# Gabriel-SGama/Semantic-SuperPoint

Hardware: AMD Instinct MI355X
Metric: image-pairs/sec at 240x320 bs32 (pair training step) (higher is better)
Workload: dtype f32

## Files before the change

### include/ssp_hip.h

```cpp
#ifndef SSP_HIP_H
#define SSP_HIP_H

#include <stddef.h>
#include <stdint.h>

#ifdef __cplusplus
extern "C" {
#endif

typedef struct ssp_handle ssp_handle;

enum { SSP_ARCH_GAUSS2 = 0, SSP_ARCH_GAUSS2_SSMALL = 1 };
enum { SSP_NREP = 32 };

typedef struct {
  int arch;
  int n_classes;
  int max_batch;
  int height;
  int width;
  int n_match;
  int n_non;
  int dense_loss;
} ssp_config;
// ... 333 lines not shown
int ssp_op_world_correspondences(const double* x_dev, const int32_t* state_dev, int map_cap, const float* match_dev,
                                 const int32_t* n_match_dev, int cap, const double* pts_new_dev, int pt_stride,
                                 const int32_t* count_new_dev, int point_cap, double* corr_dev, int32_t* n_corr_dev, void* stream);
int ssp_world_repair(const double* rw_dev, const double* c_dev, const int32_t* status_dev, double* state_dev, double* table_dev,
                     int capacity, int map_cap, int32_t* world_state_dev, void* stream);

#define SSP_LOOP_MAX_EDGES 256
#define SSP_LOOP_EDGE_WORDS 16
#define SSP_LOOP_STATE_WORDS 8
#define SSP_LOOP_CAND_WORDS 16
#define SSP_LOOP_MAX_INNER 8
#define SSP_LOOP_INFO_WORDS 8
#define SSP_LOOP_MAX_ITERATIONS 64
#define SSP_POSE_FLAG_LOOP 32
size_t ssp_pose_graph_workspace_bytes(int capacity);
int ssp_op_loop_correspondences(const double* x_dev, const int32_t* last_dev, const int32_t* state_dev, int map_cap,
                                const float* match_dev, const int32_t* n_match_dev, int cap, const double* pts_new_dev, int pt_stride,
                                const int32_t* count_new_dev, int point_cap, const double* landmarks_dev,
                                const int32_t* n_landmarks_dev, int row_cap, int f, int min_gap, double* corr_dev, double* xnew_dev,
                                int32_t* n_dev, void* stream);
int ssp_loop_edge(const double* rw_dev, const double* c_dev, const uint8_t* mask_dev, const int32_t* status_dev,
                  const double* corr_dev, const double* xnew_dev, const int32_t* n_dev, int cap, const int32_t* last_dev, int map_cap,
                  const double* table_dev, int capacity, int f, int min_inliers, int cooldown, double weight, double* edges_dev,
                  int32_t* state_dev, double* cand_dev, void* stream);
int ssp_pose_graph(const double* table_dev, int capacity, const double* edges_dev, const int32_t* state_dev, int f, int iterations,
                   void* workspace_dev, double* rw_out_dev, double* c_out_dev, double* sigma_out_dev, double* info_dev, void* stream);
int ssp_loop_apply(const double* info_dev, const double* rw_new_dev, const double* c_new_dev, const double* sigma_dev,
                   int32_t* loop_state_dev, int f, double* state_dev, double* table_dev, int capacity, double* x_dev,
                   const int32_t* last_dev, const int32_t* world_state_dev, int map_cap, void* stream);

#define SSP_EVAL_ACC_MAX_PAIRS 128
#define SSP_EVAL_ROW_WORDS 16
#define SSP_EVAL_STATE_WORDS 16
int ssp_eval_pixel_homographies(const float* hn_dev, int n_pairs, int height, int width, double* hom_dev, double* hom_inv_dev,
                                void* stream);
int ssp_eval_accumulate(const double* rep_dev, const double* h_dev, const int32_t* n_inlier_dev, const int32_t* status_dev,
                        const double* ap_dev, const int32_t* n1_dev, int pair_stride, const double* hom_dev, int n_pairs,
                        int corner_h, int corner_w, const double* thresholds, int64_t first_pair, double* rows_dev,
                        int64_t capacity, double* state_dev, void* stream);

#define SSP_DET_EVAL_MAX_R2 64
#define SSP_DET_EVAL_STATE_WORDS 80
#define SSP_DET_EVAL_CURVE_TILE 1024
typedef struct ssp_det_eval_params {
  int32_t height, width;
  float remove_zero;
  int32_t r2;
  float prob_thresh;
  int32_t simplified;
} ssp_det_eval_params;
size_t ssp_det_eval_workspace_bytes(const ssp_det_eval_params* p, int b, int cap);
int ssp_op_det_tp_fp(const float* prob_dev, const void* labels_dev, int labels_u8, const ssp_det_eval_params* p, int b,
                     void* workspace_dev, int64_t* keys_dev, int64_t capacity, int64_t* state_dev, void* stream);
int ssp_op_det_tp_fp_points(const float* pts_dev, const int32_t* count_dev, int cap, const void* labels_dev, int labels_u8,
                            const ssp_det_eval_params* p, int b, void* workspace_dev, int64_t* keys_dev, int64_t capacity,
                            int64_t* state_dev, void* stream);
size_t ssp_det_pr_curve_workspace_bytes(int64_t n_records);
int ssp_op_det_pr_curve(const int64_t* sorted_keys_dev, int64_t n_records, const int64_t* state_dev, void* workspace_dev,
                        float* prob_dev, uint8_t* tp_dev, double* precision_dev, double* recall_dev, double* map_dev,
                        void* stream);

#define SSP_TRACK_MAX_LENGTH 16
size_t ssp_track_workspace_bytes(int max_length, int point_cap, int row_cap);
int ssp_op_track_update(const int32_t* ids_in_dev, const int32_t* tid_in_dev, const double* score_in_dev,
                        const int32_t* state_in_dev, const float* match_dev, const double* match_score64_dev,
                        const int32_t* n_match_dev, const int32_t* n_points_dev, int max_length, int point_cap, int row_cap,
                        void* workspace_dev, int32_t* ids_out_dev, int32_t* tid_out_dev, double* score_out_dev,
                        int32_t* state_out_dev, void* stream);
int ssp_op_track_select(const int32_t* ids_dev, const int32_t* tid_dev, const double* score_dev, const int32_t* state_dev,
                        int max_length, int row_cap, int min_length, void* workspace_dev, double* tracks_dev,
                        int32_t* n_tracks_dev, void* stream);
int ssp_op_track_points(const double* tracks_dev, const int32_t* n_tracks_dev, const double* pts_dev, const int32_t* state_dev,
                        int max_length, int point_cap, int track_cap, int first_slot, double* xy_dev, void* stream);

int ssp_op_bn_bwd(const float* y_dev, const float* dout_dev, const float* gamma_dev, const float* stats4_dev,
                  float* dy_dev, float* dgamma_dev, float* dbeta_dev, float* dbias_dev, double* sums_dev, int n, int h,
                  int w, int c, int relu, int pool, void* stream);
int ssp_op_bn_bwd_strided(const float* y_dev, const float* dout_dev, const float* gamma_dev, const float* stats4_dev,
                          float* dy_dev, float* dgamma_dev, float* dbeta_dev, float* dbias_dev, double* sums_dev, int n,
                          int h, int w, int c, int cs, int relu, int pool, void* stream);

int ssp_set_conv_algo(int algo);
int ssp_handle_set_conv_algo(ssp_handle* h, int algo);

int ssp_debug_conv_knobs(int ablate, int grid);
int ssp_debug_occupancy(int which);

int ssp_debug_buffer(ssp_handle* h, int slot, const char* name, float** ptr, size_t* nfloats);

int ssp_debug_backward_taps(ssp_handle* h, float* arena_dev, size_t arena_floats, unsigned layer_mask);
size_t ssp_debug_backward_tap_floats(const ssp_handle* h, unsigned layer_mask);
int ssp_debug_backward_tap(ssp_handle* h, int slot, int layer, int which, size_t* offset, size_t* nfloats, unsigned* route);

int ssp_op_sparse_loss(const float* desc_a_nhwc_dev, const float* desc_b_nhwc_dev, const int32_t* match_a_dev,
                       const int32_t* match_b_dev, const int32_t* nonmatch_b_dev, int b, int hc, int wc, int n_match,
                       int n_non, int method, int dist, float coef_pos, float coef_neg, float* dd_a_nhwc_dev, float* dd_b_nhwc_dev,
                       float* out2_dev, void* stream);
int ssp_op_sparse_loss_path(const float* desc_a_nhwc_dev, const float* desc_b_nhwc_dev, const int32_t* match_a_dev,
                            const int32_t* match_b_dev, const int32_t* nonmatch_b_dev, int b, int hc, int wc, int n_match,
                            int n_non, int method, int dist, float coef_pos, float coef_neg, float* dd_a_nhwc_dev, float* dd_b_nhwc_dev,
                            float* out2_dev, int gather, int32_t* csr_off_dev, int32_t* csr_match_dev, float* csr_weight_dev,
                            void* stream);

int ssp_op_dense_loss(const float* desc_a_nhwc_dev, const float* desc_b_nhwc_dev, const float* homographies_dev,
                      const float* valid_dev, int b, int hc, int wc, float lamda_d, float descriptor_dist, int multi_task,
                      float scale, void* scratch_dev, size_t scratch_bytes, float* out3_dev, float* dda_dev,
                      float* ddb_dev, void* stream);

#ifdef __cplusplus
}
#endif
#endif
```

### semantic-superpoint_amd/csrc/bn_kernels.hip.h

```cpp
#pragma once
#include <hip/hip_runtime.h>
#include <stdint.h>

#include "conv_mfma.hip.h"

namespace sspk {

template <typename T>
__device__ __forceinline__ float4 ld4(const T* p) {
  if constexpr (sizeof(T) == 4) {
    return *reinterpret_cast<const float4*>(p);
  } else {
    const u32x2 v = *reinterpret_cast<const u32x2*>(p);
    return make_float4(bf16_lo(v[0]), bf16_hi(v[0]), bf16_lo(v[1]), bf16_hi(v[1]));
  }
}
template <typename T>
__device__ __forceinline__ void st4(T* p, float4 v) {
  if constexpr (sizeof(T) == 4) {
    *reinterpret_cast<float4*>(p) = v;
  } else {
    u32x2 o;
    o[0] = pack_bf16(v.x, v.y);
    o[1] = pack_bf16(v.z, v.w);
// ... 192 lines not shown
      var = s2 / L.count - mean * mean;
      if (var < 0) var = 0;
      const double unbiased = L.count > 1 ? var * L.count / (L.count - 1) : var;
      if (writer) {
        L.running_mean[c] = (float)(0.9 * (double)L.running_mean[c] + 0.1 * mean);
        L.running_var[c] = (float)(0.9 * (double)L.running_var[c] + 0.1 * unbiased);
        if (c == 0 && nbt != nullptr) *nbt += 1;
      }
    } else {
      mean = L.running_mean[c];
      var = L.running_var[c];
    }
    if (writer) {
      const float invstd = (float)(1.0 / sqrt(var + 1e-5));
      const float sc = L.gamma[c] * invstd;
      L.mean[c] = (float)mean;
      L.invstd[c] = invstd;
      L.scale[c] = sc;
      L.shift[c] = L.beta[c] - (float)mean * sc;
    }
  }
}
__global__ void bn_finalize_kernel(const BnLayer L0, const BnLayer L1, int nviews, int train, int64_t* nbt) {
  bn_finalize_body(L0, L1, nviews, train, nbt);
}
struct BnFinJobs {
  BnLayer L0[3], L1[3];
  int64_t* nbt[3];
  int n;
};
__global__ void bn_finalize_multi_kernel(const BnFinJobs J, int nviews, int train) {
  const int j = blockIdx.y;
  bn_finalize_body(J.L0[j], J.L1[j], nviews, train, J.nbt[j]);
}

__global__ __launch_bounds__(256) void bn_relu_pool_kernel(const float* __restrict__ y0, const float* __restrict__ scale0,
                                                           const float* __restrict__ shift0, float* __restrict__ out0,
                                                           const float* __restrict__ y1, const float* __restrict__ scale1,
                                                           const float* __restrict__ shift1, float* __restrict__ out1,
                                                           int N, int H, int W, int C) {
  const float* __restrict__ y = blockIdx.y ? y1 : y0;
  const float* __restrict__ scale = blockIdx.y ? scale1 : scale0;
  const float* __restrict__ shift = blockIdx.y ? shift1 : shift0;
  float* __restrict__ out = blockIdx.y ? out1 : out0;
  const int nq = C >> 2;
  const long total = (long)N * (H / 2) * (W / 2) * nq;
  const int Wo = W / 2, Ho = H / 2;
  for (long idx = (long)blockIdx.x * blockDim.x + threadIdx.x; idx < total; idx += (long)gridDim.x * blockDim.x) {
    const int q = (int)(idx % nq);
    const long p = idx / nq;
    const int ox = (int)(p % Wo), oy = (int)((p / Wo) % Ho), n = (int)(p / ((long)Wo * Ho));
    const float4 sc = *reinterpret_cast<const float4*>(scale + q * 4);
    const float4 sh = *reinterpret_cast<const float4*>(shift + q * 4);
    const size_t base = ((size_t)(n * H + 2 * oy) * W + 2 * ox) * C + q * 4;
    const float4 a = xform<1>(*reinterpret_cast<const float4*>(y + base), sc, sh);
    const float4 b = xform<1>(*reinterpret_cast<const float4*>(y + base + C), sc, sh);
    const float4 c = xform<1>(*reinterpret_cast<const float4*>(y + base + (size_t)W * C), sc, sh);
    const float4 d = xform<1>(*reinterpret_cast<const float4*>(y + base + (size_t)W * C + C), sc, sh);
    *reinterpret_cast<float4*>(out + (size_t)p * C + q * 4) = max4(max4(a, b), max4(c, d));
  }
}

struct BnBwdArgs {
  const float* y;
  const float* dout;
  float* dy;
  const float* scale;
  const float* shift;
  const float* mean;
  const float* invstd;
  const float* gamma;
  double* sums;
  const float* k12;
  float* dbias;
  const float* x;
  const float* apool;
  const float* beta;
  int pool_fix;
  int N, H, W, C;
  int y_cs, y_co, d_cs, d_co, dy_cs, dy_co;
  double count;
};

template <bool RELU, bool POOL, bool APPLY, typename T = float>
__global__ __launch_bounds__(256) void bn_bwd_kernel(const BnBwdArgs a0, const BnBwdArgs a1, const BnBwdArgs b0, const BnBwdArgs b1) {
  const BnBwdArgs& a = blockIdx.y == 0 ? a0 : blockIdx.y == 1 ? a1 : blockIdx.y == 2 ? b0 : b1;
  const T* const t_y = reinterpret_cast<const T*>(a.y);
  const T* const t_dout = reinterpret_cast<const T*>(a.dout);
  T* const t_dy = reinterpret_cast<T*>(a.dy);
  __shared__ float red[256 * 8];
  const int tid = threadIdx.x;
  const int nq = (a.C + 3) / 4;
  const int rows = 256 / nq;
  const int q = tid % nq, pl = tid / nq;
  const bool active = pl < rows;
  const int c0 = q * 4;
  const int Ho = POOL ? a.H / 2 : a.H, Wo = POOL ? a.W / 2 : a.W;
  const long npix = (long)a.N * Ho * Wo;
  float4 sc = make_float4(0, 0, 0, 0), sh = sc, mu = sc, is = sc, k1 = sc, k2 = sc, gs = sc;
  bool cv[4];
#pragma unroll
  for (int i = 0; i < 4; ++i) cv[i] = (c0 + i) < a.C;
  auto ldp = [&](const float* p) {
    float4 v = make_float4(0, 0, 0, 0);
    if (cv[0]) v.x = p[c0];
    if (cv[1]) v.y = p[c0 + 1];
    if (cv[2]) v.z = p[c0 + 2];
    if (cv[3]) v.w = p[c0 + 3];
    return v;
  };
  if (active) {
    sc = ldp(a.scale);
    sh = ldp(a.shift);
    mu = ldp(a.mean);
    is = ldp(a.invstd);
    if (APPLY) {
      const float4 g = ldp(a.gamma);
      float s1[4], s2[4];
#pragma unroll
      for (int i = 0; i < 4; ++i) {
        s1[i] = cv[i] ? a.k12[c0 + i] : 0.f;
        s2[i] = cv[i] ? a.k12[a.C + c0 + i] : 0.f;
      }
      k1 = make_float4(s1[0], s1[1], s1[2], s1[3]);
      k2 = make_float4(s2[0], s2[1], s2[2], s2[3]);
      gs = make_float4(g.x * is.x, g.y * is.y, g.z * is.z, g.w * is.w);
    }
  }
  float acc[8] = {0, 0, 0, 0, 0, 0, 0, 0};
  const float scv[4] = {sc.x, sc.y, sc.z, sc.w}, shv[4] = {sh.x, sh.y, sh.z, sh.w};
  const float muv[4] = {mu.x, mu.y, mu.z, mu.w}, isv[4] = {is.x, is.y, is.z, is.w};
  const float k1v[4] = {k1.x, k1.y, k1.z, k1.w}, k2v[4] = {k2.x, k2.y, k2.z, k2.w};
  const float gsv[4] = {gs.x, gs.y, gs.z, gs.w};
  if (active) {
    for (long p = (long)blockIdx.x * rows + pl; p < npix; p += (long)gridDim.x * rows) {
      const int ox = (int)(p % Wo);
      const int oy = (int)((p / Wo) % Ho);
      const int n = (int)(p / ((long)Wo * Ho));
      const float4 d4 = ld4<T>(t_dout + (size_t)p * a.d_cs + a.d_co + c0);
      const float dv[4] = {d4.x, d4.y, d4.z, d4.w};
      if (!POOL) {
        const size_t yo = (size_t)p * a.y_cs + a.y_co + c0;
        const float4 y4 = ld4<T>(t_y + yo);
        const float yv[4] = {y4.x, y4.y, y4.z, y4.w};
        float o[4];
#pragma unroll
        for (int i = 0; i < 4; ++i) {
          const float z = fmaf(yv[i], scv[i], shv[i]);
          const float dz = (!RELU || z > 0.f) ? dv[i] : 0.f;
          const float xh = (yv[i] - muv[i]) * isv[i];
          if (!APPLY) {
            acc[i] += dz;
            acc[4 + i] += dz * xh;
          } else {
            o[i] = gsv[i] * (dz - k1v[i] - xh * k2v[i]);
            acc[i] += o[i];
          }
        }
        if (APPLY) st4<T>(t_dy + (size_t)p * a.dy_cs + a.dy_co + c0, make_float4(o[0], o[1], o[2], o[3]));
      } else {
        float yv[4][4], o[4][4];
        size_t yo[4];
#pragma unroll
        for (int k = 0; k < 4; ++k) {
          const int yy = 2 * oy + (k >> 1), xx = 2 * ox + (k & 1);
          yo[k] = ((size_t)(n * a.H + yy) * a.W + xx);
// ... 372 lines not shown
  if (idx >= (long)N * C * HW) return;
  const int c = (int)(idx % C);
  const int p = (int)((idx / C) % HW);
  const int n = (int)(idx / ((long)HW * C));
  out[((size_t)n * HW + p) * cs + co + c] = in[((size_t)n * C + c) * HW + p];
}

__global__ __launch_bounds__(256) void desc_normalize_kernel(const float* __restrict__ y0, const float* __restrict__ scale0,
                                                             const float* __restrict__ shift0, float* __restrict__ desc0,
                                                             float* __restrict__ inv_norm0, float* __restrict__ zero_out0, int ncells,
                                                             int cs, int co, const float* __restrict__ y1 = nullptr,
                                                             const float* __restrict__ scale1 = nullptr,
                                                             const float* __restrict__ shift1 = nullptr, float* __restrict__ desc1 = nullptr,
                                                             float* __restrict__ inv_norm1 = nullptr, float* __restrict__ zero_out1 = nullptr) {
  const bool v1 = blockIdx.y != 0;
  const float* __restrict__ y = v1 ? y1 : y0;
  const float* __restrict__ scale = v1 ? scale1 : scale0;
  const float* __restrict__ shift = v1 ? shift1 : shift0;
  float* __restrict__ desc = v1 ? desc1 : desc0;
  float* __restrict__ inv_norm = v1 ? inv_norm1 : inv_norm0;
  float* __restrict__ zero_out = v1 ? zero_out1 : zero_out0;
  const int wave = (blockIdx.x * blockDim.x + threadIdx.x) >> 6;
  const int lane = threadIdx.x & 63;
  if (wave >= ncells) return;
  if (zero_out != nullptr) *reinterpret_cast<float4*>(zero_out + (size_t)wave * 256 + lane * 4) = make_float4(0.f, 0.f, 0.f, 0.f);
  const float4 v = *reinterpret_cast<const float4*>(y + (size_t)wave * cs + co + lane * 4);
  const float4 sc = *reinterpret_cast<const float4*>(scale + lane * 4);
  const float4 sh = *reinterpret_cast<const float4*>(shift + lane * 4);
  float4 r = make_float4(fmaf(v.x, sc.x, sh.x), fmaf(v.y, sc.y, sh.y), fmaf(v.z, sc.z, sh.z), fmaf(v.w, sc.w, sh.w));
  float s = r.x * r.x + r.y * r.y + r.z * r.z + r.w * r.w;
#pragma unroll
  for (int o = 32; o > 0; o >>= 1) s += __shfl_xor(s, o);
  const float inv = 1.f / sqrtf(s);
  *reinterpret_cast<float4*>(desc + (size_t)wave * 256 + lane * 4) = make_float4(r.x * inv, r.y * inv, r.z * inv, r.w * inv);
  if (lane == 0) inv_norm[wave] = inv;
}

struct DescGather {
  const int32_t* off;
  const int32_t* match;
  const float* weight;
  const float* rows;
  int cells, n_match;
};
__device__ __forceinline__ float4 desc_gather_cell(const DescGather& G, int cell, int side, int lane, float4 g) {
  const int img = cell / G.cells, c = cell - img * G.cells;
  const int list = img * 2 + side;
  const int32_t* off = G.off + (size_t)list * (G.cells + 1);
  const int e0 = off[c], e1 = off[c + 1];
  const int32_t* em = G.match + (size_t)list * 4 * G.n_match;
  const float* ew = G.weight + (size_t)list * 4 * G.n_match;
  const float* rows = G.rows + ((size_t)img * G.n_match * 2 + side) * 256 + lane * 4;
  for (int b0 = e0; b0 < e1; b0 += 64) {
    const int n = min(64, e1 - b0);
    const int le = b0 + min(lane, n - 1);
    const int ml = em[le];
    const int wl = lane < n ? __float_as_int(ew[le]) : 0;
    for (int i = 0; i < n; i += 4) {
      float4 r[4];
      float w[4];
#pragma unroll
      for (int u = 0; u < 4; ++u) {
        const int s = min(i + u, 63);
        w[u] = __int_as_float(__builtin_amdgcn_readlane(wl, s));
        r[u] = *reinterpret_cast<const float4*>(rows + (size_t)__builtin_amdgcn_readlane(ml, s) * 512);
      }
#pragma unroll
      for (int u = 0; u < 4; ++u) {
        g.x = fmaf(w[u], r[u].x, g.x); g.y = fmaf(w[u], r[u].y, g.y); g.z = fmaf(w[u], r[u].z, g.z); g.w = fmaf(w[u], r[u].w, g.w);
      }
    }
  }
  return g;
}
__global__ __launch_bounds__(256) void desc_gather_kernel(float* __restrict__ d0, float* __restrict__ d1, int ncells, DescGather G) {
  float* __restrict__ d = blockIdx.y != 0 ? d1 : d0;
  const int wave = (blockIdx.x * blockDim.x + threadIdx.x) >> 6;
  const int lane = threadIdx.x & 63;
  if (wave >= ncells) return;
  float4* p = reinterpret_cast<float4*>(d + (size_t)wave * 256 + lane * 4);
  *p = desc_gather_cell(G, wave, (int)blockIdx.y, lane, *p);
}

__global__ __launch_bounds__(256) void desc_normalize_bwd_kernel(const float* __restrict__ desc0,
                                                                 const float* __restrict__ inv_norm0,
                                                                 float* __restrict__ d0, int ncells,
                                                                 const float* __restrict__ desc1 = nullptr,
                                                                 const float* __restrict__ inv_norm1 = nullptr,
                                                                 float* __restrict__ d1 = nullptr,
                                                                 DescGather G = DescGather{nullptr, nullptr, nullptr, nullptr, 0, 0}) {
  const bool v1 = blockIdx.y != 0;
  const float* __restrict__ desc = v1 ? desc1 : desc0;
  const float* __restrict__ inv_norm = v1 ? inv_norm1 : inv_norm0;
  float* __restrict__ d = v1 ? d1 : d0;
  const int wave = (blockIdx.x * blockDim.x + threadIdx.x) >> 6;
  const int lane = threadIdx.x & 63;
  if (wave >= ncells) return;
  const float4 n = *reinterpret_cast<const float4*>(desc + (size_t)wave * 256 + lane * 4);
  float4 g = *reinterpret_cast<const float4*>(d + (size_t)wave * 256 + lane * 4);
  if (G.off != nullptr) g = desc_gather_cell(G, wave, v1 ? 1 : 0, lane, g);
  float s = n.x * g.x + n.y * g.y + n.z * g.z + n.w * g.w;
#pragma unroll
  for (int o = 32; o > 0; o >>= 1) s += __shfl_xor(s, o);
  const float inv = inv_norm[wave];
  g = make_float4((g.x - n.x * s) * inv, (g.y - n.y * s) * inv, (g.z - n.z * s) * inv, (g.w - n.w * s) * inv);
  *reinterpret_cast<float4*>(d + (size_t)wave * 256 + lane * 4) = g;
}

__global__ void adam_kernel(float* __restrict__ p, const float* __restrict__ g, float* __restrict__ m,
                            float* __restrict__ v, long n, float step_size, float bc2_sqrt) {
  const long i = (long)blockIdx.x * blockDim.x + threadIdx.x;
  if (i >= n) return;
  const float gi = g[i];
  const float mi = 0.9f * m[i] + 0.1f * gi;
  const float vi = 0.999f * v[i] + 0.001f * gi * gi;
  m[i] = mi;
  v[i] = vi;
  const float denom = sqrtf(vi) / bc2_sqrt + 1e-8f;
  p[i] -= step_size * (mi / denom);
}

__global__ void adam_scaled_kernel(float* __restrict__ p, const float* __restrict__ g, float* __restrict__ m,
                                   float* __restrict__ v, long n, float step_size, float bc2_sqrt, float gscale) {
  const long i = (long)blockIdx.x * blockDim.x + threadIdx.x;
  if (i >= n) return;
  const float gi = g[i] * gscale;
  const float mi = 0.9f * m[i] + 0.1f * gi;
  const float vi = 0.999f * v[i] + 0.001f * gi * gi;
  m[i] = mi;
  v[i] = vi;
  const float denom = sqrtf(vi) / bc2_sqrt + 1e-8f;
  p[i] -= step_size * (mi / denom);
}

}
```

### semantic-superpoint_amd/csrc/loss_kernels.hip.h

```cpp
#pragma once
#include <hip/hip_runtime.h>
#include <stdint.h>

#include "det.hip.h"

namespace sspk {

template <typename Op>
__device__ __forceinline__ float wave_reduce(float v, float identity, Op op) {
  auto dpp = [&](float x, int ctrl_sel) {
    const int xi = __float_as_int(x), idn = __float_as_int(identity);
    int r;
    switch (ctrl_sel) {
      case 0: r = __builtin_amdgcn_update_dpp(idn, xi, 0xB1, 0xF, 0xF, false); break;
      case 1: r = __builtin_amdgcn_update_dpp(idn, xi, 0x4E, 0xF, 0xF, false); break;
      case 2: r = __builtin_amdgcn_update_dpp(idn, xi, 0x141, 0xF, 0xF, false); break;
      case 3: r = __builtin_amdgcn_update_dpp(idn, xi, 0x140, 0xF, 0xF, false); break;
      case 4: r = __builtin_amdgcn_update_dpp(idn, xi, 0x142, 0xA, 0xF, false); break;
      default: r = __builtin_amdgcn_update_dpp(idn, xi, 0x143, 0xC, 0xF, false); break;
    }
    return __int_as_float(r);
  };
  v = op(v, dpp(v, 0));
  v = op(v, dpp(v, 1));
  v = op(v, dpp(v, 2));
  v = op(v, dpp(v, 3));
  v = op(v, dpp(v, 4));
  v = op(v, dpp(v, 5));
  return __int_as_float(__builtin_amdgcn_readlane(__float_as_int(v), 63));
}
__device__ __forceinline__ float wave_sum(float v) {
  return wave_reduce(v, 0.f, [](float a, float b) { return a + b; });
}
__device__ __forceinline__ float wave_max(float v) {
  return wave_reduce(v, -__builtin_inff(), [](float a, float b) { return fmaxf(a, b); });
}
__device__ __forceinline__ float wave_prod(float v) {
  return wave_reduce(v, 1.f, [](float a, float b) { return a * b; });
}

__device__ __forceinline__ float block_sum_of_waves(float v, float* smem4) {
  const int wave = threadIdx.x >> 6, lane = threadIdx.x & 63;
  __syncthreads();
  if (lane == 0) smem4[wave] = v;
  __syncthreads();
  return smem4[0] + smem4[1] + smem4[2] + smem4[3];
}

constexpr int SSP_MAX_PAIRS = 128;
constexpr int SSP_DENSE_REPS = 1024;
struct StepAccum {
  double det_sum[2];
  double mask_cnt[2];
  double sem_sum[2];
  double sem_cnt[2];
  double pos_sum[SSP_MAX_PAIRS * 16];
  double neg_sum[SSP_MAX_PAIRS * 16];
  unsigned int nnz[SSP_MAX_PAIRS * 16];
  unsigned int nnz_img[SSP_MAX_PAIRS];
  double dense_sum[SSP_DENSE_REPS];
  float coef_det, coef_pos, coef_neg, coef_sem;
};

static_assert(sizeof(StepAccum) <= 65536, "the ssp_op_* loss operators carve a StepAccum out of a 64 KiB scratch");

__device__ __forceinline__ unsigned nnz_of_image(const StepAccum* acc, int img) {
  unsigned nz = 0;
#pragma unroll
  for (int r = 0; r < 16; ++r) nz += acc->nnz[img * 16 + r];
  return nz;
}

__global__ __launch_bounds__(256) void cell_mask_kernel(const float* __restrict__ mask2d0, float* __restrict__ cellmask0,
                                                        double* __restrict__ mask_cnt0, int B, int H, int W,
                                                        const float* __restrict__ mask2d1 = nullptr, float* __restrict__ cellmask1 = nullptr,
                                                        double* __restrict__ mask_cnt1 = nullptr) {
  const float* __restrict__ mask2d = blockIdx.y ? mask2d1 : mask2d0;
  float* __restrict__ cellmask = blockIdx.y ? cellmask1 : cellmask0;
  double* __restrict__ mask_cnt = blockIdx.y ? mask_cnt1 : mask_cnt0;
  __shared__ float red[4];
  const int Hc = H / 8, Wc = W / 8;
  const int lane = threadIdx.x & 63;
  const int ncell = B * Hc * Wc;
  float cnt = 0.f;
  for (int cell = (blockIdx.x * blockDim.x + threadIdx.x) >> 6; cell < ncell; cell += (gridDim.x * blockDim.x) >> 6) {
    const int cx = cell % Wc, cy = (cell / Wc) % Hc, n = cell / (Wc * Hc);
    const float m = mask2d[((size_t)n * H + cy * 8 + (lane >> 3)) * W + cx * 8 + (lane & 7)];
    const float p = wave_prod(m);
    if (lane == 0) cellmask[cell] = p;
    cnt += p;
  }
  const float tot = block_sum_of_waves(cnt, red);
  if (threadIdx.x == 0) unsafeAtomicAdd(mask_cnt, (double)tot);
}

__global__ __launch_bounds__(256) void labels2dto3d_kernel(const float* __restrict__ labels2d, float* __restrict__ target,
                                                           int B, int H, int W) {
  const int Hc = H / 8, Wc = W / 8;
  const int cell = (blockIdx.x * blockDim.x + threadIdx.x) >> 6;
  const int lane = threadIdx.x & 63;
  if (cell >= B * Hc * Wc) return;
  const int cx = cell % Wc, cy = (cell / Wc) % Hc, n = cell / (Wc * Hc);
  const float lab = labels2d[((size_t)n * H + cy * 8 + (lane >> 3)) * W + cx * 8 + (lane & 7)];
  const float lsum = wave_sum(lab);
  float dust = 1.f - lsum;
  if (dust < 1.f) dust = 0.f;
  const float dn = lsum + dust;
  target[(((size_t)n * 65 + lane) * Hc + cy) * Wc + cx] = lab / dn;
  if (lane == 0) target[(((size_t)n * 65 + 64) * Hc + cy) * Wc + cx] = dust / dn;
}

__global__ __launch_bounds__(256) void detector_loss_kernel(const float* __restrict__ ypb0, const float* __restrict__ scale0,
                                                            const float* __restrict__ shift0,
                                                            const float* __restrict__ labels2d0,
                                                            const float* __restrict__ cellmask0, float* __restrict__ dsemi0,
                                                            StepAccum* __restrict__ acc, int view0, int B, int H, int W,
                                                            int cs, const float* __restrict__ ypb1 = nullptr,
                                                            const float* __restrict__ scale1 = nullptr,
                                                            const float* __restrict__ shift1 = nullptr,
                                                            const float* __restrict__ labels2d1 = nullptr,
                                                            const float* __restrict__ cellmask1 = nullptr,
                                                            float* __restrict__ dsemi1 = nullptr) {
  const bool v1 = blockIdx.y != 0;
  const float* __restrict__ ypb = v1 ? ypb1 : ypb0;
  const float* __restrict__ scale = v1 ? scale1 : scale0;
  const float* __restrict__ shift = v1 ? shift1 : shift0;
  const float* __restrict__ labels2d = v1 ? labels2d1 : labels2d0;
  const float* __restrict__ cellmask = v1 ? cellmask1 : cellmask0;
  float* __restrict__ dsemi = v1 ? dsemi1 : dsemi0;
  const int view = view0 + (v1 ? 1 : 0);
  __shared__ float red[4];
  const int Hc = H / 8, Wc = W / 8;
  const int lane = threadIdx.x & 63;
  const int ncell = B * Hc * Wc;
  const float sc_l = scale[lane], sh_l = shift[lane], sc_d = scale[64], sh_d = shift[64];
  const float coef0 = (dsemi != nullptr) ? acc->coef_det / ((float)acc->mask_cnt[view] + 1e-5f) : 0.f;
  float lsum_acc = 0.f;
  for (int cell = (blockIdx.x * blockDim.x + threadIdx.x) >> 6; cell < ncell; cell += (gridDim.x * blockDim.x) >> 6) {
    const int cx = cell % Wc, cy = (cell / Wc) % Hc, n = cell / (Wc * Hc);
    const float lab = labels2d[((size_t)n * H + cy * 8 + (lane >> 3)) * W + cx * 8 + (lane & 7)];
    const float lsum = wave_sum(lab);
    float dust = 1.f - lsum;
    if (dust < 1.f) dust = 0.f;
    const float dn = lsum + dust;
    const float t = lab / dn, td = dust / dn;
    const float* yp = ypb + (size_t)cell * cs;
    const float s = fmaf(yp[lane], sc_l, sh_l);
    const float sd = fmaf(yp[64], sc_d, sh_d);
    const float mx = fmaxf(wave_max(s), sd);
    const float e = expf(s - mx), ed = expf(sd - mx);
    const float inv = 1.f / (wave_sum(e) + ed);
    const float p = e * inv, pd = ed * inv;
    const float l = -(t * fmaxf(logf(p), -100.f) + (1.f - t) * fmaxf(log1pf(-p), -100.f));
    const float ld = -(td * fmaxf(logf(pd), -100.f) + (1.f - td) * fmaxf(log1pf(-pd), -100.f));
    const float m = cellmask[cell];
    lsum_acc += (wave_sum(l) + ld) * m;
    if (dsemi != nullptr) {
      const float coef = coef0 * m;
      const float g = (p - t) / fmaxf(p * (1.f - p), 1e-12f);
      const float gd = (pd - td) / fmaxf(pd * (1.f - pd), 1e-12f);
      const float dot = wave_sum(g * p) + gd * pd;
      float* dp = dsemi + (size_t)cell * cs;
      dp[lane] = coef * p * (g - dot);
      if (lane == 0) dp[64] = coef * pd * (gd - dot);
      if (lane >= 1 && lane < cs - 64) dp[64 + lane] = 0.f;
    }
  }
  const float tot = block_sum_of_waves(lsum_acc, red);
  if (threadIdx.x == 0) acc_add_loss(&acc->det_sum[view], (double)tot);
}

struct Bilin {
  int i00, i01, i10, i11;
  float w00, w01, w10, w11;
};
__device__ __forceinline__ Bilin bilin_setup(int cell, int Hc, int Wc) {
  const float u = (float)(cell % Wc), v = (float)(cell / Wc);
  const float gx = u / (float)Wc * 2.f - 1.f, gy = v / (float)Hc * 2.f - 1.f;
  const float tx = (gx + 1.f) / 2.f, ty = (gy + 1.f) / 2.f;
  const float ix = tx * (float)(Wc - 1), iy = ty * (float)(Hc - 1);
  const float fx = floorf(ix), fy = floorf(iy);
  const int x0 = (int)fx, y0 = (int)fy, x1 = x0 + 1, y1 = y0 + 1;
  const float ax = fmaf(tx, (float)(Wc - 1), -fx), ay = fmaf(ty, (float)(Hc - 1), -fy);
  Bilin b;
  const bool vx0 = x0 >= 0 && x0 < Wc, vx1 = x1 >= 0 && x1 < Wc, vy0 = y0 >= 0 && y0 < Hc, vy1 = y1 >= 0 && y1 < Hc;
  const int cx0 = min(max(x0, 0), Wc - 1), cx1 = min(max(x1, 0), Wc - 1);
  const int cy0 = min(max(y0, 0), Hc - 1), cy1 = min(max(y1, 0), Hc - 1);
  b.i00 = cy0 * Wc + cx0; b.i01 = cy0 * Wc + cx1; b.i10 = cy1 * Wc + cx0; b.i11 = cy1 * Wc + cx1;
  b.w00 = (vx0 && vy0) ? (1.f - ax) * (1.f - ay) : 0.f;
  b.w01 = (vx1 && vy0) ? ax * (1.f - ay) : 0.f;
  b.w10 = (vx0 && vy1) ? (1.f - ax) * ay : 0.f;
  b.w11 = (vx1 && vy1) ? ax * ay : 0.f;
  return b;
}
__device__ __forceinline__ Bilin bilin_cell(int cell) {
  Bilin b;
  b.i00 = b.i01 = b.i10 = b.i11 = cell;
  b.w00 = 1.f; b.w01 = b.w10 = b.w11 = 0.f;
  return b;
}
constexpr int DESC_METHOD_1D = 1;
constexpr int DESC_EUCLIDEAN = 2;
__device__ __forceinline__ float4 f4_fma(float w, float4 a, float4 acc) {
  return make_float4(fmaf(w, a.x, acc.x), fmaf(w, a.y, acc.y), fmaf(w, a.z, acc.z), fmaf(w, a.w, acc.w));
}
__device__ __forceinline__ void atomic_add4(float* p, float4 v) {
  facc_add(p, v.x);
  facc_add(p + 1, v.y);
  facc_add(p + 2, v.z);
  facc_add(p + 3, v.w);
}


static inline int desc_grid(int B, int n_match) { return ((B + 7) / 8) * 8 * ((n_match + 3) / 4); }
__device__ __forceinline__ int desc_wave_of_block(int B, int n_match, int& img) {
  const int bpi = (n_match + 3) >> 2;
  const int xcd = blockIdx.x & 7, slot = blockIdx.x >> 3;
  const int round = slot / bpi;
  img = round * 8 + xcd;
  const int k = (slot - round * bpi) * 4 + (threadIdx.x >> 6);
  return (img < B && k < n_match) ? img * n_match + k : -1;
}
template <bool BWD, bool EUC = false, bool GATHER = false>
__global__ __launch_bounds__(256) void desc_match_kernel(const float* __restrict__ desc_a, const float* __restrict__ desc_b,
                                                         const int32_t* __restrict__ match_a,
                                                         const int32_t* __restrict__ match_b, float* __restrict__ dd_a,
                                                         float* __restrict__ dd_b, StepAccum* __restrict__ acc, int B,
                                                         int Hc, int Wc, int n_match, int flags, float* __restrict__ g_rows = nullptr) {
  const DetTarget t_a = GATHER ? DetTarget{nullptr, nullptr} : det_resolve(dd_a);
  const DetTarget t_b = GATHER ? DetTarget{nullptr, nullptr} : det_resolve(dd_b);
  int img;
  const int w = desc_wave_of_block(B, n_match, img);
  const int lane = threadIdx.x & 63;
  if (w < 0) return;
  const bool m1d = (flags & DESC_METHOD_1D) != 0;
  constexpr bool euc = EUC;
  const size_t base = (size_t)img * Hc * Wc * 256 + lane;
  const Bilin ba = m1d ? bilin_cell(match_a[w]) : bilin_setup(match_a[w], Hc, Wc);
  const Bilin bb = m1d ? bilin_cell(match_b[w]) : bilin_setup(match_b[w], Hc, Wc);
  float va[4] = {0.f, 0.f, 0.f, 0.f}, vb[4] = {0.f, 0.f, 0.f, 0.f};
  const int ia[4] = {ba.i00, ba.i01, ba.i10, ba.i11}, ib[4] = {bb.i00, bb.i01, bb.i10, bb.i11};
  const float wa[4] = {ba.w00, ba.w01, ba.w10, ba.w11}, wb[4] = {bb.w00, bb.w01, bb.w10, bb.w11};
  if (m1d) {
#pragma unroll
    for (int j = 0; j < 4; ++j) {
      va[j] = desc_a[base + (size_t)ia[0] * 256 + 64 * j];
      vb[j] = desc_b[base + (size_t)ib[0] * 256 + 64 * j];
    }
  } else {
// ... 388 lines not shown
```

### semantic-superpoint_amd/csrc/ssp.hip

```cpp
#include "../../include/ssp_hip.h"

#include <hip/hip_runtime.h>

#include <cmath>
#include <cstdarg>
#include <cstdio>
#include <cstdlib>
#include <algorithm>
#include <cstring>
#include <string>
#include <vector>

#include "bn_kernels.hip.h"
#include "conv_mfma.hip.h"
#include "conv1x1_group.hip.h"
#include "conv_wino.hip.h"
#include "conv_wino_pipe.hip.h"
#include "conv_wino_p2.hip.h"
#include "conv_wino4.hip.h"
#include "wgrad_wino4.hip.h"
#include "wgrad_wino_fused.hip.h"
#include "conv_bf16.hip.h"
#include "conv_bf16_ws.hip.h"
#include "wgrad_bf16.hip.h"
// ... 116 lines not shown
    HIPCHK(hipMemcpy(host, dev, sizeof(host), hipMemcpyDeviceToHost));
    return 0;
  }
};

static inline int cdiv(long a, long b) { return (int)((a + b - 1) / b); }
static int device_cu_count() {
  static int cached[64] = {};
  int dev = 0;
  if (hipGetDevice(&dev) != hipSuccess || dev < 0 || dev >= 64) return 256;
  if (cached[dev] == 0) {
    int n = 0;
    cached[dev] = (hipDeviceGetAttribute(&n, hipDeviceAttributeMultiprocessorCount, dev) == hipSuccess && n > 0) ? n : 256;
  }
  return cached[dev];
}
static inline size_t align_up(size_t v, size_t a) { return (v + a - 1) / a * a; }

struct LayerDesc {
  int cin, cout, ks;
  bool bn;
  size_t w_off, b_off, g_off, be_off;
  int bn_index;
  size_t bn_ch_off;
  size_t pk_fwd, pk_bwd;
  int nchunks_fwd, ncob_fwd, nchunks_bwd, ncob_bwd;
};

struct BnBufs {
  double* stats;
  double* bsums;
  float *scale, *shift, *mean, *invstd;
  float* k12;
};

struct Slot {
  float* Y[16];
  int y_cs[16], y_co[16];
  BnBufs bn[16];
  float* desc;
  float* inv_norm;
  float* cellmask;
  float* dsemi;
  float* ddesc;
  float* dsout;
  float *gP, *gQ;
  float* Apool[8];
  bool pool_raw[8] = {false, false, false, false, false, false, false, false};
  float* act[8] = {nullptr, nullptr, nullptr, nullptr, nullptr, nullptr, nullptr, nullptr};
  bool act_valid[8] = {false, false, false, false, false, false, false, false};
  const float* x;
  void* stats_region;
  size_t stats_bytes;
  int N, H, W;
  bool bsums_dirty;
  bool has_desc;
};

struct ssp_handle {
  ssp_config cfg;
  int nlayers, nheads;
  LayerDesc L[16];
  size_t n_params, n_bn_ch;
  int n_bn;
  ssp_buffers buf;
  bool bound;
  size_t ws_bytes;
  Slot slot[2];
  float *wpk_fwd, *wpk_bwd, *wpk_heads_bwd;
  float* partial;
  size_t partial_floats;
  size_t partial_used = 0;
  struct WredBQueue* rq_bf16 = nullptr;
  WredJobs rjobs{};
  bool bsums_fused[16] = {};
  bool sums_lazy[16] = {};
  bool fin_pending[16] = {};
  double fin_count[16] = {};
  bool apply_fused[16] = {};
  bool bf16_fuse_apply = true;
  StepAccum* accum;
  float* dots;
  bool desc_gather = true;
  int32_t *csr_off = nullptr, *csr_match = nullptr;
  float* csr_weight = nullptr;
  float* g_rows = nullptr;
  float* dense_coef;
  int sout_cs;
  int conv_algo;
  bool pk_w4_fwd[16] = {}, pk_w4_bwd[16] = {};
  float *wpk_g1_fwd[16] = {}, *wpk_g1_bwd[16] = {};
  bool pk_g1[16] = {};
  float* g1_partial = nullptr;
  TailJobs tail = {};
  int g1_partial_slabs = 0;
  int packed_algo = -1;
  bool packed_bwd = false;
  struct GraphEntry { std::vector<unsigned char> key; hipGraphExec_t exec; };
  std::vector<GraphEntry> graphs;
  uint64_t* graph_seed;
  hipStream_t aux_stream = nullptr;
  hipStream_t aux2_stream = nullptr;
  hipEvent_t ev_fork = nullptr, ev_join = nullptr;
  hipEvent_t ev_pack_fork = nullptr, ev_pack_join = nullptr;
  hipEvent_t ev_early_fork = nullptr, ev_early_join = nullptr;
  int prof_family;
  bool prof_paused = false;
  std::vector<hipEvent_t> ev_pool;
  size_t ev_used;
  double prof_flops, prof_bytes, prof_exec_flops;
  int64_t prof_launches;
  struct ProfKernel { double flops = 0, exec_flops = 0, bytes = 0; int64_t launches = 0; } prof_k[SSP_PROF_K_COUNT];
  std::vector<unsigned char> ev_kernel;
  int n_cu;
  float* tap_arena = nullptr;
  unsigned tap_mask = 0;
  unsigned tap_route[16] = {};
  int tap_wk = 0, tap_dk = 0;
};

enum { TAP_BSUMS_FUSED = 1, TAP_APPLY_FUSED = 2, TAP_SUMS_LAZY = 4, TAP_ACT_INPUT = 8, TAP_WG_SHIFT = 4, TAP_DG_SHIFT = 8 };
enum { TAP_WG_FUSED12 = 1, TAP_WG_WINO = 2, TAP_WG_WINO4 = 3, TAP_WG_DIRECT = 4, TAP_WG_GROUPED = 5, TAP_WG_L0 = 6, TAP_WG_BF16 = 7 };
enum { TAP_DG_WINO4 = 1, TAP_DG_PIPE = 2, TAP_DG_P2 = 3, TAP_DG_DIRECT = 4, TAP_DG_GROUPED = 5, TAP_DG_BF16 = 6, TAP_DG_BF16_WS = 7 };

struct AlgoScope {
  int prev;
  explicit AlgoScope(const ssp_handle* h) : prev(g_conv_algo) { g_conv_algo = h ? h->conv_algo : g_default_conv_algo; }
  ~AlgoScope() { g_conv_algo = prev; }
};

enum { L_PA = 8, L_PB = 9, L_DA = 10, L_DB = 11, L_DS = 12, L_SOUT = 13 };
static const int kEnc[8][2] = {{1, 64}, {64, 64}, {64, 64}, {64, 64}, {64, 128}, {128, 128}, {128, 128}, {128, 128}};

static void build_layers(ssp_handle* h) {
  int n = 0;
  auto add = [&](int cin, int cout, int ks, bool bn) {
    LayerDesc& d = h->L[n++];
    d.cin = cin; d.cout = cout; d.ks = ks; d.bn = bn;
  };
  for (int i = 0; i < 8; ++i) add(kEnc[i][0], kEnc[i][1], 3, true);
  add(128, 256, 3, true);
  add(256, 65, 1, true);
  add(128, 256, 3, true);
  add(256, 256, 1, true);
  h->nheads = 2;
  if (h->cfg.arch == SSP_ARCH_GAUSS2_SSMALL) {
    add(128, 256, 3, true);
    add(256, h->cfg.n_classes, 1, false);
    h->nheads = 3;
  }
  h->nlayers = n;
  size_t off = 0, bnch = 0, pf = 0, pb = 0;
  int nbn = 0;
  for (int i = 0; i < n; ++i) {
    LayerDesc& d = h->L[i];
    d.w_off = off; off += (size_t)d.cout * d.cin * d.ks * d.ks;
    d.b_off = off; off += d.cout;
    if (d.bn) {
      d.g_off = off; off += d.cout;
      d.be_off = off; off += d.cout;
      d.bn_index = nbn++;
      d.bn_ch_off = bnch; bnch += d.cout;
    } else {
      d.g_off = d.be_off = 0; d.bn_index = -1; d.bn_ch_off = 0;
    }
    const int taps = d.ks * d.ks;
// ... 620 lines not shown
#if WGF_TRACE
      if (a.trace) {
        CHK(tr.fetch(st));
        const unsigned long long* hbuf = tr.host;
        const double nt = (double)std::max<unsigned long long>(hbuf[6], 1);
        fprintf(stderr, "[wgf trace] %dx%d cin %d cout %d mode %d pool %d nprob %d: %llu tiles of workgroup 0 at %.0f MHz; cycles per tile (MFMA floor 2 x 8192 per SIMD)\n",
                a.H, a.W, a.Cin, a.Cout, c.in_mode, (int)c.fuse_pool, a.nprob, hbuf[6], 100.0 * (double)hbuf[5] / (double)std::max<unsigned long long>(hbuf[7], 1));
        for (int w = 0; w < 8; ++w)
          fprintf(stderr, "  wave %d: top barrier %.0f  staging %.0f  barrier %.0f  issue %.0f  mfma %.0f  | loop %.0f\n", w, hbuf[w * 8] / nt,
                  hbuf[w * 8 + 1] / nt, hbuf[w * 8 + 2] / nt, hbuf[w * 8 + 3] / nt, hbuf[w * 8 + 4] / nt, hbuf[w * 8 + 5] / nt);
      }
#endif
    } else if (wino4) {
      constexpr size_t lw = Wgrad4Geom<true>::LDS_BYTES, ln = Wgrad4Geom<false>::LDS_BYTES;
      const dim3 block(WG4_THREADS);
      if (c.in_mode == 0) CHK((wide ? launch_lds<wgrad_wino4_kernel<0, true>>(lw, grid, block, lw, st, a)
                                    : launch_lds<wgrad_wino4_kernel<0, false>>(ln, grid, block, ln, st, a)));
      else CHK((wide ? launch_lds<wgrad_wino4_kernel<1, true>>(lw, grid, block, lw, st, a)
                     : launch_lds<wgrad_wino4_kernel<1, false>>(ln, grid, block, ln, st, a)));
    } else if (wino) {
      constexpr size_t lw = WgradWinoGeom<true>::LDS_BYTES, ln = WgradWinoGeom<false>::LDS_BYTES;
      if (c.in_mode == 0) CHK((wide ? launch_lds<wgrad_wino_kernel<0, true>>(lw, grid, dim3(512), lw, st, a)
                                    : launch_lds<wgrad_wino_kernel<0, false>>(ln, grid, dim3(512), ln, st, a)));
      else CHK((wide ? launch_lds<wgrad_wino_kernel<1, true>>(lw, grid, dim3(512), lw, st, a)
                     : launch_lds<wgrad_wino_kernel<1, false>>(ln, grid, dim3(512), ln, st, a)));
    }
    if (wino) {
      if (!deferred && wino4)
        hipLaunchKernelGGL(wgrad_wino4_reduce_kernel, dim3(a.ncob * c.cin), dim3(256), 0, st, partial, c.dw, c.cin, c.cout,
                           a.ncob, nsplit);
      else if (!deferred && fused12)
        hipLaunchKernelGGL(wgrad_fused12_reduce_kernel, dim3(3 * a.ncob * c.cin), dim3(256), 0, st, partial, c.dw, c.cin, c.cout,
                           a.ncob, nsplit);
      else if (!deferred)
        hipLaunchKernelGGL(wgrad_wino_reduce_kernel, dim3(a.ncob * c.cin), dim3(256), 0, st, partial, c.dw, c.cin, c.cout,
                           a.ncob, nsplit);
      HIPCHK(hipGetLastError());
      return 0;
    }
#define WG_CASE(KS_, M_)                                                                                    \
  if (c.ks == KS_ && c.in_mode == M_) {                                                                     \
    constexpr size_t lw = WgradGeom<KS_, 1, 32>::LDS_BYTES, ln = WgradGeom<KS_, 4, 8>::LDS_BYTES;           \
    CHK((wide ? launch_lds<wgrad_mfma_kernel<KS_, M_, 1, 32>>(lw, grid, dim3(256), lw, st, a)               \
              : launch_lds<wgrad_mfma_kernel<KS_, M_, 4, 8>>(ln, grid, dim3(256), ln, st, a)));             \
  } else
    WG_CASE(3, 0) WG_CASE(3, 1) WG_CASE(3, 2) WG_CASE(1, 0) WG_CASE(1, 1)
    return fail(-3, "unsupported wgrad variant ks=%d in_mode=%d", c.ks, c.in_mode);
#undef WG_CASE
  }
  const int total = c.cout * c.cin * taps;
  hipLaunchKernelGGL(wgrad_reduce_kernel, dim3(cdiv(total, 64)), dim3(256), 0, st, partial, c.dw, c.cin, c.cout, c.ks,
                     a.ncob, nsplit);
  HIPCHK(hipGetLastError());
  return 0;
}

static int launch_pack(const float* w, float* dst, int cout_w, int cin_w, int ks, int tf, bool wino, hipStream_t st, bool w4 = false) {
  const int taps = ks * ks;
  const int conv_cin = tf ? cout_w : cin_w, conv_cout = tf ? cin_w : cout_w;
  const int nchunks = cdiv(conv_cin, CK), ncob = cdiv(conv_cout, NB);
  if (wino) {
    const int total = ncob * nchunks * WB_FLOATS;
    if (w4)
      hipLaunchKernelGGL(pack_weights_wino4_kernel, dim3(cdiv(ncob * 2 * nchunks * W4_B_FLOATS, 256)), dim3(256), 0, st, w, dst,
                         cout_w, cin_w, tf, 2 * nchunks, 0, 0, ncob, 2 * nchunks);
    else
      hipLaunchKernelGGL(pack_weights_wino8_kernel, dim3(cdiv(total, 256)), dim3(256), 0, st, w, dst, cout_w, cin_w, tf,
                         2 * nchunks, 0, 0, ncob, 2 * nchunks);
    HIPCHK(hipGetLastError());
    return 0;
  }
  const int total = ncob * nchunks * taps * CK * NB;
  hipLaunchKernelGGL(pack_weights_kernel, dim3(cdiv(total, 256)), dim3(256), 0, st, w, dst, cout_w, cin_w, ks, tf,
                     nchunks, 0, 0, ncob, nchunks);
  HIPCHK(hipGetLastError());
  return 0;
}

struct BnPlainJob {
  BnBwdArgs a[2];
  float* dg = nullptr;
  float* db = nullptr;
  bool filled = false;
};
struct BnSumsQueue {
  BnSumsJobs J;
  int maxC = 0;
  BnSumsQueue() { J.n = 0; }
};
static int flush_bn_sums(BnSumsQueue& q, int nviews, hipStream_t st) {
  if (q.J.n == 0) return 0;
  if (q.J.n == 1) hipLaunchKernelGGL(bn_bwd_sums_kernel<float>, dim3(cdiv(q.maxC * 32, 256)), dim3(256), 0, st, q.J.a0[0], q.J.a1[0], nviews,
                                     q.J.dgamma[0], q.J.dbeta[0]);
  else hipLaunchKernelGGL(bn_bwd_sums_multi_kernel<float>, dim3(cdiv(q.maxC * 32, 256), q.J.n), dim3(256), 0, st, q.J, nviews);
  HIPCHK(hipGetLastError());
  q.J.n = 0; q.maxC = 0;
  return 0;
}
template <bool RELU, bool POOL, typename T = float>
static int launch_bn_bwd(const BnBwdArgs* a, int nviews, float* dgamma, float* dbeta, hipStream_t st,
                         bool sums_done = false, bool skip_apply = false, BnSumsQueue* queue = nullptr) {
  if (queue != nullptr && sums_done && skip_apply && (sizeof(T) == 4 || a[0].pool_fix == 0) && queue->J.n < 3) {
    const int j = queue->J.n++;
    queue->J.a0[j] = a[0]; queue->J.a1[j] = a[nviews - 1]; queue->J.dgamma[j] = dgamma; queue->J.dbeta[j] = dbeta;
    queue->maxC = std::max(queue->maxC, a[0].C);
    return 0;
  }
  const BnBwdArgs& a0 = a[0];
  const BnBwdArgs& a1 = a[nviews - 1];
  const int nq = (a0.C + 3) / 4, rows = 256 / nq;
  const long npix = (long)a0.N * (POOL ? a0.H / 2 : a0.H) * (POOL ? a0.W / 2 : a0.W);
  int nb = cdiv(npix, rows);
  if (nb > 1024) nb = 1024;
  if (!sums_done)
    hipLaunchKernelGGL((bn_bwd_kernel<RELU, POOL, false, T>), dim3(nb, nviews), dim3(256), 0, st, a0, a1, a0, a1);
  hipLaunchKernelGGL(bn_bwd_sums_kernel<T>, dim3(cdiv(a0.C * 32, 256)), dim3(256), 0, st, a0, a1, nviews, dgamma, dbeta);
  if (!skip_apply)
    hipLaunchKernelGGL((bn_bwd_kernel<RELU, POOL, true, T>), dim3(nb, nviews), dim3(256), 0, st, a0, a1, a0, a1);
  HIPCHK(hipGetLastError());
  return 0;
}

template <typename K>
static int l0_resident_grid(K kern, const ssp_handle* h, int nviews, long rows, int W) {
  static int per_cu = 0, per_cu_w = 0;
  if (per_cu_w != W) { per_cu = 0; per_cu_w = W; }
  if (per_cu == 0 && (hipOccupancyMaxActiveBlocksPerMultiprocessor(&per_cu, kern, 256, l0_lds_bytes(W)) != hipSuccess || per_cu < 1)) {
    (void)hipGetLastError();
    per_cu = -1;
  }
  if (per_cu < 1) return l0_grid(rows);
  const long g = std::max(1L, (long)per_cu * (h ? h->n_cu : 256) / std::max(1, nviews));
  return (int)std::min(rows, g);
}

#include "bf16_host.hip.h"

static int flush_wgrad_reduce_bf16(ssp_handle* h, hipStream_t st) { return h->rq_bf16 != nullptr ? h->rq_bf16->flush(st) : 0; }

static int ensure_aux_stream(ssp_handle* h);

struct DetHostRegion { float* lo; size_t n; long long* shadow; const ssp_handle* owner; };
static std::vector<DetHostRegion> g_det_regions;
static int g_det_mode = -1;
static int g_det_device = -1;
static bool det_mode() {
  if (g_det_mode < 0) g_det_mode = deterministic_env() ? 1 : 0;
  return g_det_mode == 1;
}
static int det_upload() {
  DetRegion tab[DET_MAX_REGIONS];
  int n = 0;
  for (const DetHostRegion& r : g_det_regions) {
    if (n == DET_MAX_REGIONS) return fail(-3, "deterministic mode: more than %d fp32 scatter targets are bound in this process", DET_MAX_REGIONS);
    tab[n].lo = r.lo; tab[n].hi = r.lo + r.n; tab[n].shadow = r.shadow; ++n;
  }
  for (int i = n; i < DET_MAX_REGIONS; ++i) { tab[i].lo = tab[i].hi = nullptr; tab[i].shadow = nullptr; }
  const int flag = det_mode() ? 1 : 0;
  HIPCHK(hipMemcpyToSymbol(HIP_SYMBOL(g_det_region), tab, sizeof(tab)));
  HIPCHK(hipMemcpyToSymbol(HIP_SYMBOL(g_det_nregion), &n, sizeof(n)));
  HIPCHK(hipMemcpyToSymbol(HIP_SYMBOL(g_det), &flag, sizeof(flag)));
  return 0;
}
static void det_release(const ssp_handle* h) {
  bool any = false;
  for (size_t i = 0; i < g_det_regions.size();) {
// ... 600 lines not shown
  else for (int k = 0; k < SS.n; ++k) CHK(dev_zero(SS.s[k]->stats_region, SS.s[k]->stats_bytes, st));
  SideFork pack_fork;
  CHK(ensure_aux_stream(h));
  CHK(pack_fork.fork(st, h->aux_stream, h->ev_pack_fork, h->ev_pack_join));
  CHK(pack_all(h, for_backward, SS.n, N, H, W, h->aux_stream));
  {
    const LayerDesc& d = h->L[0];
    Slot &S0 = *SS.s[0], &S1 = *SS.s[SS.n - 1];
    if (bf16_path())
      hipLaunchKernelGGL(conv0_direct_kernel<uint16_t>, dim3(l0_resident_grid(conv0_direct_kernel<uint16_t>, h, SS.n, (long)N * H, W), SS.n), dim3(256), l0_lds_bytes(W), st, S0.x, S1.x, P(h, d.w_off),
                         P(h, d.b_off), reinterpret_cast<uint16_t*>(S0.Y[0]), reinterpret_cast<uint16_t*>(S1.Y[0]),
                         train ? S0.bn[0].stats : nullptr, train ? S1.bn[0].stats : nullptr, N, H, W);
    else
    hipLaunchKernelGGL(conv0_direct_kernel<float>, dim3(l0_resident_grid(conv0_direct_kernel<float>, h, SS.n, (long)N * H, W), SS.n), dim3(256), l0_lds_bytes(W), st, S0.x, S1.x, P(h, d.w_off),
                       P(h, d.b_off), S0.Y[0], S1.Y[0], train ? S0.bn[0].stats : nullptr, train ? S1.bn[0].stats : nullptr,
                       N, H, W);
    HIPCHK(hipGetLastError());
    if (train && !bf16_path()) { h->fin_pending[0] = true; h->fin_count[0] = (double)N * H * W; }
    else CHK(bn_finalize(h, SS.s, SS.n, 0, (double)N * H * W, train, st));
  }
  CHK(pack_fork.join());
  for (int l = 1; l < 8; ++l) {
    int lh, lw; layer_res(l, H, W, lh, lw);
    CHK(conv_layer_fwd(h, SS, l, l - 1, N, lh, lw, layer_in_mode(l), train, st));
  }
  const int Hc = H / 8, Wc = W / 8;
  auto pointwise = [&](const int* layers, int n) -> int {
    bool grouped = true;
    for (int i = 0; i < n; ++i) grouped = grouped && h->pk_g1[layers[i]];
    if (!grouped) {
      BnDeferred fin;
      for (int i = 0; i < n; ++i) CHK(conv_layer_fwd(h, SS, layers[i], layers[i] - 1, N, Hc, Wc, 1, train, st, &fin));
      return bn_finalize_n(h, SS.s, SS.n, fin.layers, fin.n, (double)N * Hc * Wc, train, st);
    }
    G1Layer Lg[3];
    for (int i = 0; i < n; ++i) {
      const int l = layers[i], src = l - 1;
      const LayerDesc& d = h->L[l];
      G1Layer& y = Lg[i];
      y.in_cs = SS.s[0]->y_cs[src]; y.in_co = SS.s[0]->y_co[src]; y.out_cs = SS.s[0]->y_cs[l]; y.out_co = SS.s[0]->y_co[l];
      y.wpk = h->wpk_g1_fwd[l]; y.bias = P(h, d.b_off); y.K = d.cin; y.N = d.cout;
      for (int k = 0; k < SS.n; ++k) {
        Slot& S = *SS.s[k];
        y.in[k] = S.Y[src]; y.out[k] = S.Y[l]; y.scale[k] = S.bn[src].scale; y.shift[k] = S.bn[src].shift;
        y.stats[k] = (d.bn && train) ? S.bn[l].stats : nullptr;
      }
    }
    CHK(launch_g1(Lg, n, SS.n, (long)N * Hc * Wc, 1, h->n_cu, st));
    int bl[3], nbl = 0;
    for (int i = 0; i < n; ++i)
      if (h->L[layers[i]].bn) bl[nbl++] = layers[i];
    return bn_finalize_n(h, SS.s, SS.n, bl, nbl, (double)N * Hc * Wc, train, st);
  };
  const int pw[3] = {L_DB, L_SOUT, L_PB};
  BnDeferred fin3;
  CHK(conv_layer_fwd(h, SS, L_PA, 7, N, Hc, Wc, 1, train, st, &fin3));
  if (detector_only) {
    CHK(bn_finalize_n(h, SS.s, SS.n, fin3.layers, fin3.n, (double)N * Hc * Wc, train, st));
    return pointwise(pw + 2, 1);
  }
  CHK(conv_layer_fwd(h, SS, L_DA, 7, N, Hc, Wc, 1, train, st, &fin3));
  if (h->nheads == 3) CHK(conv_layer_fwd(h, SS, L_DS, 7, N, Hc, Wc, 1, train, st, &fin3));
  CHK(bn_finalize_n(h, SS.s, SS.n, fin3.layers, fin3.n, (double)N * Hc * Wc, train, st));
  if (h->nheads == 3) {
    CHK(pointwise(pw, 3));
  } else {
    const int pw2[2] = {L_DB, L_PB};
    CHK(pointwise(pw2, 2));
  }
  for (int l = 0; l < 8; ++l) CHK(bn_finalize_pending(h, SS, l, train, st));
  const int ncells = N * Hc * Wc;
  {
    Slot &S = *SS.s[0], &T = *SS.s[SS.n - 1];
    hipLaunchKernelGGL(desc_normalize_kernel, dim3(cdiv(ncells, 4), SS.n), dim3(256), 0, st, S.Y[L_DB], S.bn[L_DB].scale,
                       S.bn[L_DB].shift, S.desc, S.inv_norm, zero_ddesc ? S.ddesc : (float*)nullptr, ncells, S.y_cs[L_DB], S.y_co[L_DB],
                       T.Y[L_DB], T.bn[L_DB].scale, T.bn[L_DB].shift, T.desc, T.inv_norm, zero_ddesc ? T.ddesc : (float*)nullptr);
  }
  HIPCHK(hipGetLastError());
  return 0;
}

static int bn_layer_backward(ssp_handle* h, const SlotSet& SS, int l, const float* const* dout, int d_cs, int d_co, bool relu,
                             bool pool_after, float* const* dy, int dy_cs, int dy_co, int N, int H, int W, hipStream_t st,
                             BnSumsQueue* queue = nullptr, BnPlainJob* collect = nullptr) {
  const LayerDesc& d = h->L[l];
  BnBwdArgs a[2];
  bool have_pool = true;
  for (int k = 0; k < SS.n; ++k) {
    Slot& S = *SS.s[k];
    BnBwdArgs& v = a[k];
    v.y = S.Y[l]; v.dout = dout[k]; v.dy = dy[k]; v.scale = S.bn[l].scale; v.shift = S.bn[l].shift; v.mean = S.bn[l].mean;
    v.invstd = S.bn[l].invstd; v.gamma = P(h, d.g_off); v.sums = S.bn[l].bsums; v.dbias = Gd(h, d.b_off);
    v.x = S.x; v.apool = l < 8 ? S.Apool[l] : nullptr; v.beta = P(h, d.be_off); v.pool_fix = 0;
    v.N = N; v.H = H; v.W = W; v.C = d.cout; v.y_cs = S.y_cs[l]; v.y_co = S.y_co[l]; v.d_cs = d_cs; v.d_co = d_co;
    v.dy_cs = dy_cs; v.dy_co = dy_co; v.count = (double)N * H * W;
    v.k12 = S.bn[l].k12;
    have_pool = have_pool && v.apool != nullptr;
  }
  const bool fused = h->bsums_fused[l];
  h->bsums_fused[l] = false;
  if (fused) h->tap_route[l] |= TAP_BSUMS_FUSED;
  h->apply_fused[l] = false;
  const bool raw_pool = pool_after && l < 8 && SS.s[0]->pool_raw[l];
  if ((fused || raw_pool) && pool_after)
    for (int k = 0; k < SS.n; ++k) a[k].pool_fix = 1;
  const BnBwdArgs &a0 = a[0], &a1 = a[SS.n - 1];
  float *dg = Gd(h, d.g_off), *db = Gd(h, d.be_off);
  if (l == 0) {
    const int nb1 = l0_resident_grid(bn_bwd_reduce_l0_kernel<float>, h, SS.n, (long)N * H, W);
    const int nb2 = l0_resident_grid(bn_bwd_apply_l0_kernel<float>, h, SS.n, (long)N * H, W);
    if (!fused)
      hipLaunchKernelGGL(bn_bwd_reduce_l0_kernel<float>, dim3(nb1, SS.n), dim3(256), l0_lds_bytes(W), st, a0, a1, P(h, d.w_off), P(h, d.b_off));
    hipLaunchKernelGGL(bn_bwd_sums_kernel<float>, dim3(cdiv(64 * 32, 256)), dim3(256), 0, st, a0, a1, SS.n, dg, db);
    hipLaunchKernelGGL(bn_bwd_apply_l0_kernel<float>, dim3(nb2, SS.n), dim3(256), l0_lds_bytes(W), st, a0, a1, P(h, d.w_off), P(h, d.b_off),
                       Gd(h, d.w_off));
    h->tap_route[0] |= TAP_WG_L0 << TAP_WG_SHIFT;
  } else if (relu && pool_after && have_pool && d.cout % 4 == 0 && d_cs == d.cout && d_co == 0) {
    const long npix = (long)N * (H / 2) * (W / 2);
    const int rows = 256 / (d.cout / 4);
    const int nb = std::max(1, std::min(cdiv(npix, rows), 1024));
    if (!fused && !SS.s[0]->pool_raw[l]) hipLaunchKernelGGL(bn_bwd_reduce_pool_kernel, dim3(nb, SS.n), dim3(256), 0, st, a0, a1, P(h, d.be_off));
    else if (!fused) {
      BnBwdArgs r[2] = {a[0], a[SS.n - 1]};
      for (int k = 0; k < 2; ++k) {
        r[k].y = r[k].apool; r[k].y_cs = d.cout; r[k].y_co = 0; r[k].H = H / 2; r[k].W = W / 2;
      }
      hipLaunchKernelGGL((bn_bwd_kernel<true, false, false>), dim3(nb, SS.n), dim3(256), 0, st, r[0], r[1], r[0], r[1]);
    }
    hipLaunchKernelGGL(bn_bwd_sums_kernel<float>, dim3(cdiv(d.cout * 32, 256)), dim3(256), 0, st, a0, a1, SS.n, dg, db);
    const bool defer = l >= 1 && l < 8 && layer_in_mode(l) == 1 && dy_cs == d.cout && dy_co == 0 && SS.s[0]->y_cs[l] == d.cout &&
                       SS.s[0]->y_co[l] == 0 && wgrad_can_fuse_apply(d.ks, 1, H, W, d.cout);
    h->apply_fused[l] = defer;
    if (!defer) hipLaunchKernelGGL((bn_bwd_kernel<true, true, true>), dim3(nb, SS.n), dim3(256), 0, st, a0, a1, a0, a1);
  } else if (relu && pool_after) CHK((launch_bn_bwd<true, true>(a, SS.n, dg, db, st, fused)));
  else if (relu) {
    const bool defer = l >= 1 && d_cs == SS.s[0]->y_cs[l] && d_co == SS.s[0]->y_co[l] && dy_cs == d_cs && dy_co == d_co &&
                       wgrad_can_fuse_apply(d.ks, 1, H, W, d.cout);
    h->apply_fused[l] = defer;
    if (fused && defer) h->sums_lazy[l] = true;
    else CHK((launch_bn_bwd<true, false>(a, SS.n, dg, db, st, fused, defer, queue)));
  }
  else if (collect != nullptr) {
    collect->a[0] = a0; collect->a[1] = a1; collect->dg = dg; collect->db = db; collect->filled = true;
    return 0;
  }
  else CHK((launch_bn_bwd<false, false>(a, SS.n, dg, db, st)));
  HIPCHK(hipGetLastError());
  return 0;
}
static int launch_bn_bwd_pair(const BnPlainJob& p, const BnPlainJob& q, int nviews, hipStream_t st) {
  auto blocks = [](const BnBwdArgs& a) {
    const int nq = (a.C + 3) / 4, rows = 256 / nq;
    return std::min(cdiv((long)a.N * a.H * a.W, rows), 1024);
  };
  const int nb = std::max(blocks(p.a[0]), blocks(q.a[0]));
  hipLaunchKernelGGL((bn_bwd_kernel<false, false, false, float>), dim3(nb, 4), dim3(256), 0, st, p.a[0], p.a[1], q.a[0], q.a[1]);
  BnSumsQueue sq;
  sq.J.n = 2; sq.maxC = std::max(p.a[0].C, q.a[0].C);
  sq.J.a0[0] = p.a[0]; sq.J.a1[0] = p.a[1]; sq.J.dgamma[0] = p.dg; sq.J.dbeta[0] = p.db;
  sq.J.a0[1] = q.a[0]; sq.J.a1[1] = q.a[1]; sq.J.dgamma[1] = q.dg; sq.J.dbeta[1] = q.db;
  CHK(flush_bn_sums(sq, nviews, st));
  hipLaunchKernelGGL((bn_bwd_kernel<false, false, true, float>), dim3(nb, 4), dim3(256), 0, st, p.a[0], p.a[1], q.a[0], q.a[1]);
  HIPCHK(hipGetLastError());
  return 0;
}

static void setup_bnr(ssp_handle* h, const SlotSet& SS, int src, bool pooled, ConvCall& c) {
  if (src < 0 || !h->L[src].bn || !can_fuse_bnr(c) || c.out_co != 0 || c.out_cs != c.cout || c.cout != h->L[src].cout) return;
  const LayerDesc& ds = h->L[src];
  for (int k = 0; k < SS.n; ++k) {
    Slot& S = *SS.s[k];
    if (pooled && S.pool_raw[src]) {
      if (S.Apool[src] == nullptr) return;
      c.bnr_t[k] = S.Apool[src];
      c.bnr_p[0][k] = S.bn[src].scale; c.bnr_p[1][k] = S.bn[src].shift; c.bnr_p[2][k] = S.bn[src].mean;
      c.bnr_p[3][k] = S.bn[src].invstd;
    } else if (pooled) {
      if (S.Apool[src] == nullptr) return;
      c.bnr_t[k] = S.Apool[src];
      c.bnr_p[0][k] = P(h, ds.be_off); c.bnr_p[1][k] = P(h, ds.g_off);
    } else {
      c.bnr_t[k] = S.Y[src];
      c.bnr_p[0][k] = S.bn[src].scale; c.bnr_p[1][k] = S.bn[src].shift; c.bnr_p[2][k] = S.bn[src].mean;
      c.bnr_p[3][k] = S.bn[src].invstd;
    }
  }
  c.bnr_mode = (pooled && !SS.s[0]->pool_raw[src]) ? 2 : 1;
  c.bnr_cs = pooled ? ds.cout : SS.s[0]->y_cs[src];
  c.bnr_co = pooled ? 0 : SS.s[0]->y_co[src];
  if (c.bnr_cs % 4 != 0 || c.bnr_co % 4 != 0) { c.bnr_mode = 0; return; }
  c.stats = SS.s[0]->bn[src].bsums;
  if (SS.n == 2) c.stats2 = SS.s[1]->bn[src].bsums;
  h->bsums_fused[src] = true;
}

static int conv_layer_backward(ssp_handle* h, const SlotSet& SS, int l, int src, float* const* dy, int dy_cs, int dy_co,
                               float* const* din, int din_cs, int din_co, int N, int H, int W, int in_mode,
                               hipStream_t st, bool skip_dgrad = false, bool skip_wgrad = false) {
  const LayerDesc& d = h->L[l];
  Slot& A = *SS.s[0];
  const bool pooled = in_mode == 2;
  if (pooled) in_mode = A.pool_raw[src] ? 1 : 0;
  WgradCall w;
  w.in = pooled ? A.Apool[src] : A.Y[src]; w.in_cs = A.y_cs[src]; w.in_co = A.y_co[src]; w.cin = d.cin;
  w.dout = dy[0]; w.dout_cs = dy_cs; w.dout_co = dy_co; w.cout = d.cout;
  w.in_scale = A.bn[src].scale; w.in_shift = A.bn[src].shift; w.dw = Gd(h, d.w_off);
  w.N = N; w.H = H; w.W = W; w.ks = d.ks; w.in_mode = in_mode;
  ConvCall c;
  c.in = dy[0]; c.in_cs = dy_cs; c.in_co = dy_co; c.cin = (int)align_up(d.cout, 4);
  c.wpk = h->wpk_bwd + d.pk_bwd; c.bias = nullptr; c.wino = wino_ok(d.ks, d.cout);
  c.out = din[0]; c.out_cs = din_cs; c.out_co = din_co; c.cout = d.cin;
  c.in_scale = nullptr; c.in_shift = nullptr; c.stats = nullptr;
  c.N = N; c.H = H; c.W = W; c.ks = d.ks; c.in_mode = 0; c.nchunks = d.nchunks_bwd; c.ncob = d.ncob_bwd;
  c.force_w4 = h->pk_w4_bwd[l] ? 1 : 0;
  if (SS.n == 2) {
    Slot& B = *SS.s[1];
    w.nprob = 2; w.in2 = pooled ? B.Apool[src] : B.Y[src]; w.dout2 = dy[1]; w.in_scale2 = B.bn[src].scale;
    w.in_shift2 = B.bn[src].shift;
    c.nprob = 2; c.in2 = dy[1]; c.out2 = din[1];
  }
  if (d.ks == 3 && src < 8) setup_bnr(h, SS, src, pooled, c);
  if (l < 8 && h->apply_fused[l]) {
    h->apply_fused[l] = false;
    h->tap_route[l] |= TAP_APPLY_FUSED;
    w.fuse_apply = true;
    w.fuse_pool = (l == 1 || l == 3 || l == 5);
    w.dout_cs = d.cout; w.dout_co = 0; w.f_gamma = P(h, d.g_off); w.f_ycs = A.y_cs[l];
    for (int k = 0; k < SS.n; ++k) {
      Slot& S = *SS.s[k];
      (k ? w.dout2 : w.dout) = din[k];
      w.f_y[k] = S.Y[l]; w.f_dy[k] = dy[k]; w.f_scale[k] = S.bn[l].scale; w.f_shift[k] = S.bn[l].shift;
      w.f_mean[k] = S.bn[l].mean; w.f_invstd[k] = S.bn[l].invstd; w.f_k12[k] = S.bn[l].k12;
    }
    if (h->sums_lazy[l]) {
      h->sums_lazy[l] = false;
      h->tap_route[l] |= TAP_SUMS_LAZY;
      w.f_lazy = 1; w.f_count = (double)N * H * W; w.f_dgamma = Gd(h, d.g_off); w.f_dbeta = Gd(h, d.be_off); w.f_dbias = Gd(h, d.b_off);
      for (int k = 0; k < SS.n; ++k) w.f_bsums[k] = SS.s[k]->bn[l].bsums;
    }
// ... 174 lines not shown
    hipLaunchKernelGGL(colsum_kernel, dim3(cdiv((long)ncells, COLSUM_ROWS), SS.n), dim3(256), 0, st, dsout[0], Gd(h, d.b_off), (int)ncells, d.cout,
                       h->sout_cs, dsout[SS.n - 1]);
    HIPCHK(hipGetLastError());
    CHK(pointwise(L_SOUT, L_DS, dsout, h->sout_cs, 512));
  }
  if (has_semi) CHK(tap_copy(h, SS, L_PB, 1, gQs, ncells * 80, st));
  if (has_desc) CHK(tap_copy(h, SS, L_DB, 1, gQd, ncells * 256, st));
  {
    float* gP[2] = {nullptr, nullptr};
    for (int k = 0; k < SS.n; ++k) gP[k] = SS.s[k]->gP;
    CHK(tap_copy(h, SS, L_PA, 0, gP, ncells * hcs, st, sizeof(uint16_t)));
  }
  const int heads[3] = {L_PA, L_DA, L_DS};
  const bool heads_fuse = h->bf16_fuse_apply;
  BnSumsQueue sums_queue;
  for (int hk = 0; hk < h->nheads; ++hk) {
    const LayerDesc& d = h->L[heads[hk]];
    BnBwdArgs a[2];
    for (int k = 0; k < SS.n; ++k) {
      Slot& S = *SS.s[k];
      BnBwdArgs& v = a[k];
      const int l = heads[hk];
      v.y = S.Y[l]; v.dout = S.gP; v.dy = S.gQ; v.scale = S.bn[l].scale; v.shift = S.bn[l].shift; v.mean = S.bn[l].mean;
      v.invstd = S.bn[l].invstd; v.gamma = P(h, d.g_off); v.sums = S.bn[l].bsums; v.dbias = Gd(h, d.b_off);
      v.x = nullptr; v.apool = nullptr; v.beta = P(h, d.be_off); v.pool_fix = 0;
      v.N = N; v.H = Hc; v.W = Wc; v.C = 256; v.y_cs = hcs; v.y_co = 256 * hk; v.d_cs = hcs; v.d_co = 256 * hk;
      v.dy_cs = hcs; v.dy_co = 256 * hk; v.count = (double)ncells; v.k12 = S.bn[l].k12;
    }
    const bool sums_fused = h->bsums_fused[heads[hk]];
    h->bsums_fused[heads[hk]] = false;
    if (sums_fused) h->tap_route[heads[hk]] |= TAP_BSUMS_FUSED;
    CHK((launch_bn_bwd<true, false, uint16_t>(a, SS.n, Gd(h, d.g_off), Gd(h, d.be_off), st, sums_fused, heads_fuse, &sums_queue)));
  }
  CHK(flush_bn_sums(sums_queue, SS.n, st));
  for (int hk = 0; hk < h->nheads; ++hk) {
    const LayerDesc& d = h->L[heads[hk]];
    WgradBCall w;
    w.nviews = SS.n; w.N = N; w.H = Hc; w.W = Wc; w.ks = 3; w.in_mode = 1;
    w.x_cs = 128; w.x_co = 0; w.cin = 128; w.dy_cs = hcs; w.dy_co = 256 * hk; w.cout = 256; w.dw = Gd(h, d.w_off);
    const bool from_act7 = S0.act_valid[7] && SS.s[SS.n - 1]->act_valid[7];
    if (from_act7) w.in_mode = 0;
    h->tap_route[heads[hk]] |= (from_act7 ? (unsigned)TAP_ACT_INPUT : 0u) | (heads_fuse ? (unsigned)TAP_APPLY_FUSED : 0u) |
                               (unsigned)TAP_WG_BF16 << TAP_WG_SHIFT;
    for (int k = 0; k < SS.n; ++k) {
      Slot& S = *SS.s[k];
      w.x[k] = from_act7 ? S.act[7] : S.Y[7]; w.dy[k] = S.gQ; w.x_scale[k] = S.bn[7].scale; w.x_shift[k] = S.bn[7].shift;
    }
    if (heads_fuse) {
      const int l = heads[hk];
      w.fuse = 1; w.f_gamma = P(h, d.g_off); w.f_dcs = hcs; w.f_dco = 256 * hk;
      for (int k = 0; k < SS.n; ++k) {
        Slot& S = *SS.s[k];
        w.f_y[k] = S.Y[l]; w.f_dout[k] = S.gP; w.f_scale[k] = S.bn[l].scale; w.f_shift[k] = S.bn[l].shift; w.f_mean[k] = S.bn[l].mean;
        w.f_invstd[k] = S.bn[l].invstd; w.f_k12[k] = S.bn[l].k12;
      }
    }
    const double flops = 2.0 * SS.n * ncells * 128.0 * 256 * 9;
    ProfScope ps(h, SSP_PROF_CONV3X3_WGRAD, st, flops, 2.0 * SS.n * ncells * (128.0 + 256.0), flops, SSP_PROF_K_WGRAD_BF16);
    CHK(launch_wgrad_bf16(w, h->partial, h->partial_floats, h->n_cu, st, h->rq_bf16));
  }
  {
    float* gQ[2] = {nullptr, nullptr};
    for (int k = 0; k < SS.n; ++k) gQ[k] = SS.s[k]->gQ;
    CHK(tap_copy(h, SS, L_PA, 1, gQ, ncells * hcs, st, sizeof(uint16_t)));
  }
  ConvBCall c;
  c.nviews = SS.n; c.N = N; c.H = Hc; c.W = Wc; c.ks = 3; c.in_mode = 0;
  c.in_cs = hcs; c.in_co = 0; c.cin = hcs; c.wpk = reinterpret_cast<const uint16_t*>(h->wpk_heads_bwd);
  c.out_cs = 128; c.out_co = 0; c.cout = 128;
  for (int k = 0; k < SS.n; ++k) { c.in[k] = SS.s[k]->gQ; c.out[k] = SS.s[k]->gP; }
  const bool bnr = bf16_bnr_env() && launch_conv_bf16_is_ws(c);
  if (bnr) set_bnr_bf16(c, SS, 7, false);
  const double flops = 2.0 * SS.n * ncells * (double)hcs * 128 * 9;
  ProfScope ps(h, SSP_PROF_CONV3X3_DGRAD, st, flops, 2.0 * SS.n * ncells * (hcs + 128.0), flops, SSP_PROF_K_CONV_BF16);
  CHK(launch_conv_bf16(c, h->n_cu, st));
  if (bnr) h->bsums_fused[7] = true;
  for (int hk = 0; hk < h->nheads; ++hk)
    h->tap_route[heads[hk]] |= (unsigned)(launch_conv_bf16_is_ws(c) ? TAP_DG_BF16_WS : TAP_DG_BF16) << TAP_DG_SHIFT;
  return 0;
}

enum { EARLY_SPLIT_LAYER = 2 };
static int run_backward_impl(ssp_handle* h, const SlotSet& SS, const float* const* dsemi, const float* const* draw_desc,
                             float* const* dsout, hipStream_t st, int part);
static int run_backward(ssp_handle* h, const SlotSet& SS, const float* const* dsemi, const float* const* draw_desc,
                        float* const* dsout, hipStream_t st, int part = 0) {
  if (part != 2) h->bf16_fuse_apply = bf16_fuse_apply_env();
  CHK(run_backward_impl(h, SS, dsemi, draw_desc, dsout, st, part));
  return det_fold(h->buf.grads_dev, st);
}
static int run_backward_impl(ssp_handle* h, const SlotSet& SS, const float* const* dsemi, const float* const* draw_desc,
                             float* const* dsout, hipStream_t st, int part) {
  Slot& S0 = *SS.s[0];
  if (h->rq_bf16 != nullptr) { h->rq_bf16->J.n = 0; h->rq_bf16->used = 0; }
  if (part != 2) { h->tail.g1_blocks = 0; h->tail.cs_views = 0; }
  if (!h->packed_bwd || h->packed_algo != g_conv_algo)
    return fail(-3, "backward: the packed weight images do not belong to this pass (%s) - run the forward of the step again",
                !h->packed_bwd ? "the last forward packed no data-gradient weights" : "the conv algorithm changed since the forward");
  for (int k = 0; k < SS.n; ++k)
    if (SS.s[k]->N <= 0) return fail(-3, "backward: the slot holds no forward");
  const int N = S0.N, H = S0.H, W = S0.W, Hc = H / 8, Wc = W / 8;
  const int hcs = 256 * h->nheads;
  const bool has_semi = dsemi[0] != nullptr, has_desc = draw_desc[0] != nullptr;
  const bool has_sem = dsout[0] != nullptr && h->nheads == 3;
  float *gP[2] = {nullptr, nullptr}, *gQ[2] = {nullptr, nullptr};
  for (int k = 0; k < SS.n; ++k) { gP[k] = SS.s[k]->gP; gQ[k] = SS.s[k]->gQ; }
  auto encoder = [&](int l_hi, int l_lo) -> int {
    if (bf16_path()) {
      CHK(encoder_backward_bf16(h, SS, l_hi, l_lo, st));
      return flush_wgrad_reduce(h, st);
    }
    for (int l = l_hi; l >= l_lo; --l) {
      int lh, lw; layer_res(l, H, W, lh, lw);
      const bool pool_after = (l == 1 || l == 3 || l == 5);
      const int C = h->L[l].cout;
      CHK(tap_copy(h, SS, l, 0, gP, (size_t)N * (pool_after ? (lh / 2) * (lw / 2) : lh * lw) * C, st));
      CHK(bn_layer_backward(h, SS, l, gP, C, 0, true, pool_after, gQ, C, 0, N, lh, lw, st));
      if (l > 0) CHK(conv_layer_backward(h, SS, l, l - 1, gQ, C, 0, gP, h->L[l].cin, 0, N, lh, lw, layer_in_mode(l), st));
      if (l > 0) CHK(tap_copy(h, SS, l, 1, gQ, (size_t)N * lh * lw * C, st));
    }
    return flush_wgrad_reduce(h, st);
  };
  if (part == 2) return encoder(EARLY_SPLIT_LAYER - 1, 0);
  for (int l = 0; l < 16; ++l) h->bsums_fused[l] = h->apply_fused[l] = false;
  for (int l = 0; l < 16; ++l) h->tap_route[l] = 0;
  for (int k = 0; k < SS.n; ++k) {
    Slot& S = *SS.s[k];
    if (S.bsums_dirty) {
      for (int l = 0; l < h->nlayers; ++l)
        CHK(dev_zero(S.bn[l].bsums, 2 * (size_t)h->L[l].cout * NREP * sizeof(double), st));
    }
    S.bsums_dirty = true;
    if (!has_semi || !has_desc || (h->nheads == 3 && !has_sem))
      CHK(dev_zero(S.gP, (size_t)N * Hc * Wc * hcs * sizeof(float), st));
  }
  if (bf16_path()) {
    CHK(heads_backward_bf16(h, SS, dsemi, draw_desc, dsout, st));
    if (part == 1) return encoder(7, EARLY_SPLIT_LAYER);
    return encoder(7, 0);
  }
  float* dact[2] = {gP[0], gP[1]};
  const bool grouped = (!has_semi || h->pk_g1[L_PB]) && (!has_desc || h->pk_g1[L_DB]) && (!has_sem || h->pk_g1[L_SOUT]);
  const size_t ncells_all = (size_t)N * Hc * Wc;
  float* gQd[2] = {gQ[0], gQ[1]};
  if (grouped && has_semi)
    for (int k = 0; k < SS.n; ++k) gQd[k] = gQ[k] + ncells_all * 80;
  G1Layer Lg[3];
  int ng = 0;
  const bool gw = grouped && g1w_fits(256, 65, (long)ncells_all, hcs, std::max(256, h->sout_cs));
  G1WLayer Lw[3];
  int nw = 0;
  auto add_wgrad = [&](int l, float* const* dy, int dy_cs) {
    const LayerDesc& d = h->L[l];
    const int src = l - 1;
    G1WLayer& y = Lw[nw++];
    y.x_cs = S0.y_cs[src]; y.x_co = S0.y_co[src]; y.dy_cs = dy_cs; y.dy_co = 0; y.dw = Gd(h, d.w_off); y.N = d.cout;
    for (int k = 0; k < SS.n; ++k) {
      Slot& S = *SS.s[k];
      y.x[k] = S.Y[src]; y.scale[k] = S.bn[src].scale; y.shift[k] = S.bn[src].shift; y.dy[k] = dy[k];
    }
  };
  auto add_dgrad = [&](int l, float* const* dy, int dy_cs, int co) {
    const LayerDesc& d = h->L[l];
    const int src = l - 1;
    G1Layer& y = Lg[ng++];
    y.in_cs = dy_cs; y.in_co = 0; y.out_cs = hcs; y.out_co = co; y.wpk = h->wpk_g1_bwd[l]; y.K = d.cout; y.N = d.cin;
    const bool bnr = h->L[src].bn && S0.y_cs[src] == hcs && S0.y_co[src] == co && h->L[src].cout == d.cin;
    for (int k = 0; k < SS.n; ++k) {
      Slot& S = *SS.s[k];
      y.in[k] = dy[k]; y.out[k] = dact[k];
      if (bnr) {
        y.bnr_y[k] = S.Y[src]; y.bnr_scale[k] = S.bn[src].scale; y.bnr_shift[k] = S.bn[src].shift; y.bnr_mean[k] = S.bn[src].mean;
        y.bnr_invstd[k] = S.bn[src].invstd; y.stats[k] = S.bn[src].bsums;
      }
    }
    if (bnr) h->bsums_fused[src] = true;
  };
  BnPlainJob job_pb, job_db;
  const bool pair = has_semi && has_desc && grouped && gw && SS.n == 2;
  if (pair) {
    CHK(bn_layer_backward(h, SS, L_PB, dsemi, 80, 0, false, false, gQ, 80, 0, N, Hc, Wc, st, nullptr, &job_pb));
    CHK(bn_layer_backward(h, SS, L_DB, draw_desc, 256, 0, false, false, gQd, 256, 0, N, Hc, Wc, st, nullptr, &job_db));
    if (!job_pb.filled || !job_db.filled) return fail(-3, "pointwise heads: BatchNorm backward not in the plain form");
    CHK(launch_bn_bwd_pair(job_pb, job_db, SS.n, st));
  }
  if (has_semi) {
    if (!pair) CHK(bn_layer_backward(h, SS, L_PB, dsemi, 80, 0, false, false, gQ, 80, 0, N, Hc, Wc, st));
    CHK(conv_layer_backward(h, SS, L_PB, L_PA, gQ, 80, 0, dact, hcs, 0, N, Hc, Wc, 1, st, grouped, gw));
    CHK(tap_copy(h, SS, L_PB, 1, gQ, ncells_all * 80, st));
    if (grouped) add_dgrad(L_PB, gQ, 80, 0);
    if (gw) add_wgrad(L_PB, gQ, 80);
  }
  if (has_desc) {
    if (!pair) CHK(bn_layer_backward(h, SS, L_DB, draw_desc, 256, 0, false, false, gQd, 256, 0, N, Hc, Wc, st));
    CHK(conv_layer_backward(h, SS, L_DB, L_DA, gQd, 256, 0, dact, hcs, 256, N, Hc, Wc, 1, st, grouped, gw));
    CHK(tap_copy(h, SS, L_DB, 1, gQd, ncells_all * 256, st));
    if (grouped) add_dgrad(L_DB, gQd, 256, 256);
    if (gw) add_wgrad(L_DB, gQd, 256);
  }
  if (has_sem) {
    const LayerDesc& d = h->L[L_SOUT];
    const int ncells = N * Hc * Wc;
    if (h->sout_cs > 256) return fail(-3, "segmentation head: more than 256 classes are not supported by colsum_kernel");
    TailJobs& T = h->tail;
    T.cs_m[0] = dsout[0]; T.cs_m[1] = dsout[SS.n - 1]; T.cs_out = Gd(h, d.b_off);
    T.cs_rows = ncells; T.cs_C = d.cout; T.cs_cs = h->sout_cs; T.cs_blocks = cdiv(ncells, COLSUM_ROWS); T.cs_views = SS.n;
    CHK(conv_layer_backward(h, SS, L_SOUT, L_DS, dsout, h->sout_cs, 0, dact, hcs, 512, N, Hc, Wc, 1, st, grouped, gw));
    if (grouped) add_dgrad(L_SOUT, dsout, h->sout_cs, 512);
    if (gw) add_wgrad(L_SOUT, dsout, h->sout_cs);
  }
  if (gw && nw > 0) CHK(launch_g1_wgrad(Lw, nw, SS.n, (long)ncells_all, h->g1_partial, h->g1_partial_slabs, h->n_cu, st, &h->tail));
  if (grouped && ng > 0) CHK(launch_g1(Lg, ng, SS.n, (long)ncells_all, 0, h->n_cu, st));
  for (int l : {L_PB, L_DB, L_SOUT}) {
    const bool ran = l == L_PB ? has_semi : l == L_DB ? has_desc : has_sem;
    if (ran && gw) h->tap_route[l] |= TAP_WG_GROUPED << TAP_WG_SHIFT;
    if (ran && grouped) h->tap_route[l] |= TAP_DG_GROUPED << TAP_DG_SHIFT;
  }
  {
    const int heads[3] = {L_PA, L_DA, L_DS};
    CHK(tap_copy(h, SS, L_PA, 0, gP, ncells_all * hcs, st));
    BnSumsQueue sums_queue;
    for (int hk = 0; hk < h->nheads; ++hk)
      CHK(bn_layer_backward(h, SS, heads[hk], gP, hcs, 256 * hk, true, false, gQ, hcs, 256 * hk, N, Hc, Wc, st, &sums_queue));
    CHK(flush_bn_sums(sums_queue, SS.n, st));
    for (int hk = 0; hk < h->nheads; ++hk) {
      const LayerDesc& d = h->L[heads[hk]];
      WgradCall w;
      w.in = S0.Y[7]; w.in_cs = 128; w.in_co = 0; w.cin = 128; w.dout = gQ[0]; w.dout_cs = hcs; w.dout_co = 256 * hk;
      w.cout = 256; w.in_scale = S0.bn[7].scale; w.in_shift = S0.bn[7].shift; w.dw = Gd(h, d.w_off);
      w.N = N; w.H = Hc; w.W = Wc; w.ks = 3; w.in_mode = 1;
      if (SS.n == 2) {
        Slot& B = *SS.s[1];
        w.nprob = 2; w.in2 = B.Y[7]; w.dout2 = gQ[1]; w.in_scale2 = B.bn[7].scale; w.in_shift2 = B.bn[7].shift;
      }
      if (h->apply_fused[heads[hk]]) {
        h->apply_fused[heads[hk]] = false;
        h->tap_route[heads[hk]] |= TAP_APPLY_FUSED;
        w.fuse_apply = true; w.fuse_pool = false;
        w.dout_cs = hcs; w.dout_co = 0; w.f_gamma = P(h, d.g_off); w.f_ycs = hcs;
        for (int k = 0; k < SS.n; ++k) {
          Slot& S = *SS.s[k];
          (k ? w.dout2 : w.dout) = gP[k] + 256 * hk;
          w.f_y[k] = S.Y[heads[hk]] + S.y_co[heads[hk]]; w.f_dy[k] = gQ[k] + 256 * hk;
          w.f_scale[k] = S.bn[heads[hk]].scale; w.f_shift[k] = S.bn[heads[hk]].shift; w.f_mean[k] = S.bn[heads[hk]].mean;
          w.f_invstd[k] = S.bn[heads[hk]].invstd; w.f_k12[k] = S.bn[heads[hk]].k12;
        }
        if (h->sums_lazy[heads[hk]]) {
          h->sums_lazy[heads[hk]] = false;
          h->tap_route[heads[hk]] |= TAP_SUMS_LAZY;
          w.f_lazy = 1; w.f_count = (double)N * Hc * Wc; w.f_dgamma = Gd(h, d.g_off); w.f_dbeta = Gd(h, d.be_off); w.f_dbias = Gd(h, d.b_off);
          for (int k = 0; k < SS.n; ++k) w.f_bsums[k] = SS.s[k]->bn[heads[hk]].bsums;
        }
      }
      CHK(launch_wgrad(h, w, h->partial, h->partial_floats, h->n_cu, st));
      h->tap_route[heads[hk]] |= (unsigned)h->tap_wk << TAP_WG_SHIFT;
    }
    CHK(tap_copy(h, SS, L_PA, 1, gQ, ncells_all * hcs, st));
    ConvCall c;
    c.in = gQ[0]; c.in_cs = hcs; c.in_co = 0; c.cin = hcs; c.wpk = h->wpk_heads_bwd; c.bias = nullptr; c.wino = wino_ok(3, hcs);
    c.allow_w4 = false;
    c.out = gP[0]; c.out_cs = 128; c.out_co = 0; c.cout = 128; c.in_scale = nullptr; c.in_shift = nullptr;
    c.stats = nullptr; c.N = N; c.H = Hc; c.W = Wc; c.ks = 3; c.in_mode = 0; c.nchunks = 16 * h->nheads; c.ncob = 2;
    if (SS.n == 2) { c.nprob = 2; c.in2 = gQ[1]; c.out2 = gP[1]; }
    setup_bnr(h, SS, 7, false, c);
    CHK(launch_conv(h, c, st, SSP_PROF_CONV3X3_DGRAD));
    for (int hk = 0; hk < h->nheads; ++hk) h->tap_route[heads[hk]] |= (unsigned)h->tap_dk << TAP_DG_SHIFT;
  }
  if (part == 1) return encoder(7, EARLY_SPLIT_LAYER);
  return encoder(7, 0);
}

extern "C" {

int ssp_forward(ssp_handle* h, int slot, const float* x_dev, int n, int height, int width, int train, float* semi_dev,
                float* desc_dev, float* sem_dev, void* stream) {
  if (!h || !h->bound) return fail(-1, "handle not bound");
  if (slot < 0 || slot > 1) return fail(-1, "slot must be 0 or 1");
  AlgoScope algo(h);
  if (n < 1 || n > h->cfg.max_batch || height > h->cfg.height || width > h->cfg.width || height % 8 || width % 8)
    return fail(-1, "forward shape [%d,1,%d,%d] exceeds the configured maximum or is not a multiple of 8", n, height, width);
  if ((size_t)height * width != (size_t)h->cfg.height * h->cfg.width && (size_t)n * height * width > (size_t)h->cfg.max_batch * h->cfg.height * h->cfg.width)
    return fail(-1, "forward shape too large");
  hipStream_t st = (hipStream_t)stream;
  {
    SlotSet SS{1, {&h->slot[slot], nullptr}};
    const float* xs[2] = {x_dev, nullptr};
    CHK(run_forward(h, SS, xs, n, height, width, train, h->buf.grads_dev != nullptr, st));
  }
  Slot& S = h->slot[slot];
  const int HW = (height / 8) * (width / 8);
  if (semi_dev) {
    const long tot = (long)n * 65 * HW;
    hipLaunchKernelGGL(nhwc_affine_to_nchw_kernel, dim3(cdiv(tot, 256)), dim3(256), 0, st, S.Y[L_PB], S.bn[L_PB].scale,
                       S.bn[L_PB].shift, semi_dev, n, HW, 65, 80, 0);
  }
  if (desc_dev) {
    const long tot = (long)n * 256 * HW;
    hipLaunchKernelGGL(nhwc_affine_to_nchw_kernel, dim3(cdiv(tot, 256)), dim3(256), 0, st, S.desc, (const float*)nullptr,
                       (const float*)nullptr, desc_dev, n, HW, 256, 256, 0);
  }
  if (sem_dev) {
    if (h->nheads != 3) return fail(-1, "sem output requested from a model without a segmentation head");
    const long tot = (long)n * h->cfg.n_classes * height * width;
    hipLaunchKernelGGL(sem_upsample_nchw_kernel, dim3(cdiv(tot, 256)), dim3(256), 0, st, S.Y[L_SOUT], sem_dev, n,
                       height / 8, width / 8, height, width, h->cfg.n_classes, h->sout_cs);
  }
  HIPCHK(hipGetLastError());
  return 0;
}

int ssp_backward(ssp_handle* h, int slot, const float* dsemi_dev, const float* ddesc_dev, const float* dsem_dev,
                 void* stream) {
  if (!h || !h->bound || !h->buf.grads_dev) return fail(-1, "handle not bound with a gradient buffer");
  if (slot < 0 || slot > 1) return fail(-1, "slot must be 0 or 1");
  AlgoScope algo(h);
  hipStream_t st = (hipStream_t)stream;
  Slot& S = h->slot[slot];
  const int N = S.N, Hc = S.H / 8, Wc = S.W / 8, HW = Hc * Wc, ncells = N * HW;
  const float *ds = nullptr, *dd = nullptr, *dso = nullptr;
  if (dsemi_dev) {
    const long tot = (long)N * 65 * HW;
    hipLaunchKernelGGL(nchw_to_nhwc_kernel, dim3(cdiv(tot, 256)), dim3(256), 0, st, dsemi_dev, S.dsemi, N, HW, 65, 80, 0);
    ds = S.dsemi;
  }
  if (ddesc_dev) {
    const long tot = (long)N * 256 * HW;
    hipLaunchKernelGGL(nchw_to_nhwc_kernel, dim3(cdiv(tot, 256)), dim3(256), 0, st, ddesc_dev, S.ddesc, N, HW, 256, 256, 0);
    hipLaunchKernelGGL(desc_normalize_bwd_kernel, dim3(cdiv(ncells, 4)), dim3(256), 0, st, S.desc, S.inv_norm, S.ddesc, ncells);
    dd = S.ddesc;
  }
  if (dsem_dev) {
    if (h->nheads != 3) return fail(-1, "dsem given for a model without a segmentation head");
    CHK(dev_zero(S.dsout, (size_t)ncells * h->sout_cs * sizeof(float), st));
    const long tot = (long)N * h->cfg.n_classes * Hc * Wc;
    hipLaunchKernelGGL(sem_upsample_bwd_nchw_kernel, dim3(cdiv(tot, 256)), dim3(256), 0, st, dsem_dev, S.dsout, N, Hc, Wc,
                       S.H, S.W, h->cfg.n_classes, h->sout_cs);
    dso = S.dsout;
  }
  HIPCHK(hipGetLastError());
  SlotSet SS{1, {&h->slot[slot], nullptr}};
  const float* dss[2] = {ds, nullptr};
  const float* dds[2] = {dd, nullptr};
  float* dsos[2] = {const_cast<float*>(dso), nullptr};
  return run_backward(h, SS, dss, dds, dsos, st);
}

int ssp_adam_step(ssp_handle* h, float lr, int step, void* stream) {
  if (!h || !h->bound || !h->buf.grads_dev || !h->buf.adam_m_dev || !h->buf.adam_v_dev)
    return fail(-1, "handle not bound with gradient and Adam state buffers");
  if (step < 1) return fail(-1, "Adam step index starts at 1");
  const long n = (long)h->n_params + 3;
  const AdamScalars a = adam_scalars(lr, step);
  hipLaunchKernelGGL(adam_kernel, dim3(cdiv(n, 256)), dim3(256), 0, (hipStream_t)stream, h->buf.params_dev,
                     h->buf.grads_dev, h->buf.adam_m_dev, h->buf.adam_v_dev, n, a.step_size, a.bc2_sqrt);
  HIPCHK(hipGetLastError());
  return 0;
}

}

constexpr int SEM_XC_WGS_PER_CU = 2;
static int launch_sem_ce(int algo, bool train, const float* sout, const int64_t* labels, float* dsout, StepAccum* acc, int view, int B,
                         int Hc, int Wc, int H, int W, int C, int cs, hipStream_t st, const float* sout1 = nullptr,
                         const int64_t* labels1 = nullptr, float* dsout1 = nullptr) {
  const bool xc_ok = H == 8 * Hc && W == 8 * Wc && C <= 16 * SEMX_NB;
  if (algo == 2 && !xc_ok) return fail(-1, "sem_ce: the (x, class) form needs H = 8 Hc, W = 8 Wc and <= %d classes", 16 * SEMX_NB);
  if (C > SEM_MAX_C) return fail(-1, "sem_ce: at most %d classes", SEM_MAX_C);
  const bool xc = algo == 2 || (algo == 0 && xc_ok && sem_xc_env() != 0);
  const long ntile = (long)B * (Hc + 1) * (Wc + 1);
  const int nviews = sout1 != nullptr ? 2 : 1;
  if (xc) {
    const SemXcGeom geom = sem_xc_geom(B, Hc, Wc, SEM_XC_WGS_PER_CU * device_cu_count());
    const int grid = B * geom.row_groups * geom.x_splits * nviews;
#define SSP_SEM_XC(MODE, NB) \
  hipLaunchKernelGGL((sem_ce_xc_kernel<MODE, NB>), dim3(grid), dim3(256), 0, st, sout, labels, dsout, acc, view, B, Hc, Wc, C, cs, geom, sout1, \
                     labels1, dsout1)
    if (train) { if (C <= 48) SSP_SEM_XC(3, 3); else if (C <= 96) SSP_SEM_XC(3, 6); else SSP_SEM_XC(3, 9); }
    else { if (C <= 48) SSP_SEM_XC(1, 3); else if (C <= 96) SSP_SEM_XC(1, 6); else SSP_SEM_XC(1, 9); }
#undef SSP_SEM_XC
  } else {
    const int grid = (int)std::min<long>((ntile + 3) / 4, 4096);
    for (int v = 0; v < nviews; ++v) {
      const float* so = v ? sout1 : sout; const int64_t* la = v ? labels1 : labels; float* ds = v ? dsout1 : dsout;
      if (train) hipLaunchKernelGGL((sem_ce_kernel<3>), dim3(grid), dim3(256), 0, st, so, la, ds, acc, view + v, B, Hc, Wc, H, W, C, cs);
      else hipLaunchKernelGGL((sem_ce_kernel<1>), dim3(grid), dim3(256), 0, st, so, la, ds, acc, view + v, B, Hc, Wc, H, W, C, cs);
    }
  }
  return 0;
}

static int launch_desc_csr(const int32_t* match_a, const int32_t* match_b, int32_t* off, int32_t* em, float* ew, int B, int Hc, int Wc,
                           int n_match, int dflags, hipStream_t st) {
  const size_t lds = desc_csr_lds_bytes(Hc * Wc, n_match);
  constexpr size_t lds_max = 128 * 1024;
  if (lds > lds_max) return fail(-1, "desc_csr: %d cells x %d matches need %zu B of LDS (> %zu)", Hc * Wc, n_match, lds, lds_max);
  return launch_lds<desc_csr_kernel>(lds_max, dim3(B, 2), dim3(DESC_CSR_THREADS), lds, st, match_a, match_b, off, em, ew, Hc, Wc, n_match, dflags);
}

static int pair_step_impl(ssp_handle* h, const ssp_pair_inputs* in, float* scalars_dev, int phase, hipStream_t st_in) {
  void* stream = st_in;
  if (!h || !h->bound) return fail(-1, "handle not bound");
  if (!in || !scalars_dev) return fail(-1, "null argument");
  if (phase < 0 || phase > 2) return fail(-1, "pair-step phase must be 0, 1 or 2");
  AlgoScope algo(h);
  const int nv = in && in->warped_image_dev ? 2 : 1;
  if (phase == 2) {
    if (!in->train) return 0;
    SlotSet SS2{nv, {&h->slot[0], nv == 2 ? &h->slot[1] : nullptr}};
    const float* none[2] = {nullptr, nullptr};
    float* nonef[2] = {nullptr, nullptr};
    return run_backward(h, SS2, none, none, nonef, (hipStream_t)stream, 2);
  }
  if (in->train && !h->buf.grads_dev) return fail(-1, "train step needs a gradient buffer");
  const int B = in->batch, H = h->cfg.height, W = h->cfg.width, Hc = H / 8, Wc = W / 8;
  if (B < 1 || B > h->cfg.max_batch || B > SSP_MAX_PAIRS)
    return fail(-1, "pair-step batch %d out of range (1..min(max_batch, %d))", B, SSP_MAX_PAIRS);
  const bool semantic = h->nheads == 3;
  if (semantic && (!in->semantic_dev || (nv == 2 && !in->warped_semantic_dev))) return fail(-1, "semantic labels required for the ssmall model");
  const bool use_desc = in->lambda_loss > 0.f;
  if (use_desc && nv == 1) return fail(-1, "need a pair of images: lambda_loss > 0 with warped_image_dev == NULL");
  if (!in->image_dev || !in->labels_dev || !in->valid_mask_dev || (nv == 2 && (!in->warped_labels_dev || !in->warped_valid_mask_dev)))
    return fail(-1, "pair step: image / labels / valid mask pointers of every view are required");
  const bool dense = use_desc && in->dense_loss != 0;
  if (dense && !h->dense_coef) return fail(-1, "dense descriptor loss needs a handle created with ssp_config.dense_loss = 1");
  if (use_desc && !dense && (!in->match_a_dev || !in->match_b_dev || !in->nonmatch_b_dev))
    return fail(-1, "sparse-loss indices required (call ssp_sample_indices or pass the reference's indices)");
  hipStream_t st = (hipStream_t)stream;
  const float* eta = h->buf.params_dev + h->n_params;
  const int ncells = B * Hc * Wc;
  hipLaunchKernelGGL(step_begin_kernel, dim3(1), dim3(64), 0, st, h->accum, eta, in->multi_task, in->lambda_loss,
                     in->lamda_d, (int)semantic, B);
  SlotSet SS{nv, {&h->slot[0], nv == 2 ? &h->slot[1] : nullptr}};
  const float* masks[2] = {in->valid_mask_dev, in->warped_valid_mask_dev};
  const int64_t* sems[2] = {in->semantic_dev, in->warped_semantic_dev};
  const bool zero_dsout = semantic && in->train;
  const bool gather = h->desc_gather && in->train && use_desc && !dense;
  const int dflags = (in->sparse_method != 0 ? DESC_METHOD_1D : 0) | (in->sparse_dist != 0 ? DESC_EUCLIDEAN : 0);
  {
    CHK(ensure_aux_stream(h));
    hipStream_t se = h->aux2_stream;
    HIPCHK(hipEventRecord(h->ev_early_fork, st));
    HIPCHK(hipStreamWaitEvent(se, h->ev_early_fork, 0));
    if (gather)
      CHK(launch_desc_csr(in->match_a_dev, in->match_b_dev, h->csr_off, h->csr_match, h->csr_weight, B, Hc, Wc, h->cfg.n_match, dflags, se));
    hipLaunchKernelGGL(cell_mask_kernel, dim3(std::min(cdiv(ncells, 4), 512), nv), dim3(256), 0, se, masks[0], h->slot[0].cellmask,
                       &h->accum->mask_cnt[0], B, H, W, masks[nv - 1], h->slot[nv - 1].cellmask, &h->accum->mask_cnt[nv - 1]);
    if (semantic)
      hipLaunchKernelGGL(sem_count_kernel, dim3(512, nv), dim3(256), 0, se, sems[0], sems[1], (long)B * H * W, h->cfg.n_classes, h->accum,
                         zero_dsout ? h->slot[0].dsout : (float*)nullptr, zero_dsout && nv == 2 ? h->slot[1].dsout : (float*)nullptr,
                         (long)ncells * h->sout_cs);
    HIPCHK(hipGetLastError());
    HIPCHK(hipEventRecord(h->ev_early_join, se));
  }
  {
    const float* xs[2] = {in->image_dev, in->warped_image_dev};
    CHK(run_forward(h, SS, xs, B, H, W, 1, in->train != 0, st, false, in->train && use_desc && !dense));
  }
  HIPCHK(hipStreamWaitEvent(st, h->ev_early_join, 0));
  hipStream_t sd = st;
  const bool forked = use_desc && !dense;
  SideFork loss_fork;
  if (forked) {
    CHK(ensure_aux_stream(h));
    sd = h->aux_stream;
    CHK(loss_fork.fork(st, sd, h->ev_fork, h->ev_join));
  }
  if (dense) {
    Slot &A = h->slot[0], &Bs = h->slot[1];
    const int pc = Hc * Wc;
    DenseArgs da;
    da.da = A.desc; da.db = Bs.desc; da.hn = in->homographies_dev; da.valid = Bs.cellmask;
    da.coef = in->train ? h->dense_coef : nullptr; da.acc = h->accum; da.B = B; da.Hc = Hc; da.Wc = Wc;
    da.lamda_d = in->dense_lamda_d; da.dist = in->descriptor_dist; da.multi_task = in->multi_task;
    hipLaunchKernelGGL(dense_dots_kernel, dim3(cdiv(pc, 64), cdiv(pc, 64), B), dim3(256), 0, sd, da);
    if (in->train) {
      hipLaunchKernelGGL((dense_grad_kernel<false>), dim3(4, cdiv(pc, 64), B), dim3(256), 0, sd, h->dense_coef, Bs.desc,
                         A.ddesc, pc);
      hipLaunchKernelGGL((dense_grad_kernel<true>), dim3(4, cdiv(pc, 64), B), dim3(256), 0, sd, h->dense_coef, A.desc,
                         Bs.ddesc, pc);
      hipLaunchKernelGGL(desc_normalize_bwd_kernel, dim3(cdiv(ncells, 4), 2), dim3(256), 0, sd, A.desc, A.inv_norm, A.ddesc, ncells,
                         Bs.desc, Bs.inv_norm, Bs.ddesc);
    }
    HIPCHK(hipGetLastError());
  } else if (use_desc) {
    Slot &A = h->slot[0], &Bs = h->slot[1];
    const bool euc = (dflags & DESC_EUCLIDEAN) != 0;
    const dim3 dgrid(desc_grid(B, h->cfg.n_match));
#define SSP_DESC(KERNEL, ...)                                                                 \
    {                                                                                         \
      if (euc) hipLaunchKernelGGL((KERNEL<true>), dgrid, dim3(256), 0, sd, __VA_ARGS__);      \
      else hipLaunchKernelGGL((KERNEL<false>), dgrid, dim3(256), 0, sd, __VA_ARGS__);         \
    }
#define SSP_DESC_MATCH(BWD, ...)                                                                        \
    {                                                                                                   \
      if (euc) hipLaunchKernelGGL((desc_match_kernel<BWD, true>), dgrid, dim3(256), 0, sd, __VA_ARGS__); \
      else hipLaunchKernelGGL((desc_match_kernel<BWD, false>), dgrid, dim3(256), 0, sd, __VA_ARGS__);   \
    }
    if (!in->train)
      SSP_DESC_MATCH(false, A.desc, Bs.desc, in->match_a_dev, in->match_b_dev, (float*)nullptr, (float*)nullptr, h->accum, B, Hc, Wc,
                     h->cfg.n_match, dflags)
    SSP_DESC(desc_nonmatch_fwd_kernel, A.desc, Bs.desc, in->match_a_dev, in->nonmatch_b_dev, in->train ? h->dots : (float*)nullptr, h->accum,
             B, Hc, Wc, h->cfg.n_match, h->cfg.n_non, dflags)
    if (in->train) {
      if (gather) {
        if (euc) hipLaunchKernelGGL((desc_match_kernel<true, true, true>), dgrid, dim3(256), 0, sd, A.desc, Bs.desc, in->match_a_dev, in->match_b_dev,
                                    (float*)nullptr, (float*)nullptr, h->accum, B, Hc, Wc, h->cfg.n_match, dflags, h->g_rows);
        else hipLaunchKernelGGL((desc_match_kernel<true, false, true>), dgrid, dim3(256), 0, sd, A.desc, Bs.desc, in->match_a_dev, in->match_b_dev,
                                (float*)nullptr, (float*)nullptr, h->accum, B, Hc, Wc, h->cfg.n_match, dflags, h->g_rows);
      } else
        SSP_DESC_MATCH(true, A.desc, Bs.desc, in->match_a_dev, in->match_b_dev, A.ddesc, Bs.ddesc, h->accum, B, Hc, Wc, h->cfg.n_match, dflags)
      SSP_DESC(desc_nonmatch_bwd_kernel, A.desc, Bs.desc, in->match_a_dev, in->nonmatch_b_dev, h->dots, A.ddesc, Bs.ddesc, h->accum, B, Hc, Wc,
               h->cfg.n_match, h->cfg.n_non, dflags)
#undef SSP_DESC
#undef SSP_DESC_MATCH
      CHK(det_fold(A.ddesc, sd));
      CHK(det_fold(Bs.ddesc, sd));
      const DescGather dg = {gather ? h->csr_off : nullptr, h->csr_match, h->csr_weight, h->g_rows, Hc * Wc, h->cfg.n_match};
      hipLaunchKernelGGL(desc_normalize_bwd_kernel, dim3(cdiv(ncells, 4), 2), dim3(256), 0, sd, A.desc, A.inv_norm, A.ddesc, ncells,
                         Bs.desc, Bs.inv_norm, Bs.ddesc, dg);
    }
    HIPCHK(hipGetLastError());
  }
  const float* labels[2] = {in->labels_dev, in->warped_labels_dev};
  {
    Slot &S = h->slot[0], &T = h->slot[nv - 1];
    hipLaunchKernelGGL(detector_loss_kernel, dim3(std::min(cdiv(ncells, 4), 1024), nv), dim3(256), 0, st, S.Y[L_PB], S.bn[L_PB].scale,
                       S.bn[L_PB].shift, labels[0], S.cellmask, in->train ? S.dsemi : nullptr, h->accum, 0, B, H, W, 80,
                       T.Y[L_PB], T.bn[L_PB].scale, T.bn[L_PB].shift, labels[nv - 1], T.cellmask, in->train ? T.dsemi : nullptr);
  }
  HIPCHK(hipGetLastError());
  if (semantic) {
    Slot &S = h->slot[0], &T = h->slot[nv - 1];
    CHK(launch_sem_ce(0, in->train != 0, S.Y[L_SOUT], sems[0], in->train ? S.dsout : nullptr, h->accum, 0, B, Hc, Wc, H, W, h->cfg.n_classes,
                      h->sout_cs, st, nv == 2 ? T.Y[L_SOUT] : nullptr, nv == 2 ? sems[1] : nullptr, nv == 2 && in->train ? T.dsout : nullptr));
    if (in->train)
      for (int v = 0; v < nv; ++v) CHK(det_fold(h->slot[v].dsout, st));
    HIPCHK(hipGetLastError());
  }
  CHK(loss_fork.join());
  hipLaunchKernelGGL(step_end_kernel, dim3(1), dim3(64), 0, st, h->accum, eta,
                     in->train ? h->buf.grads_dev + h->n_params : (float*)nullptr, scalars_dev, B, h->cfg.n_match,
                     in->multi_task, in->lambda_loss, in->lamda_d, (int)semantic, in->train, (int)dense, Hc * Wc, nv);
  HIPCHK(hipGetLastError());
  if (in->train) {
    const float* dss[2] = {h->slot[0].dsemi, nv == 2 ? h->slot[1].dsemi : nullptr};
    const float* dds[2] = {use_desc ? h->slot[0].ddesc : nullptr, use_desc ? h->slot[1].ddesc : nullptr};
    float* dsos[2] = {semantic ? h->slot[0].dsout : nullptr, semantic && nv == 2 ? h->slot[1].dsout : nullptr};
    CHK(run_backward(h, SS, dss, dds, dsos, st, phase));
  }
  return 0;
}

static int sample_indices_impl(ssp_handle* h, const float* homographies_dev, const float* hcell_dev, int batch, uint64_t seed,
                               const uint64_t* seed_dev, int32_t* match_a_dev, int32_t* match_b_dev, int32_t* nonmatch_b_dev,
                               hipStream_t st) {
  if (!h) return fail(-1, "null handle");
  if (!homographies_dev && !hcell_dev) return fail(-1, "sample_indices: homographies required");
  if (batch < 1 || batch > SSP_MAX_PAIRS) return fail(-1, "batch out of range (1..%d)", SSP_MAX_PAIRS);
  const int Hc = h->cfg.height / 8, Wc = h->cfg.width / 8;
  if (Hc * Wc > SAMPLER_MAX_CELLS) return fail(-1, "sampler supports at most %d cells", SAMPLER_MAX_CELLS);
  if (h->cfg.n_match > SAMPLER_MAX_CELLS) return fail(-1, "n_match too large for the device sampler");
  int cap = 2048;
  while (cap < Hc * Wc || cap < h->cfg.n_match) cap <<= 1;
  CHK(launch_lds<sample_matches_kernel>(SAMPLER_MAX_CELLS * 12, dim3(batch), dim3(1024), (size_t)cap * 12, st, homographies_dev, hcell_dev,
                                        seed, seed_dev, match_a_dev, match_b_dev, Hc, Wc, h->cfg.n_match, cap));
  const long tot = (long)batch * h->cfg.n_match * h->cfg.n_non;
  hipLaunchKernelGGL(sample_nonmatches_kernel, dim3(cdiv(tot, 256)), dim3(256), 0, st, seed, seed_dev, nonmatch_b_dev, tot, Hc,
                     Wc);
  HIPCHK(hipGetLastError());
  return 0;
}

__global__ void set_seed_kernel(uint64_t* dst, uint64_t v) { *dst = v; }

extern "C" {

int ssp_adam_step_scaled(ssp_handle* h, float lr, int step, float grad_scale, void* stream) {
  if (!h || !h->bound || !h->buf.grads_dev || !h->buf.adam_m_dev || !h->buf.adam_v_dev)
    return fail(-1, "handle not bound with gradient and Adam state buffers");
  if (step < 1) return fail(-1, "Adam step index starts at 1");
  const long n = (long)h->n_params + 3;
  const AdamScalars a = adam_scalars(lr, step);
  hipLaunchKernelGGL(adam_scaled_kernel, dim3(cdiv(n, 256)), dim3(256), 0, (hipStream_t)stream, h->buf.params_dev,
                     h->buf.grads_dev, h->buf.adam_m_dev, h->buf.adam_v_dev, n, a.step_size, a.bc2_sqrt, grad_scale);
  HIPCHK(hipGetLastError());
  return 0;
}

int ssp_handle_set_conv_algo(ssp_handle* h, int algo) {
  if (!h) return fail(-1, "null handle");
  CHK(check_conv_algo(algo));
  h->conv_algo = algo;
  return 0;
}

int ssp_pair_step(ssp_handle* h, const ssp_pair_inputs* in, float* scalars_dev, void* stream) {
  return pair_step_impl(h, in, scalars_dev, 0, (hipStream_t)stream);
}

int ssp_pair_step_phase(ssp_handle* h, const ssp_pair_inputs* in, float* scalars_dev, int phase, void* stream) {
  return pair_step_impl(h, in, scalars_dev, phase, (hipStream_t)stream);
}

size_t ssp_grad_early_offset(const ssp_handle* h) { return h ? h->L[EARLY_SPLIT_LAYER].w_off : 0; }

int ssp_pair_step_graph(ssp_handle* h, const ssp_pair_inputs* in, float* scalars_dev, int phase, int sample_indices,
                        void* stream) {
  if (!h || !h->bound) return fail(-1, "handle not bound");
  if (!in || !scalars_dev) return fail(-1, "null argument");
  hipStream_t st = (hipStream_t)stream;
  if (st == nullptr) return fail(-1, "ssp_pair_step_graph needs a non-default stream (stream capture)");
  if (h->tap_arena != nullptr) return fail(-1, "ssp_pair_step_graph: backward taps are on (ssp_debug_backward_taps); they need the eager step");
  std::vector<unsigned char> key(sizeof(ssp_pair_inputs) + sizeof(void*) + 5 * sizeof(int));
  {
    ssp_pair_inputs k;
    memcpy(&k, in, sizeof(k));
    k.seed = 0;
    memcpy(key.data(), &k, sizeof(k));
    memcpy(key.data() + sizeof(k), &scalars_dev, sizeof(void*));
    const int extra[5] = {phase, sample_indices, h->conv_algo, bf16_fuse_apply_env() ? 1 : 0,
                          h->desc_gather ? 1 : 0};
    memcpy(key.data() + sizeof(k) + sizeof(void*), extra, sizeof(extra));
  }
  hipGraphExec_t exec = nullptr;
  for (auto& g : h->graphs)
    if (g.key == key) { exec = g.exec; break; }
  if (exec == nullptr) {
    if (h->prof_family != 0) return fail(-1, "ssp_pair_step_graph: disable ssp_profile_enable before capturing");
    if (h->graphs.size() >= 16) {
      (void)hipGraphExecDestroy(h->graphs.front().exec);
      h->graphs.erase(h->graphs.begin());
    }
    hipGraph_t graph = nullptr;
    HIPCHK(hipStreamBeginCapture(st, hipStreamCaptureModeThreadLocal));
    int rc = 0;
    if (sample_indices && phase != 2) {
      if (!in->match_a_dev || !in->match_b_dev || !in->nonmatch_b_dev) rc = fail(-1, "graph step: index buffers required");
      else rc = sample_indices_impl(h, in->homographies_dev, in->cell_homographies_dev, in->batch, 0, h->graph_seed,
                                    const_cast<int32_t*>(in->match_a_dev),
                                    const_cast<int32_t*>(in->match_b_dev), const_cast<int32_t*>(in->nonmatch_b_dev), st);
    }
    if (rc == 0) rc = pair_step_impl(h, in, scalars_dev, phase, st);
    const hipError_t ce = hipStreamEndCapture(st, &graph);
    if (rc != 0) { if (graph) (void)hipGraphDestroy(graph); return rc; }
    if (ce != hipSuccess) return fail(-2, "hipStreamEndCapture failed: %s", hipGetErrorString(ce));
    const hipError_t ie = hipGraphInstantiate(&exec, graph, nullptr, nullptr, 0);
    (void)hipGraphDestroy(graph);
    if (ie != hipSuccess) return fail(-2, "hipGraphInstantiate failed: %s", hipGetErrorString(ie));
    h->graphs.push_back({key, exec});
  }
  if (sample_indices && phase != 2) {
    hipLaunchKernelGGL(set_seed_kernel, dim3(1), dim3(1), 0, st, h->graph_seed, in->seed);
    HIPCHK(hipGetLastError());
  }
  HIPCHK(hipGraphLaunch(exec, st));
  return 0;
}

int ssp_sample_indices(ssp_handle* h, const float* homographies_dev, int batch, uint64_t seed, int32_t* match_a_dev,
                       int32_t* match_b_dev, int32_t* nonmatch_b_dev, void* stream) {
  return sample_indices_impl(h, homographies_dev, nullptr, batch, seed, nullptr, match_a_dev, match_b_dev, nonmatch_b_dev,
                             (hipStream_t)stream);
}

int ssp_sample_indices_cell(ssp_handle* h, const float* cell_homographies_dev, int batch, uint64_t seed, int32_t* match_a_dev,
                            int32_t* match_b_dev, int32_t* nonmatch_b_dev, void* stream) {
  if (!cell_homographies_dev) return fail(-1, "sample_indices_cell: cell homographies required");
  return sample_indices_impl(h, nullptr, cell_homographies_dev, batch, seed, nullptr, match_a_dev, match_b_dev, nonmatch_b_dev,
                             (hipStream_t)stream);
}

int ssp_op_conv(const float* in_dev, const float* w_oihw_dev, const float* bias_dev, float* out_dev, int n, int hh, int w,
                int cin, int cout, int ksize, int in_mode, const float* in_scale_dev, const float* in_shift_dev,
                double* stats_dev, int transpose_flip, void* workspace_dev, size_t workspace_bytes, void* stream) {
  AlgoScope algo(nullptr);
  if (ksize == 1 && in_mode != 2 && g1_enabled() && g1_fits(cin, cout, (long)n * hh * w, cin, cout, 1)) {
    const size_t img = g1_image_floats(cin, cout) * sizeof(float);
    if (workspace_bytes >= img) {
      hipStream_t st = (hipStream_t)stream;
      float* wpk = reinterpret_cast<float*>(workspace_dev);
      G1PackJobs G;
      G.n = 0;
      int nb = 0;
      g1_add_pack(G, nb, w_oihw_dev, wpk, transpose_flip ? cin : cout, transpose_flip ? cout : cin, transpose_flip ? 1 : 0);
      hipLaunchKernelGGL(pack_g1_kernel, dim3(nb), dim3(256), 0, st, G);
      HIPCHK(hipGetLastError());
      G1Layer y;
      y.in[0] = in_dev; y.in_cs = cin; y.in_co = 0; y.out[0] = out_dev; y.out_cs = cout; y.out_co = 0; y.wpk = wpk; y.bias = bias_dev;
      y.scale[0] = in_scale_dev; y.shift[0] = in_shift_dev; y.stats[0] = stats_dev; y.K = cin; y.N = cout;
      return launch_g1(&y, 1, 1, (long)n * hh * w, in_mode, device_cu_count(), st);
    }
  }
  const bool wino = wino_ok(ksize, cin) && in_mode != 2;
  const int nchunks = cdiv(cin, CK), ncob = cdiv(cout, NB);
  const size_t need = (size_t)ncob * nchunks * pk_taps(ksize) * CK * NB * sizeof(float);
  if (workspace_bytes < need) return fail(-4, "ssp_op_conv workspace too small (%zu < %zu)", workspace_bytes, need);
  if (bf16_path() && ksize == 3 && cin % CK == 0 && in_mode != 2)
    return fail(-3, "ssp_op_conv: conv algorithm 12 has no fp32 3x3 kernel for Cin %% 16 == 0 (use ssp_op_conv_bf16 or another algorithm)");
  hipStream_t st = (hipStream_t)stream;
  float* wpk = reinterpret_cast<float*>(workspace_dev);
  const bool w4 = wino && ksize == 3 && w4_eligible(nullptr, 1, n, hh, w, cin, cout);
  if (!transpose_flip) CHK(launch_pack(w_oihw_dev, wpk, cout, cin, ksize, 0, wino, st, w4));
  else CHK(launch_pack(w_oihw_dev, wpk, cin, cout, ksize, 1, wino, st, w4));
  ConvCall c;
// ... 1441 lines not shown
  return rc;
}

int ssp_set_conv_algo(int algo) {
  CHK(check_conv_algo(algo));
  g_default_conv_algo = algo;
  return 0;
}

int ssp_debug_occupancy(int which) {
  int n = -1;
  hipError_t e = hipErrorInvalidValue;
  if (which == 0) {
    auto k = conv_wino_p2_kernel<1, true>;
    (void)hipFuncSetAttribute(reinterpret_cast<const void*>(k), hipFuncAttributeMaxDynamicSharedMemorySize, P2_LDS_BYTES);
    e = hipOccupancyMaxActiveBlocksPerMultiprocessor(&n, k, P2_THREADS, P2_LDS_BYTES);
  } else if (which == 1) {
    auto k = conv_wino_pipe_kernel<1, true>;
    (void)hipFuncSetAttribute(reinterpret_cast<const void*>(k), hipFuncAttributeMaxDynamicSharedMemorySize, PIPE_LDS_BYTES);
    e = hipOccupancyMaxActiveBlocksPerMultiprocessor(&n, k, WINO_THREADS, PIPE_LDS_BYTES);
  } else if (which == 2) {
    auto k = wgrad_wino_kernel<1, true>;
    (void)hipFuncSetAttribute(reinterpret_cast<const void*>(k), hipFuncAttributeMaxDynamicSharedMemorySize, WgradWinoGeom<true>::LDS_BYTES);
    e = hipOccupancyMaxActiveBlocksPerMultiprocessor(&n, k, 512, WgradWinoGeom<true>::LDS_BYTES);
  }
  else if (which == 3) {
    auto k = conv_bf16_kernel<3, 1, false, false>;
    (void)hipFuncSetAttribute(reinterpret_cast<const void*>(k), hipFuncAttributeMaxDynamicSharedMemorySize, ConvBGeom<3>::LDS_BYTES);
    e = hipOccupancyMaxActiveBlocksPerMultiprocessor(&n, k, 256, ConvBGeom<3>::LDS_BYTES);
  } else if (which == 4) {
    auto k = wgrad_bf16_kernel<3, 1, false>;
    (void)hipFuncSetAttribute(reinterpret_cast<const void*>(k), hipFuncAttributeMaxDynamicSharedMemorySize, WgradBGeom<3>::LDS_BYTES);
    e = hipOccupancyMaxActiveBlocksPerMultiprocessor(&n, k, 256, WgradBGeom<3>::LDS_BYTES);
  }
  if (e != hipSuccess) return fail(-2, "occupancy query failed: %s", hipGetErrorString(e));
  return n;
}

int ssp_debug_conv_knobs(int ablate, int grid) {
  g_dbg_ablate = ablate; g_dbg_grid = grid;
  return 0;
}

int ssp_debug_backward_taps(ssp_handle* h, float* arena_dev, size_t arena_floats, unsigned layer_mask) {
  if (!h) return fail(-1, "bad argument");
  h->tap_arena = nullptr; h->tap_mask = 0;
  if (arena_dev == nullptr) return 0;
  const unsigned mask = layer_mask & 0xffffu;
  const size_t need = tap_offset(h, mask, 2, 0, 0);
  if (arena_floats < need) return fail(-1, "backward-tap arena holds %zu floats, the layer mask needs %zu", arena_floats, need);
  h->tap_arena = arena_dev; h->tap_mask = mask;
  return 0;
}
size_t ssp_debug_backward_tap_floats(const ssp_handle* h, unsigned layer_mask) {
  return h ? tap_offset(h, layer_mask & 0xffffu, 2, 0, 0) : 0;
}
int ssp_debug_backward_tap(ssp_handle* h, int slot, int layer, int which, size_t* offset, size_t* nfloats, unsigned* route) {
  if (!h || slot < 0 || slot > 1 || layer < 0 || layer >= 16 || which < 0 || which > 1) return fail(-1, "bad argument");
  const size_t n = h->tap_arena != nullptr && (h->tap_mask >> layer & 1) ? tap_floats(h, layer, which) : 0;
  if (offset) *offset = n ? tap_offset(h, h->tap_mask, slot, layer, which) : 0;
  if (nfloats) *nfloats = n;
  if (route) *route = h->tap_route[layer];
  return 0;
}

int ssp_debug_buffer(ssp_handle* h, int slot, const char* name, float** ptr, size_t* nfloats) {
  if (!h || !h->bound || !name || !ptr) return fail(-1, "bad argument");
  Slot& S = h->slot[slot & 1];
  const size_t cells = (size_t)h->cfg.max_batch * (h->cfg.height / 8) * (h->cfg.width / 8);
  std::string n(name);
  float* p = nullptr; size_t cnt = 0;
  if (n == "gP") { p = S.gP; cnt = (size_t)h->cfg.max_batch * h->cfg.height * h->cfg.width * 64; }
  else if (n == "gQ") { p = S.gQ; cnt = (size_t)h->cfg.max_batch * h->cfg.height * h->cfg.width * 64; }
  else if (n == "dsemi") { p = S.dsemi; cnt = cells * 80; }
  else if (n == "ddesc") { p = S.ddesc; cnt = cells * 256; }
  else if (n == "desc") { p = S.desc; cnt = cells * 256; }
  else if (n == "dsout") { p = S.dsout; cnt = cells * h->sout_cs; }
  else if (n[0] == 'Y') { int l = atoi(name + 1); if (l < 0 || l >= h->nlayers) return fail(-1, "bad layer"); p = S.Y[l]; cnt = 0; }
  else if (n[0] == 'A') { int l = atoi(name + 1); if (l < 0 || l >= 8 || !S.Apool[l]) return fail(-1, "no pooled copy of that layer"); p = S.Apool[l]; cnt = 0; }
  else if (n.rfind("scale", 0) == 0) { int l = atoi(name + 5); p = S.bn[l].scale; cnt = h->L[l].cout; }
  else if (n.rfind("shift", 0) == 0) { int l = atoi(name + 5); p = S.bn[l].shift; cnt = h->L[l].cout; }
  else if (n.rfind("mean", 0) == 0) { int l = atoi(name + 4); p = S.bn[l].mean; cnt = h->L[l].cout; }
  else if (n.rfind("invstd", 0) == 0) { int l = atoi(name + 6); p = S.bn[l].invstd; cnt = h->L[l].cout; }
  else return fail(-1, "unknown buffer %s", name);
  *ptr = p;
  if (nfloats) *nfloats = cnt;
  return 0;
}

int ssp_op_dense_loss(const float* desc_a_nhwc_dev, const float* desc_b_nhwc_dev, const float* homographies_dev,
                      const float* valid_dev, int b, int hc, int wc, float lamda_d, float descriptor_dist, int multi_task,
                      float scale, void* scratch_dev, size_t scratch_bytes, float* out3_dev, float* dda_dev,
                      float* ddb_dev, void* stream) {
  const int pc = hc * wc;
  const bool grad = dda_dev != nullptr && ddb_dev != nullptr;
  const size_t need = align_up(sizeof(StepAccum), 256) + (grad ? (size_t)b * pc * pc * sizeof(float) : 0);
  if (scratch_bytes < need) return fail(-4, "ssp_op_dense_loss scratch too small (%zu < %zu)", scratch_bytes, need);
  hipStream_t st = (hipStream_t)stream;
  StepAccum* acc = reinterpret_cast<StepAccum*>(scratch_dev);
  float* coef = grad ? reinterpret_cast<float*>(reinterpret_cast<char*>(scratch_dev) + align_up(sizeof(StepAccum), 256)) : nullptr;
  hipLaunchKernelGGL(dense_op_prep_kernel, dim3(1), dim3(256), 0, st, acc, valid_dev, b * pc, scale);
  DenseArgs da;
  da.da = desc_a_nhwc_dev; da.db = desc_b_nhwc_dev; da.hn = homographies_dev; da.valid = valid_dev; da.coef = coef;
  da.acc = acc; da.B = b; da.Hc = hc; da.Wc = wc; da.lamda_d = lamda_d; da.dist = descriptor_dist; da.multi_task = multi_task;
  hipLaunchKernelGGL(dense_dots_kernel, dim3(cdiv(pc, 64), cdiv(pc, 64), b), dim3(256), 0, st, da);
  if (grad) {
    hipLaunchKernelGGL((dense_grad_kernel<false>), dim3(4, cdiv(pc, 64), b), dim3(256), 0, st, coef, desc_b_nhwc_dev, dda_dev, pc);
    hipLaunchKernelGGL((dense_grad_kernel<true>), dim3(4, cdiv(pc, 64), b), dim3(256), 0, st, coef, desc_a_nhwc_dev, ddb_dev, pc);
  }
  hipLaunchKernelGGL(dense_op_finish_kernel, dim3(1), dim3(1), 0, st, acc, out3_dev, b, pc);
  HIPCHK(hipGetLastError());
  return 0;
}

int ssp_op_sparse_loss(const float* desc_a_nhwc_dev, const float* desc_b_nhwc_dev, const int32_t* match_a_dev,
                       const int32_t* match_b_dev, const int32_t* nonmatch_b_dev, int b, int hc, int wc, int n_match,
                       int n_non, int method, int dist, float coef_pos, float coef_neg, float* dd_a_nhwc_dev, float* dd_b_nhwc_dev,
                       float* out2_dev, void* stream) {
  return ssp_op_sparse_loss_path(desc_a_nhwc_dev, desc_b_nhwc_dev, match_a_dev, match_b_dev, nonmatch_b_dev, b, hc, wc, n_match, n_non, method,
                                 dist, coef_pos, coef_neg, dd_a_nhwc_dev, dd_b_nhwc_dev, out2_dev, -1, nullptr, nullptr, nullptr, stream);
}

int ssp_op_sparse_loss_path(const float* desc_a_nhwc_dev, const float* desc_b_nhwc_dev, const int32_t* match_a_dev,
                            const int32_t* match_b_dev, const int32_t* nonmatch_b_dev, int b, int hc, int wc, int n_match,
                            int n_non, int method, int dist, float coef_pos, float coef_neg, float* dd_a_nhwc_dev, float* dd_b_nhwc_dev,
                            float* out2_dev, int gather, int32_t* csr_off_dev, int32_t* csr_match_dev, float* csr_weight_dev,
                            void* stream) {
  if (b < 1 || b > SSP_MAX_PAIRS) return fail(-1, "batch out of range (1..%d)", SSP_MAX_PAIRS);
  if ((dd_a_nhwc_dev == nullptr) != (dd_b_nhwc_dev == nullptr)) return fail(-1, "sparse_loss: both gradient pointers or none");
  hipStream_t st = (hipStream_t)stream;
  const bool grad = dd_a_nhwc_dev != nullptr;
  const int dflags = (method != 0 ? DESC_METHOD_1D : 0) | (dist != 0 ? DESC_EUCLIDEAN : 0);
  StepAccum* acc = nullptr;
  float* dots = nullptr;
  HIPCHK(hipMallocAsync((void**)&acc, sizeof(StepAccum), st));
  HIPCHK(hipMemsetAsync(acc, 0, sizeof(StepAccum), st));
  hipLaunchKernelGGL(sparse_op_prep_kernel, dim3(1), dim3(1), 0, st, acc, coef_pos, coef_neg);
  const size_t ncell_floats = (size_t)b * hc * wc * 256;
  const bool euc = (dflags & DESC_EUCLIDEAN) != 0;
  const dim3 dgrid(desc_grid(b, n_match));
  const bool use_gather = grad && (gather < 0 ? desc_gather_env() : gather != 0);
  const bool own_csr = csr_off_dev == nullptr || csr_match_dev == nullptr || csr_weight_dev == nullptr;
  if (!own_csr && !use_gather) return fail(-1, "sparse_loss: the corner lists exist on the gather path with gradients only");
  int32_t *csr_off = csr_off_dev, *csr_match = csr_match_dev;
  float *csr_weight = csr_weight_dev, *g_rows = nullptr;
  if (grad) {
    HIPCHK(hipMallocAsync((void**)&dots, (size_t)b * n_match * n_non * sizeof(float), st));
    CHK(dev_zero(dd_a_nhwc_dev, ncell_floats * sizeof(float), st));
    CHK(dev_zero(dd_b_nhwc_dev, ncell_floats * sizeof(float), st));
  }
  if (use_gather) {
    if (own_csr) {
      HIPCHK(hipMallocAsync((void**)&csr_off, (size_t)b * 2 * ((size_t)hc * wc + 1) * sizeof(int32_t), st));
      HIPCHK(hipMallocAsync((void**)&csr_match, (size_t)b * 2 * 4 * n_match * sizeof(int32_t), st));
      HIPCHK(hipMallocAsync((void**)&csr_weight, (size_t)b * 2 * 4 * n_match * sizeof(float), st));
    }
    HIPCHK(hipMallocAsync((void**)&g_rows, (size_t)b * n_match * 2 * 256 * sizeof(float), st));
    CHK(launch_desc_csr(match_a_dev, match_b_dev, csr_off, csr_match, csr_weight, b, hc, wc, n_match, dflags, st));
  }
#define SSP_OPD(KERNEL, ...)                                                                  \
  {                                                                                           \
    if (euc) hipLaunchKernelGGL((KERNEL<true>), dgrid, dim3(256), 0, st, __VA_ARGS__);        \
    else hipLaunchKernelGGL((KERNEL<false>), dgrid, dim3(256), 0, st, __VA_ARGS__);           \
  }
  if (use_gather) {
    if (euc) hipLaunchKernelGGL((desc_match_kernel<true, true, true>), dgrid, dim3(256), 0, st, desc_a_nhwc_dev, desc_b_nhwc_dev, match_a_dev,
// ... 126 lines not shown
```

### semantic-superpoint_amd/lib.py

```python
import ctypes as C
import math
import os
from collections import OrderedDict

import numpy as np
import torch

from . import hipbuild as _build

ARCHS = {"SuperPointNet_gauss2": 0, "SuperPointNet_gauss2_ssmall": 1}
SCALAR_NAMES = ["loss", "loss_det", "loss_det_warp", "loss_desc", "loss_sem", "loss_sem_warp", "positive_dist",
                "negative_dist", "eta_det", "eta_desc", "eta_sem"]
N_SCALARS = 16
NREP = 32
SAMPLER_MAX_MATCHES = 8192
PROF = {"none": 0, "conv3x3_fwd": 1, "conv3x3_dgrad": 2, "conv3x3_wgrad": 3, "conv_big_fwd": 4, "conv3x3_all": 5,
        "conv3x3_every": 6}
PROF_KERNELS = ["conv_wino4_kernel", "conv_wino_pipe_kernel", "conv_wino_p2_kernel", "wgrad_wino_kernel", "wgrad_wino4_kernel",
                "other", "conv_bf16_kernel", "wgrad_bf16_kernel"]


class SspConfig(C.Structure):
    _fields_ = [("arch", C.c_int), ("n_classes", C.c_int), ("max_batch", C.c_int), ("height", C.c_int),
                ("width", C.c_int), ("n_match", C.c_int), ("n_non", C.c_int), ("dense_loss", C.c_int)]
# ... 116 lines not shown
        "ssp_op_sem_loss": ([vp, i, vp] + [i] * 5 + [vp, sz, vp, vp, vp], i),
        "ssp_op_sem_predict": ([vp, i, vp, i, i, i, i, vp, vp, vp], i),
        "ssp_sem_predict": ([vp, i, vp, vp, vp, vp], i),
        "ssp_op_warp_image": ([vp, vp, vp, i, i, i, i, vp], i),
        "ssp_op_erode": ([vp, vp, i, i, i, i, vp], i),
        "ssp_op_warp_labels": ([vp, vp, vp, i, i, i, vp], i),
        "ssp_op_warp_labels_px": ([vp, vp, vp, i, i, i, vp], i),
        "ssp_op_sample_homographies": ([u64, P(SspHomographyParams), i, vp, vp, vp], i),
        "ssp_op_warp_labels_full": ([vp] * 5 + [i, i, i, vp], i),
        "ssp_op_warp_labels_full_px": ([vp] * 5 + [i, i, i, vp], i),
        "ssp_op_label_quantize": ([vp, vp, sz, vp], i),
        "ssp_op_sem_finalize": ([vp, vp, vp, sz, i, vp], i),
        "ssp_op_photometric_draw": ([u64, P(SspPhotometricParams), i, i, i, vp, vp], i),
        "ssp_op_photometric_apply": ([vp, vp, vp, i, i, i, vp], i),
        "ssp_shapes_workspace_bytes": ([P(SspShapesParams), i], sz),
        "ssp_op_shapes_draw": ([u64, P(SspShapesParams), i, vp, vp], i),
        "ssp_op_shapes_render": ([vp, P(SspShapesParams), i] + [vp] * 5, i),
        "ssp_op_warp_points_scatter": ([vp, vp, vp, vp, i, i, i, i, vp], i),
        "ssp_export_workspace_bytes": ([P(SspExportParams)], sz),
        "ssp_export_max_points": ([P(SspExportParams)], i),
        "ssp_export_points": ([vp, P(SspExportParams), i] + [P(vp)] * 7 + [vp], i),
        "ssp_op_homoadapt_views": ([vp, vp, vp, vp, i, i, i, vp], i),
        "ssp_op_flatten_detection": ([vp, vp, vp, i, i, i, vp], i),
        "ssp_op_combine_heatmap": ([vp, vp, vp, vp, i, i, i, vp], i),
        "ssp_op_heatmap_points": ([vp, P(SspExportParams), vp, vp, vp, vp], i),
        "ssp_op_soft_argmax_points": ([vp, vp, vp, i, i, i, vp], i),
        "ssp_detector_heatmap": ([vp, i, vp, vp], i),
        "ssp_op_heatmap_nms": ([vp, P(SspExportParams), i] + [vp] * 5, i),
        "ssp_describe_workspace_bytes": ([P(SspExportParams), i], sz),
        "ssp_describe_points": ([vp, i, P(SspExportParams), i] + [vp] * 5, i),
        "ssp_op_sample_descriptors": ([vp, i, i, i, vp, vp, i, vp, vp], i),
        "ssp_match_workspace_bytes": ([i, i], sz),
        "ssp_match_two_way": ([vp, vp, vp, vp, i, i, i, f, vp, vp, vp, vp], i),
        "ssp_op_point_classes": ([vp] + [i] * 5 + [vp, i, vp, i, vp, vp], i),
        "ssp_point_classes": ([vp, i, i, vp, i, vp, i, vp, vp], i),
        "ssp_filter_workspace_bytes": ([i, i], sz),
        "ssp_op_filter_points": ([vp, vp, vp, vp, P(u32), i, i] + [vp] * 6, i),
        "ssp_match_two_way_classes": ([vp] * 6 + [i, i, i, f, vp, vp, vp, vp], i),
        "ssp_eval_repeatability": ([vp, vp, vp, vp, i, i, i, vp, vp, i, i, i, d, vp, vp], i),
        "ssp_eval_ransac_workspace_bytes": ([i, i], sz),
        "ssp_eval_ransac": ([vp, vp, i, i, i] + [vp] * 10, i),
        "ssp_epi_ransac_workspace_bytes": ([i, i], sz),
        "ssp_epi_ransac": ([vp, vp, i, i, i, i, vp, vp, vp, d, i] + [vp] * 8, i),
        "ssp_op_filter_matches": ([vp] * 5 + [i, i, i, vp, vp, vp], i),
        "ssp_pose_from_fundamental": ([vp] * 6 + [i, i, i, i, vp, vp, vp, i] + [vp] * 11, i),
        "ssp_pose_chain": ([vp] * 5 + [i] + [vp] * 7 + [i, i, vp, vp, i, vp], i),
        "ssp_landmark_workspace_bytes": ([i, i], sz),
        "ssp_map_window": ([vp, vp, i, vp, i, i, i, vp, vp], i),
        "ssp_op_triangulate_tracks": ([vp, vp, vp, i, vp, i, i, i, i, d, d] + [vp] * 6, i),
        "ssp_op_landmarks_select": ([vp] * 8 + [i, i, i, vp, vp, vp, vp], i),
        "ssp_pnp_workspace_bytes": ([i], sz),
        "ssp_op_landmark_matches": ([vp, vp, i, vp, vp, i, vp, i, i, vp, vp, vp], i),
        "ssp_pnp_ransac": ([vp, vp, i, i, vp, i, vp, d, i, i] + [vp] * 9, i),
        "ssp_pose_repair": ([vp, vp, vp, i, vp, vp, i, vp], i),
        "ssp_ba_workspace_bytes": ([i, i], sz),
        "ssp_bundle_adjust": ([vp, vp, vp, i, vp, i, i, i, vp, vp, i] + [vp] * 6, i),
        "ssp_ba_apply": ([vp, vp, i, i, i, vp, vp, i, vp], i),
        "ssp_world_insert_workspace_bytes": ([i], sz),
        "ssp_match_world_workspace_bytes": ([i, i], sz),
        "ssp_op_world_insert": ([vp, vp, i, vp, vp, i, vp] + [i] * 5 + [vp] * 11, i),
        "ssp_match_world": ([vp, vp, i, vp, vp, i, f, vp, vp, vp, vp], i),
        "ssp_op_world_correspondences": ([vp, vp, i, vp, vp, i, vp, i, vp, i, vp, vp, vp], i),
        "ssp_world_repair": ([vp] * 5 + [i, i, vp, vp], i),
        "ssp_pose_graph_workspace_bytes": ([i], sz),
        "ssp_op_loop_correspondences": ([vp, vp, vp, i, vp, vp, i, vp, i, vp, i, vp, vp, i, i, i, vp, vp, vp, vp], i),
        "ssp_loop_edge": ([vp] * 7 + [i, vp, i, vp, i, i, i, i, d, vp, vp, vp, vp], i),
        "ssp_pose_graph": ([vp, i, vp, vp, i, i] + [vp] * 6, i),
        "ssp_loop_apply": ([vp] * 5 + [i, vp, vp, i, vp, vp, vp, i, vp], i),
        "ssp_eval_pixel_homographies": ([vp, i, i, i, vp, vp, vp], i),
        "ssp_eval_accumulate": ([vp] * 6 + [i, vp, i, i, i, P(d), i64, vp, i64, vp, vp], i),
        "ssp_det_eval_workspace_bytes": ([P(SspDetEvalParams), i, i], sz),
        "ssp_op_det_tp_fp": ([vp, vp, i, P(SspDetEvalParams), i, vp, vp, i64, vp, vp], i),
        "ssp_op_det_tp_fp_points": ([vp, vp, i, vp, i, P(SspDetEvalParams), i, vp, vp, i64, vp, vp], i),
        "ssp_det_pr_curve_workspace_bytes": ([i64], sz),
        "ssp_op_det_pr_curve": ([vp, i64] + [vp] * 8, i),
        "ssp_track_workspace_bytes": ([i, i, i], sz),
        "ssp_op_track_update": ([vp] * 8 + [i, i, i] + [vp] * 6, i),
        "ssp_op_track_select": ([vp, vp, vp, vp, i, i, i, vp, vp, vp, vp], i),
        "ssp_op_track_points": ([vp, vp, vp, vp, i, i, i, i, vp, vp], i),
        "ssp_op_bn_bwd": ([vp] * 9 + [i] * 6 + [vp], i),
        "ssp_op_bn_bwd_strided": ([vp] * 9 + [i] * 7 + [vp], i),
        "ssp_set_conv_algo": ([i], i),
        "ssp_handle_set_conv_algo": ([vp, i], i),
        "ssp_debug_conv_knobs": ([i, i], i),
        "ssp_debug_occupancy": ([i], i),
        "ssp_debug_buffer": ([vp, i, C.c_char_p, P(vp), P(sz)], i),
        "ssp_debug_backward_taps": ([vp, vp, sz, u32], i),
        "ssp_debug_backward_tap_floats": ([vp, u32], sz),
        "ssp_debug_backward_tap": ([vp, i, i, i, P(sz), P(sz), P(u32)], i),
        "ssp_op_sparse_loss": ([vp] * 5 + [i] * 7 + [f, f, vp, vp, vp, vp], i),
        "ssp_op_sparse_loss_path": ([vp] * 5 + [i] * 7 + [f, f, vp, vp, vp, i, vp, vp, vp, vp], i),
        "ssp_op_dense_loss": ([vp, vp, vp, vp, i, i, i, f, f, i, f, vp, sz, vp, vp, vp, vp], i),
    }


SIGNATURES = _signatures()
EXPORTS = list(SIGNATURES)

MATCH_MAX_POINTS = 4096
TRACK_MAX_LENGTH = 16
TRACK_NO_SCORE = 9999.0
CLASS_NONE = 255
DET_EVAL_MAX_R2 = 64
DET_EVAL_STATE_WORDS = 80
DET_EVAL_OUTSIDE = 3
DET_EVAL_HIST = 8
DET_CURVE_TILE = 1024
EVAL_ACC_MAX_PAIRS = 128
EVAL_ROW_WORDS = 16
EVAL_STATE_WORDS = 16
POSE_ROW_WORDS = 16
POSE_STATE_WORDS = 16
POSE_FLAG_NO_POSE, POSE_FLAG_SCALE_CARRIED = 1, 2
CAM_WORDS = 20
LANDMARK_WORDS = 8
LANDMARK_OK, LANDMARK_FEW_VIEWS, LANDMARK_DEGENERATE, LANDMARK_BEHIND, LANDMARK_REPROJ = 0, 1, 2, 3, 4
CORR_WORDS = 8
POSE_FLAG_ABSOLUTE = 4
POSE_FLAG_ADJUSTED = 8
BA_INFO_WORDS = 8
BA_MAX_ITERATIONS = 16
BA_ADJUSTED, BA_NOTHING, BA_NO_STEP = 0, 1, 2


def load_library(path=None):
    global _lib
    if _lib is not None and path is None:
        return _lib
    path = path or os.environ.get("SSP_HIP_LIB")
    if path is None:
        path = _build.build_locked()
    if not os.path.exists(path):
        raise RuntimeError("libssp_hip.so not found at %s" % path)
    if os.environ.get("SSP_SKIP_ISA_VERIFY") != "1" and not _build.verified(path):
        try:
            _build.verify_and_stamp(path)
        except _build.MissingTool as e:
            raise RuntimeError("%s - cannot check the accumulation-register contract of %s; set SSP_SKIP_ISA_VERIFY=1 to load it "
                               "unchecked" % (e, path)) from e
        except OSError:
            _build.verify_binary(path)
    lib = C.CDLL(path)
    for name, (argtypes, restype) in SIGNATURES.items():
        try:
            fn = getattr(lib, name)
        except AttributeError:
            if os.environ.get("SSP_HIP_LIB") is None:
                raise
            continue
        fn.argtypes, fn.restype = argtypes, restype
    _lib = lib
    return lib


def set_deterministic(on=True):
    _check(load_library().ssp_set_deterministic(1 if on else 0))


def get_deterministic():
    return bool(load_library().ssp_get_deterministic())


def clock_probe(ms=5.0):
    import torch
    lib = load_library()
    if not hasattr(lib, "ssp_clock_probe"):
# ... 17 lines not shown


def _ptr(t):
    return None if t is None else C.c_void_p(t.data_ptr())


def _stream():
    return C.c_void_p(torch.cuda.current_stream().cuda_stream)


def _need_gpu(t, name):
    if not t.is_cuda:
        raise RuntimeError("%s must live on a HIP device: the MI355X path has no CPU fallback" % name)
    if not t.is_contiguous():
        raise RuntimeError("%s must be contiguous" % name)


def scaled_homographies(hn, height, width):
    h = hn.detach().to("cpu", torch.float32).reshape(-1, 3, 3)
    trans = torch.tensor([[2.0 / width, 0.0, -1.0], [0.0, 2.0 / height, -1.0], [0.0, 0.0, 1.0]])
    inv = torch.inverse(trans)
    return torch.stack([inv @ m @ trans for m in h]).contiguous()


_ENC = [("inc.conv.conv.0", "inc.conv.conv.1", 1, 64, 3), ("inc.conv.conv.3", "inc.conv.conv.4", 64, 64, 3),
        ("down1.mpconv.1.conv.0", "down1.mpconv.1.conv.1", 64, 64, 3),
        ("down1.mpconv.1.conv.3", "down1.mpconv.1.conv.4", 64, 64, 3),
        ("down2.mpconv.1.conv.0", "down2.mpconv.1.conv.1", 64, 128, 3),
        ("down2.mpconv.1.conv.3", "down2.mpconv.1.conv.4", 128, 128, 3),
        ("down3.mpconv.1.conv.0", "down3.mpconv.1.conv.1", 128, 128, 3),
        ("down3.mpconv.1.conv.3", "down3.mpconv.1.conv.4", 128, 128, 3)]
_HEADS = [("convPa", "bnPa", 128, 256, 3), ("convPb", "bnPb", 256, 65, 1), ("convDa", "bnDa", 128, 256, 3),
          ("convDb", "bnDb", 256, 256, 1)]


def layer_table(arch, n_classes=133):
    t = _ENC + _HEADS
    if arch == "SuperPointNet_gauss2_ssmall":
        t = t + [("convDS", "bnS1", 128, 256, 3), ("convSout", None, 256, n_classes, 1)]
    elif arch != "SuperPointNet_gauss2":
        raise KeyError(arch)
    return t


def param_layout(arch, n_classes=133):
    out, off = [], 0
    for conv, bn, cin, cout, k in layer_table(arch, n_classes):
        for key, shape in ((conv + ".weight", (cout, cin, k, k)), (conv + ".bias", (cout,))):
            out.append((key, shape, off))
            off += int(np.prod(shape))
        if bn is not None:
            for key in (bn + ".weight", bn + ".bias"):
                out.append((key, (cout,), off))
                off += cout
    return out, off


def bn_layout(arch, n_classes=133):
    out, off = [], 0
    for conv, bn, cin, cout, k in layer_table(arch, n_classes):
        if bn is not None:
            out.append((bn, cout, off))
            off += cout
    return out, off


class Engine:

    def __init__(self, arch, max_batch, height, width, device, n_classes=133, n_match=1000, n_non=100,
                 with_grad=True, dense_loss=False):
        self.lib = load_library()
        self.device = torch.device(device)
        if self.device.type != "cuda":
            raise RuntimeError("Engine needs a HIP device (got %s): no CPU fallback exists" % self.device)
        self.arch, self.n_classes = arch, n_classes
        self.max_batch, self.height, self.width = max_batch, height, width
        self.n_match, self.n_non = n_match, n_non
        self.dense_loss = bool(dense_loss)
        cfg = SspConfig(ARCHS[arch], n_classes, max_batch, height, width, n_match, n_non, int(self.dense_loss))
        h = C.c_void_p()
        with torch.cuda.device(self.device):
            _check(self.lib.ssp_create(C.byref(cfg), C.byref(h)))
        self.h = h
        self.layout, self.n_params = param_layout(arch, n_classes)
        self.bns, self.n_bn_ch = bn_layout(arch, n_classes)
        assert self.n_params == self.lib.ssp_param_count(h), "parameter layout mismatch with the library"
        assert self.n_bn_ch == self.lib.ssp_bn_channel_count(h)
        f32 = dict(dtype=torch.float32, device=self.device)
        self.params = torch.zeros(self.n_params + 3, **f32)
        self.params[self.n_params:] = torch.tensor([1.0, 2.0, 1.0])
        self.grads = torch.zeros(self.n_params + 3, **f32) if with_grad else None
        self.adam_m = torch.zeros(self.n_params + 3, **f32) if with_grad else None
        self.adam_v = torch.zeros(self.n_params + 3, **f32) if with_grad else None
        self.bn_running = torch.cat([torch.zeros(self.n_bn_ch, **f32), torch.ones(self.n_bn_ch, **f32)])
        self.nbt = torch.zeros(len(self.bns), dtype=torch.int64, device=self.device)
        self.ws_bytes = self.lib.ssp_workspace_bytes(h)
        self._tap_arena = None
        self.workspace = torch.empty(self.ws_bytes, dtype=torch.uint8, device=self.device)
        self.scalars = torch.zeros(N_SCALARS, **f32)
        self.adam_t = 0
        self.bind()

    def bind(self):
        b = SspBuffers(_ptr(self.params), _ptr(self.grads), _ptr(self.adam_m), _ptr(self.adam_v),
                       _ptr(self.bn_running), _ptr(self.nbt), _ptr(self.workspace), self.ws_bytes)
        with torch.cuda.device(self.device):
            _check(self.lib.ssp_bind(self.h, C.byref(b), _stream()))

    def __del__(self):
        try:
            if getattr(self, "h", None):
                self.lib.ssp_destroy(self.h)
                self.h = None
        except Exception:
            pass

    def load_state_dict(self, sd):
        for key, shape, off in self.layout:
            v = torch.as_tensor(np.asarray(sd[key]) if not torch.is_tensor(sd[key]) else sd[key])
            self.params[off:off + v.numel()] = v.reshape(-1).to(self.device, torch.float32)
        for i, (bn, c, off) in enumerate(self.bns):
            for j, name in enumerate(("running_mean", "running_var")):
                k = bn + "." + name
                if k in sd:
                    v = torch.as_tensor(np.asarray(sd[k]) if not torch.is_tensor(sd[k]) else sd[k])
                    self.bn_running[j * self.n_bn_ch + off:j * self.n_bn_ch + off + c] = v.to(self.device, torch.float32)
            k = bn + ".num_batches_tracked"
            if k in sd:
                self.nbt[i] = int(sd[k])

    def state_dict(self):
        out = OrderedDict()
        bn_iter = {bn: (i, c, off) for i, (bn, c, off) in enumerate(self.bns)}
        for key, shape, off in self.layout:
            n = int(np.prod(shape))
            out[key] = self.params[off:off + n].view(shape).clone()
            prefix = key.rsplit(".", 1)[0]
            if key.endswith(".bias") and prefix in bn_iter:
                i, c, boff = bn_iter[prefix]
                out[prefix + ".running_mean"] = self.bn_running[boff:boff + c].clone()
                out[prefix + ".running_var"] = self.bn_running[self.n_bn_ch + boff:self.n_bn_ch + boff + c].clone()
                out[prefix + ".num_batches_tracked"] = self.nbt[i].clone()
        return out

    def grad_dict(self):
        out = OrderedDict()
        for key, shape, off in self.layout:
            out[key] = self.grads[off:off + int(np.prod(shape))].view(shape)
        out["eta"] = self.grads[self.n_params:]
        return out

    @property
    def eta(self):
        return self.params[self.n_params:]

    def forward(self, x, slot=0, train=True, want=("semi", "desc")):
        _need_gpu(x, "x")
        n, c, hh, ww = x.shape
        assert c == 1 and x.dtype == torch.float32
        f32 = dict(dtype=torch.float32, device=self.device)
        out = {}
        semi = torch.empty(n, 65, hh // 8, ww // 8, **f32) if "semi" in want else None
        desc = torch.empty(n, 256, hh // 8, ww // 8, **f32) if "desc" in want else None
        sem = torch.empty(n, self.n_classes, hh, ww, **f32) if "sem" in want else None
        if not hasattr(self, "_x"):
            self._x = [None, None]
        self._x[slot] = x
        with torch.cuda.device(self.device):
            _check(self.lib.ssp_forward(self.h, slot, _ptr(x), n, hh, ww, int(bool(train)), _ptr(semi), _ptr(desc),
                                        _ptr(sem), _stream()))
        if semi is not None:
            out["semi"] = semi
        if desc is not None:
            out["desc"] = desc
        if sem is not None:
            out["sem"] = sem
        return out

    def backward(self, slot, dsemi=None, ddesc=None, dsem=None):
        for t, nm in ((dsemi, "dsemi"), (ddesc, "ddesc"), (dsem, "dsem")):
            if t is not None:
                _need_gpu(t, nm)
        with torch.cuda.device(self.device):
            _check(self.lib.ssp_backward(self.h, slot, _ptr(dsemi), _ptr(ddesc), _ptr(dsem), _stream()))

    def zero_grad(self):
        with torch.cuda.device(self.device):
            _check(self.lib.ssp_zero_grad(self.h, _stream()))

    def adam_step(self, lr, grad_scale=None):
        self.adam_t += 1
        with torch.cuda.device(self.device):
            if grad_scale is None:
                _check(self.lib.ssp_adam_step(self.h, float(lr), self.adam_t, _stream()))
            else:
                _check(self.lib.ssp_adam_step_scaled(self.h, float(lr), self.adam_t, float(grad_scale), _stream()))

    def set_conv_algo(self, algo):
        _check(self.lib.ssp_handle_set_conv_algo(self.h, int(algo)))

    @property
    def early_offset(self):
        return int(self.lib.ssp_grad_early_offset(self.h))

    def sample_indices(self, homographies, seed, cell_homographies=None):
        _need_gpu(homographies, "homographies")
        B = homographies.shape[0]
        i32 = dict(dtype=torch.int32, device=self.device)
        ma = torch.empty(B, self.n_match, **i32)
        mb = torch.empty(B, self.n_match, **i32)
        nm = torch.empty(B, self.n_match * self.n_non, **i32)
        with torch.cuda.device(self.device):
            if cell_homographies is not None:
                hc = cell_homographies.to(self.device, torch.float32).contiguous()
                assert tuple(hc.shape) == (B, 3, 3)
                self._keep_hc = hc
                _check(self.lib.ssp_sample_indices_cell(self.h, _ptr(hc), B, int(seed), _ptr(ma), _ptr(mb), _ptr(nm), _stream()))
            else:
                _check(self.lib.ssp_sample_indices(self.h, _ptr(homographies), B, int(seed), _ptr(ma), _ptr(mb), _ptr(nm),
                                                   _stream()))
        return ma, mb, nm

    def pair_step(self, sample, indices=None, seed=0, train=True, lambda_loss=1.0, lamda_d=1.0, multi_task=True,
                  gaussian=True, dense=None, phase=0, graph=False, sparse_method="2d", sparse_dist="cos"):
        img = sample["image"]
        B, c1, H, W = img.shape
        single = sample.get("warped_img") is None
        if single and lambda_loss > 0:
            raise AssertionError("need a pair of images")
        lab = sample["labels_2D_gaussian"] if gaussian else sample["labels_2D"]
        if single:
            imgw = labw = maskw = None
            req = [img, lab, sample["valid_mask"]]
        else:
            imgw, maskw = sample["warped_img"], sample["warped_valid_mask"]
            labw = sample["warped_labels_gaussian"] if gaussian else sample["warped_labels"]
            req = [img, imgw, lab, labw, sample["valid_mask"], maskw]
        for t in req:
            _need_gpu(t, "sample tensor")
            if t.dtype != torch.float32 or tuple(t.shape) != (B, 1, H, W):
                raise ValueError("pair-step image / label / mask tensors must be float32 [B,1,H,W] = %s, got %s %s"
                                 % ((B, 1, H, W), t.dtype, tuple(t.shape)))
        if (H, W) != (self.height, self.width) or B > self.max_batch:
            raise ValueError("pair step [%d,1,%d,%d] does not match the engine (%d x %dx%d)"
                             % (B, H, W, self.max_batch, self.height, self.width))
        Hm = None
        if not single:
            Hm = sample["homographies"].to(torch.float32)
            if not Hm.is_contiguous():
                Hm = Hm.contiguous()
            _need_gpu(Hm, "homographies")
            if tuple(Hm.shape) != (B, 3, 3):
                raise ValueError("homographies must be [B,3,3]")
        if dense is not None and not self.dense_loss:
            raise RuntimeError("create the Engine with dense_loss=True to use the dense descriptor loss")
        sample_in_graph = False
        if lambda_loss > 0 and indices is None and dense is None:
            if graph:
                if getattr(self, "_graph_idx", None) is None or self._graph_idx[0].shape[0] != B:
                    i32 = dict(dtype=torch.int32, device=self.device)
                    self._graph_idx = (torch.zeros(B, self.n_match, **i32), torch.zeros(B, self.n_match, **i32),
                                       torch.zeros(B, self.n_match * self.n_non, **i32))
                indices = self._graph_idx
                sample_in_graph = True
            elif phase != 2:
                indices = self._last_idx = self.sample_indices(Hm, seed, sample.get("cell_homographies"))
            else:
                indices = self._last_idx
        if indices is not None:
            ma, mb, nm = indices
            for t, shp in ((ma, (B, self.n_match)), (mb, (B, self.n_match)), (nm, (B, self.n_match * self.n_non))):
                _need_gpu(t, "sparse-loss indices")
                if t.dtype != torch.int32 or tuple(t.shape) != shp:
                    raise ValueError("sparse-loss indices must be int32 %s, got %s %s" % (shp, t.dtype, tuple(t.shape)))
        else:
            ma = mb = nm = None
        sem = semw = None
        if self.arch.endswith("ssmall"):
            sem, semw = sample.get("semantic"), (None if single else sample.get("warped_sem"))
            for t in ((sem,) if single else (sem, semw)):
                if t is None:
                    raise KeyError("the ssmall model needs sample['semantic'] and sample['warped_sem']")
# ... 2080 lines not shown
```

Measured before the change: 2460.

## Fold head BatchNorm backward sums into loss and descriptor-normalize kernels

The per-channel BatchNorm backward reductions (sum of dy and sum of dy times x-hat) for the two pointwise heads are now accumulated inside the detector loss kernel and the descriptor normalize-backward kernel, which already produce those gradients. The separate pass-1 BN backward sums launch for the pair is then skipped. This avoids rereading the head activations and gradients in an extra kernel. In exchange the fused kernels do extra loads, shared-memory reductions and double atomics, and the descriptor kernel becomes grid-strided with a capped grid. The fold is on by default for fp32 pair training.

Result: no change. 2477, median of 6 (+0.7%).

```diff
diff --git a/include/ssp_hip.h b/include/ssp_hip.h
--- a/include/ssp_hip.h
+++ b/include/ssp_hip.h
@@ -439,6 +439,8 @@
 
 int ssp_set_conv_algo(int algo);
 int ssp_handle_set_conv_algo(ssp_handle* h, int algo);
+int ssp_handle_set_head_bn_fold(ssp_handle* h, int value);
+int ssp_handle_get_head_bn_fold(const ssp_handle* h);
 
 int ssp_debug_conv_knobs(int ablate, int grid);
 int ssp_debug_occupancy(int which);
diff --git a/semantic-superpoint_amd/csrc/bn_kernels.hip.h b/semantic-superpoint_amd/csrc/bn_kernels.hip.h
--- a/semantic-superpoint_amd/csrc/bn_kernels.hip.h
+++ b/semantic-superpoint_amd/csrc/bn_kernels.hip.h
@@ -298,6 +298,14 @@
   double count;
 };
 
+struct HeadBnSums {
+  const float* y;
+  const float* mean;
+  const float* invstd;
+  double* sums;
+  int y_cs, y_co;
+};
+
 template <bool RELU, bool POOL, bool APPLY, typename T = float>
 __global__ __launch_bounds__(256) void bn_bwd_kernel(const BnBwdArgs a0, const BnBwdArgs a1, const BnBwdArgs b0, const BnBwdArgs b1) {
   const BnBwdArgs& a = blockIdx.y == 0 ? a0 : blockIdx.y == 1 ? a1 : blockIdx.y == 2 ? b0 : b1;
@@ -836,29 +844,63 @@
   *p = desc_gather_cell(G, wave, (int)blockIdx.y, lane, *p);
 }
 
-__global__ __launch_bounds__(256) void desc_normalize_bwd_kernel(const float* __restrict__ desc0,
+template <bool FOLD = false>
+__global__ __launch_bounds__(256, FOLD ? 8 : 1) void desc_normalize_bwd_kernel(const float* __restrict__ desc0,
                                                                  const float* __restrict__ inv_norm0,
                                                                  float* __restrict__ d0, int ncells,
                                                                  const float* __restrict__ desc1 = nullptr,
                                                                  const float* __restrict__ inv_norm1 = nullptr,
                                                                  float* __restrict__ d1 = nullptr,
-                                                                 DescGather G = DescGather{nullptr, nullptr, nullptr, nullptr, 0, 0}) {
+                                                                 DescGather G = DescGather{nullptr, nullptr, nullptr, nullptr, 0, 0},
+                                                                 HeadBnSums F0 = HeadBnSums{nullptr, nullptr, nullptr, nullptr, 0, 0},
+                                                                 HeadBnSums F1 = HeadBnSums{nullptr, nullptr, nullptr, nullptr, 0, 0}) {
   const bool v1 = blockIdx.y != 0;
   const float* __restrict__ desc = v1 ? desc1 : desc0;
   const float* __restrict__ inv_norm = v1 ? inv_norm1 : inv_norm0;
   float* __restrict__ d = v1 ? d1 : d0;
-  const int wave = (blockIdx.x * blockDim.x + threadIdx.x) >> 6;
+  const HeadBnSums& F = v1 ? F1 : F0;
+  constexpr bool fold = FOLD;
   const int lane = threadIdx.x & 63;
-  if (wave >= ncells) return;
-  const float4 n = *reinterpret_cast<const float4*>(desc + (size_t)wave * 256 + lane * 4);
-  float4 g = *reinterpret_cast<const float4*>(d + (size_t)wave * 256 + lane * 4);
-  if (G.off != nullptr) g = desc_gather_cell(G, wave, v1 ? 1 : 0, lane, g);
-  float s = n.x * g.x + n.y * g.y + n.z * g.z + n.w * g.w;
-#pragma unroll
-  for (int o = 32; o > 0; o >>= 1) s += __shfl_xor(s, o);
-  const float inv = inv_norm[wave];
-  g = make_float4((g.x - n.x * s) * inv, (g.y - n.y * s) * inv, (g.z - n.z * s) * inv, (g.w - n.w * s) * inv);
-  *reinterpret_cast<float4*>(d + (size_t)wave * 256 + lane * 4) = g;
+  __shared__ float red[FOLD ? 5 : 1][FOLD ? 512 : 1];
+  float* const r1 = red[FOLD ? threadIdx.x >> 6 : 0] + (FOLD ? lane * 4 : 0);
+  const float* const par = red[FOLD ? 4 : 0] + (FOLD ? lane * 4 : 0);
+  if (fold) {
+    *reinterpret_cast<float4*>(r1) = make_float4(0.f, 0.f, 0.f, 0.f);
+    *reinterpret_cast<float4*>(r1 + 256) = make_float4(0.f, 0.f, 0.f, 0.f);
+    red[FOLD ? 4 : 0][FOLD ? threadIdx.x : 0] = F.mean[threadIdx.x];
+    red[FOLD ? 4 : 0][FOLD ? 256 + threadIdx.x : 0] = F.invstd[threadIdx.x];
+    __syncthreads();
+  }
+  for (int cell = (blockIdx.x * blockDim.x + threadIdx.x) >> 6; cell < ncells; cell += (gridDim.x * blockDim.x) >> 6) {
+    const float4 n = *reinterpret_cast<const float4*>(desc + (size_t)cell * 256 + lane * 4);
+    float4 g = *reinterpret_cast<const float4*>(d + (size_t)cell * 256 + lane * 4);
+    if (G.off != nullptr) g = desc_gather_cell(G, cell, v1 ? 1 : 0, lane, g);
+    float4 y = make_float4(0.f, 0.f, 0.f, 0.f), mu = y, is = y;
+    if (fold) {
+      y = *reinterpret_cast<const float4*>(F.y + (size_t)cell * F.y_cs + F.y_co + lane * 4);
+      mu = *reinterpret_cast<const float4*>(par);
+      is = *reinterpret_cast<const float4*>(par + 256);
+    }
+    float s = n.x * g.x + n.y * g.y + n.z * g.z + n.w * g.w;
+#pragma unroll
+    for (int o = 32; o > 0; o >>= 1) s += __shfl_xor(s, o);
+    const float inv = inv_norm[cell];
+    g = make_float4((g.x - n.x * s) * inv, (g.y - n.y * s) * inv, (g.z - n.z * s) * inv, (g.w - n.w * s) * inv);
+    *reinterpret_cast<float4*>(d + (size_t)cell * 256 + lane * 4) = g;
+    if (fold) {
+      float4 a1 = *reinterpret_cast<const float4*>(r1), a2 = *reinterpret_cast<const float4*>(r1 + 256);
+      a1.x += g.x; a1.y += g.y; a1.z += g.z; a1.w += g.w;
+      a2.x += g.x * ((y.x - mu.x) * is.x); a2.y += g.y * ((y.y - mu.y) * is.y);
+      a2.z += g.z * ((y.z - mu.z) * is.z); a2.w += g.w * ((y.w - mu.w) * is.w);
+      *reinterpret_cast<float4*>(r1) = a1;
+      *reinterpret_cast<float4*>(r1 + 256) = a2;
+    }
+  }
+  if (fold) {
+    __syncthreads();
+    double* sm = F.sums + (size_t)(blockIdx.x % NREP) * 512;
+    for (int t = threadIdx.x; t < 512; t += 256) acc_add_grad(sm + t, (double)(red[0][t] + red[1][t] + red[2][t] + red[3][t]));
+  }
 }
 
 __global__ void adam_kernel(float* __restrict__ p, const float* __restrict__ g, float* __restrict__ m,
diff --git a/semantic-superpoint_amd/csrc/loss_kernels.hip.h b/semantic-superpoint_amd/csrc/loss_kernels.hip.h
--- a/semantic-superpoint_amd/csrc/loss_kernels.hip.h
+++ b/semantic-superpoint_amd/csrc/loss_kernels.hip.h
@@ -2,6 +2,7 @@
 #include <hip/hip_runtime.h>
 #include <stdint.h>
 
+#include "bn_kernels.hip.h"
 #include "det.hip.h"
 
 namespace sspk {
@@ -120,8 +121,11 @@
                                                             const float* __restrict__ shift1 = nullptr,
                                                             const float* __restrict__ labels2d1 = nullptr,
                                                             const float* __restrict__ cellmask1 = nullptr,
-                                                            float* __restrict__ dsemi1 = nullptr) {
+                                                            float* __restrict__ dsemi1 = nullptr,
+                                                            HeadBnSums F0 = HeadBnSums{nullptr, nullptr, nullptr, nullptr, 0, 0},
+                                                            HeadBnSums F1 = HeadBnSums{nullptr, nullptr, nullptr, nullptr, 0, 0}) {
   const bool v1 = blockIdx.y != 0;
+  const HeadBnSums& F = v1 ? F1 : F0;
   const float* __restrict__ ypb = v1 ? ypb1 : ypb0;
   const float* __restrict__ scale = v1 ? scale1 : scale0;
   const float* __restrict__ shift = v1 ? shift1 : shift0;
@@ -136,6 +140,10 @@
   const float sc_l = scale[lane], sh_l = shift[lane], sc_d = scale[64], sh_d = shift[64];
   const float coef0 = (dsemi != nullptr) ? acc->coef_det / ((float)acc->mask_cnt[view] + 1e-5f) : 0.f;
   float lsum_acc = 0.f;
+  const bool fold = F.sums != nullptr && dsemi != nullptr;
+  const float mu_l = fold ? F.mean[lane] : 0.f, is_l = fold ? F.invstd[lane] : 0.f;
+  const float mu_d = fold ? F.mean[64] : 0.f, is_d = fold ? F.invstd[64] : 0.f;
+  float s1 = 0.f, s2 = 0.f, s1d = 0.f, s2d = 0.f;
   for (int cell = (blockIdx.x * blockDim.x + threadIdx.x) >> 6; cell < ncell; cell += (gridDim.x * blockDim.x) >> 6) {
     const int cx = cell % Wc, cy = (cell / Wc) % Hc, n = cell / (Wc * Hc);
     const float lab = labels2d[((size_t)n * H + cy * 8 + (lane >> 3)) * W + cx * 8 + (lane & 7)];
@@ -145,8 +153,9 @@
     const float dn = lsum + dust;
     const float t = lab / dn, td = dust / dn;
     const float* yp = ypb + (size_t)cell * cs;
-    const float s = fmaf(yp[lane], sc_l, sh_l);
-    const float sd = fmaf(yp[64], sc_d, sh_d);
+    const float y_l = yp[lane], y_d = yp[64];
+    const float s = fmaf(y_l, sc_l, sh_l);
+    const float sd = fmaf(y_d, sc_d, sh_d);
     const float mx = fmaxf(wave_max(s), sd);
     const float e = expf(s - mx), ed = expf(sd - mx);
     const float inv = 1.f / (wave_sum(e) + ed);
@@ -161,10 +170,25 @@
       const float gd = (pd - td) / fmaxf(pd * (1.f - pd), 1e-12f);
       const float dot = wave_sum(g * p) + gd * pd;
       float* dp = dsemi + (size_t)cell * cs;
-      dp[lane] = coef * p * (g - dot);
-      if (lane == 0) dp[64] = coef * pd * (gd - dot);
+      const float d_l = coef * p * (g - dot), d_d = coef * pd * (gd - dot);
+      dp[lane] = d_l;
+      if (lane == 0) dp[64] = d_d;
       if (lane >= 1 && lane < cs - 64) dp[64 + lane] = 0.f;
-    }
+      if (fold) {
+        s1 += d_l; s2 += d_l * ((y_l - mu_l) * is_l);
+        s1d += d_d; s2d += d_d * ((y_d - mu_d) * is_d);
+      }
+    }
+  }
+  if (fold) {
+    __shared__ float fred[4][130];
+    float* r = fred[threadIdx.x >> 6];
+    r[lane] = s1; r[65 + lane] = s2;
+    if (lane == 0) { r[64] = s1d; r[129] = s2d; }
+    __syncthreads();
+    if (threadIdx.x < 130)
+      acc_add_grad(F.sums + (size_t)(blockIdx.x % NREP) * 130 + threadIdx.x,
+                   (double)(fred[0][threadIdx.x] + fred[1][threadIdx.x] + fred[2][threadIdx.x] + fred[3][threadIdx.x]));
   }
   const float tot = block_sum_of_waves(lsum_acc, red);
   if (threadIdx.x == 0) acc_add_loss(&acc->det_sum[view], (double)tot);
diff --git a/semantic-superpoint_amd/csrc/ssp.hip b/semantic-superpoint_amd/csrc/ssp.hip
--- a/semantic-superpoint_amd/csrc/ssp.hip
+++ b/semantic-superpoint_amd/csrc/ssp.hip
@@ -222,6 +222,7 @@
   StepAccum* accum;
   float* dots;
   bool desc_gather = true;
+  int head_bn_fold = 1;
   int32_t *csr_off = nullptr, *csr_match = nullptr;
   float* csr_weight = nullptr;
   float* g_rows = nullptr;
@@ -1008,6 +1009,7 @@
   float* dg = nullptr;
   float* db = nullptr;
   bool filled = false;
+  bool sums_done = false;
 };
 struct BnSumsQueue {
   BnSumsJobs J;
@@ -1774,7 +1776,7 @@
 
 static int bn_layer_backward(ssp_handle* h, const SlotSet& SS, int l, const float* const* dout, int d_cs, int d_co, bool relu,
                              bool pool_after, float* const* dy, int dy_cs, int dy_co, int N, int H, int W, hipStream_t st,
-                             BnSumsQueue* queue = nullptr, BnPlainJob* collect = nullptr) {
+                             BnSumsQueue* queue = nullptr, BnPlainJob* collect = nullptr, bool plain_sums_done = false) {
   const LayerDesc& d = h->L[l];
   BnBwdArgs a[2];
   bool have_pool = true;
@@ -1834,9 +1836,10 @@
   }
   else if (collect != nullptr) {
     collect->a[0] = a0; collect->a[1] = a1; collect->dg = dg; collect->db = db; collect->filled = true;
+    collect->sums_done = plain_sums_done;
     return 0;
   }
-  else CHK((launch_bn_bwd<false, false>(a, SS.n, dg, db, st)));
+  else CHK((launch_bn_bwd<false, false>(a, SS.n, dg, db, st, plain_sums_done)));
   HIPCHK(hipGetLastError());
   return 0;
 }
@@ -1846,7 +1849,9 @@
     return std::min(cdiv((long)a.N * a.H * a.W, rows), 1024);
   };
   const int nb = std::max(blocks(p.a[0]), blocks(q.a[0]));
-  hipLaunchKernelGGL((bn_bwd_kernel<false, false, false, float>), dim3(nb, 4), dim3(256), 0, st, p.a[0], p.a[1], q.a[0], q.a[1]);
+  if (p.sums_done != q.sums_done) return fail(-3, "pointwise heads: pass 1 of one BatchNorm backward only");
+  if (!p.sums_done)
+    hipLaunchKernelGGL((bn_bwd_kernel<false, false, false, float>), dim3(nb, 4), dim3(256), 0, st, p.a[0], p.a[1], q.a[0], q.a[1]);
   BnSumsQueue sq;
   sq.J.n = 2; sq.maxC = std::max(p.a[0].C, q.a[0].C);
   sq.J.a0[0] = p.a[0]; sq.J.a1[0] = p.a[1]; sq.J.dgamma[0] = p.dg; sq.J.dbeta[0] = p.db;
@@ -2187,15 +2192,15 @@
 
 enum { EARLY_SPLIT_LAYER = 2 };
 static int run_backward_impl(ssp_handle* h, const SlotSet& SS, const float* const* dsemi, const float* const* draw_desc,
-                             float* const* dsout, hipStream_t st, int part);
+                             float* const* dsout, hipStream_t st, int part, bool head_sums);
 static int run_backward(ssp_handle* h, const SlotSet& SS, const float* const* dsemi, const float* const* draw_desc,
-                        float* const* dsout, hipStream_t st, int part = 0) {
+                        float* const* dsout, hipStream_t st, int part = 0, bool head_sums = false) {
   if (part != 2) h->bf16_fuse_apply = bf16_fuse_apply_env();
-  CHK(run_backward_impl(h, SS, dsemi, draw_desc, dsout, st, part));
+  CHK(run_backward_impl(h, SS, dsemi, draw_desc, dsout, st, part, head_sums));
   return det_fold(h->buf.grads_dev, st);
 }
 static int run_backward_impl(ssp_handle* h, const SlotSet& SS, const float* const* dsemi, const float* const* draw_desc,
-                             float* const* dsout, hipStream_t st, int part) {
+                             float* const* dsout, hipStream_t st, int part, bool head_sums) {
   Slot& S0 = *SS.s[0];
   if (h->rq_bf16 != nullptr) { h->rq_bf16->J.n = 0; h->rq_bf16->used = 0; }
   if (part != 2) { h->tail.g1_blocks = 0; h->tail.cs_views = 0; }
@@ -2240,6 +2245,7 @@
       CHK(dev_zero(S.gP, (size_t)N * Hc * Wc * hcs * sizeof(float), st));
   }
   if (bf16_path()) {
+    if (head_sums) return fail(-3, "backward: the loss kernels' BatchNorm sums are not taken by the bf16 path");
     CHK(heads_backward_bf16(h, SS, dsemi, draw_desc, dsout, st));
     if (part == 1) return encoder(7, EARLY_SPLIT_LAYER);
     return encoder(7, 0);
@@ -2283,21 +2289,22 @@
   };
   BnPlainJob job_pb, job_db;
   const bool pair = has_semi && has_desc && grouped && gw && SS.n == 2;
+  if (head_sums && !(has_semi && has_desc && SS.n == 2)) return fail(-3, "backward: BatchNorm sums of the loss kernels without both heads of a pair");
   if (pair) {
-    CHK(bn_layer_backward(h, SS, L_PB, dsemi, 80, 0, false, false, gQ, 80, 0, N, Hc, Wc, st, nullptr, &job_pb));
-    CHK(bn_layer_backward(h, SS, L_DB, draw_desc, 256, 0, false, false, gQd, 256, 0, N, Hc, Wc, st, nullptr, &job_db));
+    CHK(bn_layer_backward(h, SS, L_PB, dsemi, 80, 0, false, false, gQ, 80, 0, N, Hc, Wc, st, nullptr, &job_pb, head_sums));
+    CHK(bn_layer_backward(h, SS, L_DB, draw_desc, 256, 0, false, false, gQd, 256, 0, N, Hc, Wc, st, nullptr, &job_db, head_sums));
     if (!job_pb.filled || !job_db.filled) return fail(-3, "pointwise heads: BatchNorm backward not in the plain form");
     CHK(launch_bn_bwd_pair(job_pb, job_db, SS.n, st));
   }
   if (has_semi) {
-    if (!pair) CHK(bn_layer_backward(h, SS, L_PB, dsemi, 80, 0, false, false, gQ, 80, 0, N, Hc, Wc, st));
+    if (!pair) CHK(bn_layer_backward(h, SS, L_PB, dsemi, 80, 0, false, false, gQ, 80, 0, N, Hc, Wc, st, nullptr, nullptr, head_sums));
     CHK(conv_layer_backward(h, SS, L_PB, L_PA, gQ, 80, 0, dact, hcs, 0, N, Hc, Wc, 1, st, grouped, gw));
     CHK(tap_copy(h, SS, L_PB, 1, gQ, ncells_all * 80, st));
     if (grouped) add_dgrad(L_PB, gQ, 80, 0);
     if (gw) add_wgrad(L_PB, gQ, 80);
   }
   if (has_desc) {
-    if (!pair) CHK(bn_layer_backward(h, SS, L_DB, draw_desc, 256, 0, false, false, gQd, 256, 0, N, Hc, Wc, st));
+    if (!pair) CHK(bn_layer_backward(h, SS, L_DB, draw_desc, 256, 0, false, false, gQd, 256, 0, N, Hc, Wc, st, nullptr, nullptr, head_sums));
     CHK(conv_layer_backward(h, SS, L_DB, L_DA, gQd, 256, 0, dact, hcs, 256, N, Hc, Wc, 1, st, grouped, gw));
     CHK(tap_copy(h, SS, L_DB, 1, gQd, ncells_all * 256, st));
     if (grouped) add_dgrad(L_DB, gQd, 256, 256);
@@ -2431,7 +2438,7 @@
   if (ddesc_dev) {
     const long tot = (long)N * 256 * HW;
     hipLaunchKernelGGL(nchw_to_nhwc_kernel, dim3(cdiv(tot, 256)), dim3(256), 0, st, ddesc_dev, S.ddesc, N, HW, 256, 256, 0);
-    hipLaunchKernelGGL(desc_normalize_bwd_kernel, dim3(cdiv(ncells, 4)), dim3(256), 0, st, S.desc, S.inv_norm, S.ddesc, ncells);
+    hipLaunchKernelGGL(desc_normalize_bwd_kernel<false>, dim3(cdiv(ncells, 4)), dim3(256), 0, st, S.desc, S.inv_norm, S.ddesc, ncells);
     dd = S.ddesc;
   }
   if (dsem_dev) {
@@ -2541,6 +2548,12 @@
   const bool zero_dsout = semantic && in->train;
   const bool gather = h->desc_gather && in->train && use_desc && !dense;
   const int dflags = (in->sparse_method != 0 ? DESC_METHOD_1D : 0) | (in->sparse_dist != 0 ? DESC_EUCLIDEAN : 0);
+  const bool head_fold = h->head_bn_fold >= 1 && in->train && nv == 2 && use_desc && !dense && !bf16_path();
+  auto head_sums = [&](int l, int v) {
+    Slot& S = h->slot[v];
+    return head_fold ? HeadBnSums{S.Y[l], S.bn[l].mean, S.bn[l].invstd, S.bn[l].bsums, S.y_cs[l], S.y_co[l]}
+                     : HeadBnSums{nullptr, nullptr, nullptr, nullptr, 0, 0};
+  };
   {
     CHK(ensure_aux_stream(h));
     hipStream_t se = h->aux2_stream;
@@ -2583,7 +2596,7 @@
                          A.ddesc, pc);
       hipLaunchKernelGGL((dense_grad_kernel<true>), dim3(4, cdiv(pc, 64), B), dim3(256), 0, sd, h->dense_coef, A.desc,
                          Bs.ddesc, pc);
-      hipLaunchKernelGGL(desc_normalize_bwd_kernel, dim3(cdiv(ncells, 4), 2), dim3(256), 0, sd, A.desc, A.inv_norm, A.ddesc, ncells,
+      hipLaunchKernelGGL(desc_normalize_bwd_kernel<false>, dim3(cdiv(ncells, 4), 2), dim3(256), 0, sd, A.desc, A.inv_norm, A.ddesc, ncells,
                          Bs.desc, Bs.inv_norm, Bs.ddesc);
     }
     HIPCHK(hipGetLastError());
@@ -2621,8 +2634,12 @@
       CHK(det_fold(A.ddesc, sd));
       CHK(det_fold(Bs.ddesc, sd));
       const DescGather dg = {gather ? h->csr_off : nullptr, h->csr_match, h->csr_weight, h->g_rows, Hc * Wc, h->cfg.n_match};
-      hipLaunchKernelGGL(desc_normalize_bwd_kernel, dim3(cdiv(ncells, 4), 2), dim3(256), 0, sd, A.desc, A.inv_norm, A.ddesc, ncells,
-                         Bs.desc, Bs.inv_norm, Bs.ddesc, dg);
+      if (head_fold)
+        hipLaunchKernelGGL(desc_normalize_bwd_kernel<true>, dim3(std::min(cdiv(ncells, 4), 1024), 2), dim3(256), 0, sd, A.desc, A.inv_norm, A.ddesc,
+                           ncells, Bs.desc, Bs.inv_norm, Bs.ddesc, dg, head_sums(L_DB, 0), head_sums(L_DB, 1));
+      else
+        hipLaunchKernelGGL(desc_normalize_bwd_kernel<false>, dim3(cdiv(ncells, 4), 2), dim3(256), 0, sd, A.desc, A.inv_norm, A.ddesc, ncells,
+                           Bs.desc, Bs.inv_norm, Bs.ddesc, dg);
     }
     HIPCHK(hipGetLastError());
   }
@@ -2631,7 +2648,8 @@
     Slot &S = h->slot[0], &T = h->slot[nv - 1];
     hipLaunchKernelGGL(detector_loss_kernel, dim3(std::min(cdiv(ncells, 4), 1024), nv), dim3(256), 0, st, S.Y[L_PB], S.bn[L_PB].scale,
                        S.bn[L_PB].shift, labels[0], S.cellmask, in->train ? S.dsemi : nullptr, h->accum, 0, B, H, W, 80,
-                       T.Y[L_PB], T.bn[L_PB].scale, T.bn[L_PB].shift, labels[nv - 1], T.cellmask, in->train ? T.dsemi : nullptr);
+                       T.Y[L_PB], T.bn[L_PB].scale, T.bn[L_PB].shift, labels[nv - 1], T.cellmask, in->train ? T.dsemi : nullptr,
+                       head_sums(L_PB, 0), head_sums(L_PB, nv - 1));
   }
   HIPCHK(hipGetLastError());
   if (semantic) {
@@ -2651,7 +2669,7 @@
     const float* dss[2] = {h->slot[0].dsemi, nv == 2 ? h->slot[1].dsemi : nullptr};
     const float* dds[2] = {use_desc ? h->slot[0].ddesc : nullptr, use_desc ? h->slot[1].ddesc : nullptr};
     float* dsos[2] = {semantic ? h->slot[0].dsout : nullptr, semantic && nv == 2 ? h->slot[1].dsout : nullptr};
-    CHK(run_backward(h, SS, dss, dds, dsos, st, phase));
+    CHK(run_backward(h, SS, dss, dds, dsos, st, phase, head_fold));
   }
   return 0;
 }
@@ -2699,6 +2717,14 @@
   return 0;
 }
 
+int ssp_handle_set_head_bn_fold(ssp_handle* h, int value) {
+  if (!h) return fail(-1, "null handle");
+  if (value < 0 || value > 1) return fail(-1, "head_bn_fold must be 0 or 1 (got %d)", value);
+  h->head_bn_fold = value;
+  return 0;
+}
+int ssp_handle_get_head_bn_fold(const ssp_handle* h) { return h ? h->head_bn_fold : -1; }
+
 int ssp_pair_step(ssp_handle* h, const ssp_pair_inputs* in, float* scalars_dev, void* stream) {
   return pair_step_impl(h, in, scalars_dev, 0, (hipStream_t)stream);
 }
@@ -2716,15 +2742,15 @@
   hipStream_t st = (hipStream_t)stream;
   if (st == nullptr) return fail(-1, "ssp_pair_step_graph needs a non-default stream (stream capture)");
   if (h->tap_arena != nullptr) return fail(-1, "ssp_pair_step_graph: backward taps are on (ssp_debug_backward_taps); they need the eager step");
-  std::vector<unsigned char> key(sizeof(ssp_pair_inputs) + sizeof(void*) + 5 * sizeof(int));
+  std::vector<unsigned char> key(sizeof(ssp_pair_inputs) + sizeof(void*) + 6 * sizeof(int));
   {
     ssp_pair_inputs k;
     memcpy(&k, in, sizeof(k));
     k.seed = 0;
     memcpy(key.data(), &k, sizeof(k));
     memcpy(key.data() + sizeof(k), &scalars_dev, sizeof(void*));
-    const int extra[5] = {phase, sample_indices, h->conv_algo, bf16_fuse_apply_env() ? 1 : 0,
-                          h->desc_gather ? 1 : 0};
+    const int extra[6] = {phase, sample_indices, h->conv_algo, bf16_fuse_apply_env() ? 1 : 0,
+                          h->desc_gather ? 1 : 0, h->head_bn_fold};
     memcpy(key.data() + sizeof(k) + sizeof(void*), extra, sizeof(extra));
   }
   hipGraphExec_t exec = nullptr;
@@ -4332,6 +4358,7 @@
   else if (n.rfind("shift", 0) == 0) { int l = atoi(name + 5); p = S.bn[l].shift; cnt = h->L[l].cout; }
   else if (n.rfind("mean", 0) == 0) { int l = atoi(name + 4); p = S.bn[l].mean; cnt = h->L[l].cout; }
   else if (n.rfind("invstd", 0) == 0) { int l = atoi(name + 6); p = S.bn[l].invstd; cnt = h->L[l].cout; }
+  else if (n.rfind("k12", 0) == 0) { int l = atoi(name + 3); p = S.bn[l].k12; cnt = 2 * (size_t)h->L[l].cout; }
   else return fail(-1, "unknown buffer %s", name);
   *ptr = p;
   if (nfloats) *nfloats = cnt;
diff --git a/semantic-superpoint_amd/lib.py b/semantic-superpoint_amd/lib.py
--- a/semantic-superpoint_amd/lib.py
+++ b/semantic-superpoint_amd/lib.py
@@ -222,6 +222,8 @@
         "ssp_op_bn_bwd_strided": ([vp] * 9 + [i] * 7 + [vp], i),
         "ssp_set_conv_algo": ([i], i),
         "ssp_handle_set_conv_algo": ([vp, i], i),
+        "ssp_handle_set_head_bn_fold": ([vp, i], i),
+        "ssp_handle_get_head_bn_fold": ([vp], i),
         "ssp_debug_conv_knobs": ([i, i], i),
         "ssp_debug_occupancy": ([i], i),
         "ssp_debug_buffer": ([vp, i, C.c_char_p, P(vp), P(sz)], i),
@@ -405,6 +407,9 @@
         with torch.cuda.device(self.device):
             _check(self.lib.ssp_create(C.byref(cfg), C.byref(h)))
         self.h = h
+        fold = os.environ.get("SSP_HEAD_BN_FOLD")
+        if fold is not None and hasattr(self.lib, "ssp_handle_set_head_bn_fold"):
+            _check(self.lib.ssp_handle_set_head_bn_fold(h, int(fold)))
         self.layout, self.n_params = param_layout(arch, n_classes)
         self.bns, self.n_bn_ch = bn_layout(arch, n_classes)
         assert self.n_params == self.lib.ssp_param_count(h), "parameter layout mismatch with the library"
@@ -521,6 +526,12 @@
 
     def set_conv_algo(self, algo):
         _check(self.lib.ssp_handle_set_conv_algo(self.h, int(algo)))
+
+    def set_head_bn_fold(self, value):
+        _check(self.lib.ssp_handle_set_head_bn_fold(self.h, int(value)))
+
+    def get_head_bn_fold(self):
+        return int(self.lib.ssp_handle_get_head_bn_fold(self.h))
 
     @property
     def early_offset(self):
```
